# amathislab/HOISDF

Hardware: AMD Instinct MI355X
Metric: samples/sec (img + 2048 SDF queries) fwd+bwd at 1/2/4/8 MI355X (higher is better)
Workload: dtype f32 (emulated contractions, f32 accumulate, f16x2 form: operands as scaled hi + lo f16 pieces x 3 products - 22 operand bits, one power-of-two scale per ROW of a linear layer's row operand, per (sample, head) of the attention operands, per weight matrix; the attention backward's dS as three pieces x

## Files before the change

hoisdf_amd/csrc/chain.h:

```cpp
#pragma once
#include <stdlib.h>

#include <mutex>
#include <unordered_map>

#include "common.h"

namespace hoisdf {
namespace {

constexpr long EMU_MIN_ROWS = 2048;
constexpr long EMU_DW_MIN_ROWS = 8192;

inline bool al16(const void* p) { return (reinterpret_cast<uintptr_t>(p) & 15) == 0; }

struct Bump {
  char* base; long cap; long off = 0; bool overflow = false;
  Bump(void* b, long c) : base(static_cast<char*>(b)), cap(c) {}
  void* take(long bytes) {
    off = (off + 255) & ~255L;
    const long at = off;
    off += bytes;
    if (!base) return nullptr;
    if (off > cap) { overflow = true; return nullptr; }
    return base + at;
  }
  float* floats(long n) { return static_cast<float*>(take(n * 4)); }
};

struct SavedMags {
  std::mutex mu;
  std::unordered_map<const void*, int> on;
  void put(const void* key, bool v) { if (!key) return; std::lock_guard<std::mutex> l(mu); if (on.size() > 8192) on.clear(); on[key] = v ? 1 : 0; }
  int get(const void* key) { std::lock_guard<std::mutex> l(mu); auto it = on.find(key); return it == on.end() ? -1 : it->second; }
};
inline SavedMags& saved_mags() { static SavedMags s; return s; }

struct Ctx {
  hipStream_t st; void* stream;
  Bump* ws;
  bool dry;
  bool emu;
  int rc = HOISDF_OK;
  bool ok() const { return rc == HOISDF_OK; }
};

inline bool emu_small(const Ctx& c, long M, const float* a, long lda, const float* W, long ldw, int N, int K) {
  if (!c.emu || M > hoisdf_linear_emu_small_max_rows() || N % 4 || K % 4 || lda % 4 || ldw % 4) return false;
  return c.dry || hoisdf_linear_emu_small_supported(a, lda, W, ldw, M, N, K);
}
bool emu_rows(const Ctx& c, long M, const float* a, long lda, int contraction) {
  return c.emu && M >= EMU_MIN_ROWS && contraction % 4 == 0 && lda % 4 == 0 && (c.dry || al16(a));
}
const void* image_of(Ctx& c, const void* given, const float* W, int ldw, int N, int K, int transpose) {
  if (given) return given;
  void* img = c.ws->take(hoisdf_linear_emu_image_bytes(transpose ? K : N, transpose ? N : K));
  if (c.dry) return nullptr;
  if (!img) { c.rc = HOISDF_ERR_WORKSPACE; return nullptr; }
  c.rc = hoisdf_linear_emu_prepare(W, ldw, N, K, transpose, img, c.stream);
  return img;
}
void lin_fwd(Ctx& c, const float* x, int ldx, const float* W, int ldw, const void* img, const float* b, float* y, int ldy, long M, int N,
             int K, int act, float p, uint64_t seed, uint32_t* bits, int K_pad = 0, const uint32_t* x_mag = nullptr, uint32_t* y_mag = nullptr,
             uint32_t* y_heads = nullptr, int head_L = 0) {
  if (!c.ok()) return;
  if (K_pad < K || (K_pad + 15) / 16 != (K + 15) / 16) K_pad = K;
  if (emu_rows(c, M, x, ldx, K_pad)) {
    const void* im = image_of(c, img, W, ldw, N, K, 0);
    if (c.dry || !c.ok()) return;
    c.rc = linear_fwd_emu_mag(x, ldx, im, b, y, ldy, M, N, K_pad, act, p, seed, bits, x_mag, y_mag, c.stream, y_heads, head_L);
    return;
  }
  if (c.dry) return;
  if (emu_small(c, M, x, ldx, W, ldw, N, K)) { c.rc = hoisdf_linear_fwd_emu_small(x, ldx, W, ldw, b, y, ldy, M, N, K, act, p, seed, bits, c.stream); return; }
  c.rc = hoisdf_linear_fwd(x, ldx, W, ldw, b, y, ldy, M, N, K, act, p, seed, bits, c.stream);
}
void lin_bwd_input(Ctx& c, const float* dy, int lddy, const uint32_t* bits, float p, const float* W, int ldw, const void* img_t, float* dx,
                   int lddx, long M, int N, int K, int accumulate, const uint32_t* dy_mag = nullptr, uint32_t* dx_mag = nullptr,
                   uint32_t* dx_heads = nullptr, int head_L = 0) {
  if (!c.ok()) return;
  if (!bits) p = 0.f;
  if (emu_rows(c, M, dy, lddy, N)) {
    const void* im = image_of(c, img_t, W, ldw, N, K, 1);
    if (c.dry || !c.ok()) return;
    c.rc = linear_bwd_input_emu_mag(dy, lddy, bits, p, im, dx, lddx, M, N, K, accumulate, dy_mag, accumulate ? nullptr : dx_mag, c.stream,
                                    accumulate ? nullptr : dx_heads, head_L);
    return;
  }
  if (c.dry) return;
  if (emu_small(c, M, dy, lddy, W, ldw, N, K)) { c.rc = hoisdf_linear_bwd_input_emu_small(dy, lddy, bits, p, W, ldw, dx, lddx, M, N, K, accumulate, c.stream); return; }
  c.rc = hoisdf_linear_bwd_input(dy, lddy, bits, p, W, ldw, dx, lddx, M, N, K, accumulate, c.stream);
}
void lin_bwd_weight(Ctx& c, const float* dy, int lddy, const uint32_t* bits, float p, const float* x, int ldx, float* dW, float* db, long M,
                    int N, int K, int K_pad = 0, const uint32_t* dy_mag = nullptr, const uint32_t* x_mag = nullptr) {
  if (!c.ok()) return;
  if (!bits) p = 0.f;
  if (K_pad < K) K_pad = K;
  const bool emu = c.emu && M >= EMU_DW_MIN_ROWS && (N < K ? N : K) >= 64 && N % 4 == 0 && K_pad % 4 == 0 && lddy % 4 == 0 && ldx % 4 == 0 &&
                   (c.dry || (al16(dy) && al16(x) && al16(dW)));
  if (emu) {
    const long nws = hoisdf_linear_bwd_weight_emu_workspace(M, N, K_pad);
    float* w = c.ws->floats(nws > 4 ? nws : 4);
    if (!c.dry) {
      if (!w) { c.rc = HOISDF_ERR_WORKSPACE; return; }
      if (dy_mag || x_mag) c.rc = linear_bwd_weight_emu_mag(dy, lddy, bits, p, x, ldx, dW, K_pad, db, M, N, K_pad, w, nws, dy_mag, x_mag, c.stream);
      else c.rc = hoisdf_linear_bwd_weight_emu(dy, lddy, bits, p, x, ldx, dW, K_pad, db, M, N, K_pad, w, nws, c.stream);
    }
    return;
  }
  if (c.emu && M <= hoisdf_linear_emu_small_max_rows()) {
    if (!c.dry) c.rc = hoisdf_linear_bwd_weight_emu_small(dy, lddy, bits, p, x, ldx, dW, K_pad, db, M, N, K_pad, c.stream);
    return;
  }
  long nws = 0; float* w = nullptr;
  if (deterministic_mode()) {
    nws = hoisdf_linear_bwd_weight_workspace(M, N, K_pad);
    if (nws > 0) w = c.ws->floats(nws);
    if (!c.dry && nws > 0 && !w) { c.rc = HOISDF_ERR_WORKSPACE; return; }
  }
  if (c.dry) return;
  c.rc = hoisdf_linear_bwd_weight(dy, lddy, bits, p, x, ldx, dW, K_pad, db, M, N, K_pad, w, nws, c.stream);
}


}
}
```

hoisdf_amd/csrc/gemm_emu.h:

```cpp
#pragma once
#include "common.h"

namespace hoisdf {

typedef float f32x16 __attribute__((ext_vector_type(16)));
typedef float f32x4 __attribute__((ext_vector_type(4)));
typedef float f32x2 __attribute__((ext_vector_type(2)));
typedef __bf16 bf16x8 __attribute__((ext_vector_type(8)));
typedef __bf16 bf16x2 __attribute__((ext_vector_type(2)));
typedef _Float16 f16x8 __attribute__((ext_vector_type(8)));
typedef _Float16 f16x2 __attribute__((ext_vector_type(2)));
typedef unsigned int u32x4 __attribute__((ext_vector_type(4)));
typedef unsigned int u32x2 __attribute__((ext_vector_type(2)));
#define MFB(a, b, c) __builtin_amdgcn_mfma_f32_32x32x16_bf16((a), (b), (c), 0, 0, 0)
#define MFH(a, b, c) __builtin_amdgcn_mfma_f32_32x32x16_f16((a), (b), (c), 0, 0, 0)

constexpr int TM = 256, TN = 128, KS = 16, NT = 256;
constexpr int WN = TN / 2, NJ = WN / 32;
constexpr int A_U4 = 3 * 2 * TM, B_U4 = 3 * 2 * TN, STAGE_U4 = A_U4 + B_U4;
constexpr int NB = B_U4 / NT;
constexpr int HTM = 256, HTN = 256;
constexpr int HA_U4 = 2 * 2 * HTM, HB_U4 = 2 * 2 * HTN;
constexpr int H_TRAILER = 128;
constexpr int DT = 256;

#define SPLIT1(x, i)                             \
  do {                                           \
    const __bf16 a_ = (__bf16)(x);               \
    const float r1_ = (x) - (float)a_;           \
    const __bf16 b_ = (__bf16)r1_;               \
    const float r2_ = r1_ - (float)b_;           \
    p0[i] = a_; p1[i] = b_; p2[i] = (__bf16)r2_; \
  } while (0)
__device__ __forceinline__ void split3x8(const float4 u, const float4 w, bf16x8& p0, bf16x8& p1, bf16x8& p2) {
  SPLIT1(u.x, 0); SPLIT1(u.y, 1); SPLIT1(u.z, 2); SPLIT1(u.w, 3);
  SPLIT1(w.x, 4); SPLIT1(w.y, 5); SPLIT1(w.z, 6); SPLIT1(w.w, 7);
}

struct EmuArgs {
  const float* A; long lda;
  const u32x4* Bimg;
  float* C; int ldc;
  const float* bias;
  const uint32_t* abits; int ldbits; float ascale;
  uint32_t* bits_out; int ldbits_out;
  int M, N, K;
  int act; float drop_p, inv_keep; uint32_t thresh; uint64_t seed;
  int tiles_m, tiles_n, vecC, beta;
  QkvPlanes qkv;
  const uint32_t* a_amax; const float* b_scale;
  uint32_t* amax_out;
  uint32_t* head_out; int head_L, head_nb;
};

struct DwArgs {
  const float* dy; long lddy;
  const float* x; long ldx;
  const uint32_t* bits; int ldbits; float ascale;
  float* C; long c_split_stride;
  float* colsum; long colsum_split_stride;
  int M, N, K;
  int splitk, m_per_split, tiles_n, tiles_k;
  const uint32_t* dy_amax; const uint32_t* x_amax;
};

__device__ __forceinline__ uint32_t h2_exp(uint32_t amax_bits) { return mag_exp(amax_bits); }
__device__ __forceinline__ float h2_scale(uint32_t amax_bits) { return mag_scale(amax_bits); }
__device__ __forceinline__ float h2_inv_scale(uint32_t amax_bits) { return mag_inv_scale(amax_bits); }
__host__ __device__ __forceinline__ uint32_t* h2_trailer(void* image, int R, int Kc) {
  return reinterpret_cast<uint32_t*>(static_cast<char*>(image) + (size_t)((R + HTN - 1) / HTN) * ((Kc + KS - 1) / KS) * HB_U4 * 16);
}

#define EMU_PREP_FIND(items, n, lo)                                                                                    \
  int lo = 0, hi_ = (n) - 1;                                                                                           \
  while (lo < hi_) {                                                                                                   \
    const int mid_ = (lo + hi_ + 1) >> 1;                                                                              \
    if ((items)[mid_].first_block <= (long)blockIdx.x) lo = mid_; else hi_ = mid_ - 1;                                 \
  }

#define NOP_ ((void)0)
#define SYNC() do { SB(); __syncthreads(); SB(); } while (0)

#define EMU_A_DESCRIPTORS(TM_, arow0)                                                                                  \
  const int rows_in = min(TM_, g.M - m0);                                                                              \
  __amdgpu_buffer_rsrc_t rsa[4], rsm[4];                                                                               \
  _Pragma("unroll") for (int i = 0; i < 4; ++i) {                                                                      \
    const int rows_q = max(min(rows_in - i * 64, 64), 0);                              \
    rsa[i] = __builtin_amdgcn_make_buffer_rsrc(const_cast<float*>(g.A + ((size_t)(arow0) + i * 64) * g.lda), 0,        \
                                               rows_q > 0 ? (int)((((long)rows_q - 1) * g.lda + g.K) * 4) : 0, 0x00020000); \
    rsm[i] = __builtin_amdgcn_make_buffer_rsrc(const_cast<uint32_t*>(MASK ? g.abits + ((size_t)m0 + i * 64) * g.ldbits : nullptr), 0, \
                                               MASK ? (int)((long)rows_q * g.ldbits * 4) : 0, 0x00020000);             \
  }
#define EMU_A_SLOTS(TM_)                                                                                               \
  const int aoff = (int)((((long)wave * 16 + rl) * g.lda + 4 * qd) * 4);                                               \
  const int moff = (int)(((long)wave * 16 + rl) * g.ldbits * 4);                                                       \
  const int wslot = 2 * (cq * TM_ + ((wave * 16 + rl) ^ (cq << 2))) + (qd & 1);                                        \
  const int aread = (wm * 128 + l31) ^ (kh << 2);                                                                      \
  const int kq = g.K - 4 * qd;
#define EMU_LDGA(i, sl)                                                                                                \
  do {                                                                                                                 \
    const int k0_ = min((sl), last) * KS;                              \
    const f32x4 v_ = __builtin_bit_cast(f32x4, __builtin_amdgcn_raw_buffer_load_b128(rsa[i], aoff, k0_ * 4, 0));       \
    rp[2 * (i)] = f32x2{v_[0], v_[1]}; rp[2 * (i) + 1] = f32x2{v_[2], v_[3]};                                          \
    if (MASK) rm[i] = __builtin_amdgcn_raw_buffer_load_b32(rsm[i], moff, (k0_ >> 5) * 4, 0);                           \
  } while (0)
#define EMU_UI(i, sl) do { if (MASK) mb = rm[i] >> ((((sl) & 1) << 4) + 4 * qd); if (KTAIL) kin = (sl) * KS < kq; } while (0)
#define EMU_MASK_KTAIL(v_, p)                                                                                          \
  do {                                                                                                                 \
    if (MASK) {            \
      float xa_, xb_;      \
      asm("v_and_b32 %0, %1, %2" : "=v"(xa_) : "v"(__builtin_amdgcn_sbfe((int)mb, 2 * ((p) & 1), 1)), "v"(v_.x));       \
      asm("v_and_b32 %0, %1, %2" : "=v"(xb_) : "v"(__builtin_amdgcn_sbfe((int)mb, 2 * ((p) & 1) + 1, 1)), "v"(v_.y));   \
      v_ = f32x2{xa_, xb_};                                                                                            \
    }                                                                                                                  \
    if (KTAIL) { if (!kin) v_ = f32x2{0.f, 0.f}; }              \
  } while (0)

template <int TM_, int TN_, int NJ_>
__device__ __forceinline__ void emu_epilogue(const EmuArgs& g, f32x16 (&acc)[4][NJ_], u32x4* lds, int m0, int n0, int wm, int wn, int wave,
                                             int lane, int l31, int kh, float post_scale, const float* row_post = nullptr) {
  constexpr int WN_ = TN_ / 2;
  static_assert(WN_ == NJ_ * 32, "wave tile");
  if (row_post) {
#pragma unroll
    for (int i = 0; i < 4; ++i)
#pragma unroll
      for (int q = 0; q < 4; ++q) {
        const f32x4 ps = *reinterpret_cast<const f32x4*>(row_post + wm * 128 + i * 32 + 8 * q + 4 * kh);
#pragma unroll
        for (int j = 0; j < NJ_; ++j)
#pragma unroll
          for (int e = 0; e < 4; ++e) acc[i][j][4 * q + e] *= ps[e];
      }
  } else if (post_scale != 1.f) {
#pragma unroll
    for (int j = 0; j < NJ_; ++j)
#pragma unroll
      for (int i = 0; i < 4; ++i)
#pragma unroll
        for (int r = 0; r < 16; ++r) acc[i][j][r] *= post_scale;
  }
  const int rbase = m0 + wm * 128 + 4 * kh;
  const int cbase = n0 + wn * WN_ + l31;
#pragma unroll
  for (int j = 0; j < NJ_; ++j) {
    const int col = cbase + j * 32;
    const float bv = (g.bias != nullptr && col < g.N) ? g.bias[col] : 0.f;
#pragma unroll
    for (int i = 0; i < 4; ++i)
#pragma unroll
      for (int r = 0; r < 16; ++r) {
        float v = acc[i][j][r] + bv;
        if (g.act == 1) v = fmaxf(v, 0.f);
        acc[i][j][r] = v;
      }
  }
  if (g.drop_p > 0.f) {
#pragma unroll
    for (int i = 0; i < 4; ++i)
#pragma unroll
      for (int r = 0; r < 16; ++r) {
        const int row = rbase + i * 32 + (r & 3) + 8 * (r >> 2);
        const uint32_t rk = drop_rowkey(g.seed, (uint32_t)row);
#pragma unroll
        for (int j = 0; j < NJ_; ++j) acc[i][j][r] *= drop_scale(rk, (uint32_t)(cbase + j * 32), g.thresh, g.inv_keep);
      }
  }
  if (g.head_out) {
    const int row0 = m0 + wm * 128;
    if (row0 < g.M) {
      const int b0 = row0 / g.head_L, b1 = (min(row0 + 127, g.M - 1)) / g.head_L;
#pragma unroll
      for (int hh = 0; hh < NJ_ / 2; ++hh) {
        float m = 0.f;
#pragma unroll
        for (int j = 0; j < 2; ++j)
#pragma unroll
          for (int i = 0; i < 4; ++i)
#pragma unroll
            for (int r = 0; r < 16; ++r) m = fmaxf(m, __builtin_fabsf(acc[i][2 * hh + j][r]));
        uint32_t mb = group_max_u32<64>(__builtin_bit_cast(uint32_t, m));
        const int grp = (n0 + wn * WN_ + hh * 64) >> 6;
        if (lane == 0 && n0 + wn * WN_ + hh * 64 < g.N)
          for (int b = b0; b <= b1; ++b) atomicMax(g.head_out + (size_t)grp * g.head_nb + b, mb);
      }
    }
  }
  if (g.qkv.on) {
    constexpr int ES = 64 + 4;
    float* w = reinterpret_cast<float*>(lds) + wave * (32 * ES);
    const int row0 = m0 + wm * 128, cw = n0 + wn * WN_;
    if (row0 + 128 > g.M || cw + WN_ > g.N) return;
    const int b = row0 / g.qkv.L, s0 = row0 - b * g.qkv.L;
#pragma unroll
    for (int hh = 0; hh < NJ_ / 2; ++hh) {
      const int colg = g.qkv.col0 + cw + hh * 64;
      const int part = colg / g.qkv.E, head = (colg - part * g.qkv.E) >> 6;
      const size_t bh = (size_t)b * g.qkv.H + head;
      const float sc = part == 0 ? g.qkv.qscale : 1.f;
      __bf16* const r0 = static_cast<__bf16*>(g.qkv.r[part][0]);
      __bf16* const r1 = static_cast<__bf16*>(g.qkv.r[part][1]);
      __bf16* const r2 = static_cast<__bf16*>(g.qkv.r[part][2]);
      const bool trn = part == 2 && g.qkv.vt[0] != nullptr;
#pragma unroll
      for (int i = 0; i < 4; ++i) {
#pragma unroll
        for (int j = 0; j < 2; ++j)
#pragma unroll
          for (int r = 0; r < 16; ++r) w[((r & 3) + 8 * (r >> 2) + 4 * kh) * ES + j * 32 + l31] = acc[i][2 * hh + j][r] * sc;
        if (r0) {
#pragma unroll
          for (int p = 0; p < 4; ++p) {
            const int rr = p * 8 + (lane >> 3), cc = (lane & 7) * 8;
            const float4 u = *reinterpret_cast<const float4*>(w + rr * ES + cc);
            const float4 v = *reinterpret_cast<const float4*>(w + rr * ES + cc + 4);
            bf16x8 p0, p1, p2;
            split3x8(u, v, p0, p1, p2);
            const size_t o = ((size_t)bh * g.qkv.Lp + s0 + i * 32 + rr) * 64 + cc;
            *reinterpret_cast<bf16x8*>(r0 + o) = p0;
            *reinterpret_cast<bf16x8*>(r1 + o) = p1;
            *reinterpret_cast<bf16x8*>(r2 + o) = p2;
          }
        }
        if (trn) {
          __bf16* const t0 = static_cast<__bf16*>(g.qkv.vt[0]);
          __bf16* const t1 = static_cast<__bf16*>(g.qkv.vt[1]);
          __bf16* const t2 = static_cast<__bf16*>(g.qkv.vt[2]);
#pragma unroll
          for (int q = 0; q < 4; ++q) {
            const float* c0 = w + (8 * q) * ES + lane;
            const float4 u = make_float4(c0[0], c0[ES], c0[2 * ES], c0[3 * ES]);
            const float4 v = make_float4(c0[4 * ES], c0[5 * ES], c0[6 * ES], c0[7 * ES]);
            bf16x8 p0, p1, p2;
            split3x8(u, v, p0, p1, p2);
            const size_t o = ((size_t)bh * 64 + lane) * g.qkv.Lp + s0 + i * 32 + 8 * q;
            *reinterpret_cast<bf16x8*>(t0 + o) = p0;
            *reinterpret_cast<bf16x8*>(t1 + o) = p1;
            *reinterpret_cast<bf16x8*>(t2 + o) = p2;
          }
        }
      }
    }
    return;
  }
  const bool full = (m0 + TM_ <= g.M) && (n0 + TN_ <= g.N);
  const bool stream_c = !g.beta && (long)g.M * g.N >= (16L << 20);
  if (full && g.vecC) {
    constexpr int ES = WN_ + 4, LPR = WN_ / 4, RPI = 64 / LPR;
    float* w = reinterpret_cast<float*>(lds) + wave * (32 * ES);
#pragma unroll
    for (int i = 0; i < 4; ++i) {
#pragma unroll
      for (int j = 0; j < NJ_; ++j)
#pragma unroll
        for (int r = 0; r < 16; ++r) w[((r & 3) + 8 * (r >> 2) + 4 * kh) * ES + j * 32 + l31] = acc[i][j][r];
      if (g.amax_out) {
        const float* rp = w + l31 * ES + kh * (WN_ / 2);
        float m = 0.f;
#pragma unroll
        for (int q = 0; q < WN_ / 8; ++q) {
          const float4 t = *reinterpret_cast<const float4*>(rp + 4 * q);
          m = __builtin_fmaxf(__builtin_fmaxf(m, __builtin_fabsf(t.x)), __builtin_fmaxf(__builtin_fabsf(t.y), __builtin_fmaxf(__builtin_fabsf(t.z), __builtin_fabsf(t.w))));
        }
        uint32_t mb = __builtin_bit_cast(uint32_t, m);
        mb = max(mb, (uint32_t)__shfl_xor((int)mb, 32, 64));
        if (kh == 0) atomicMax(g.amax_out + (m0 + wm * 128 + i * 32 + l31), mb);
      }
#pragma unroll
      for (int p = 0; p < 32 / RPI; ++p) {
        const int rr = p * RPI + lane / LPR, cc = (lane % LPR) * 4;
        float4 v = *reinterpret_cast<const float4*>(w + rr * ES + cc);
        float4* cp = reinterpret_cast<float4*>(g.C + (size_t)(m0 + wm * 128 + i * 32 + rr) * g.ldc + n0 + wn * WN_ + cc);
        if (g.beta) {
          const float4 old = *cp;
          v.x += old.x; v.y += old.y; v.z += old.z; v.w += old.w;
        }
        typedef float v4f_ __attribute__((ext_vector_type(4)));
#ifdef H2_ABL_NOSTORE
        if (g.seed != 0x5eed5eed5eedull) continue;
#endif
        if (stream_c) __builtin_nontemporal_store(v4f_{v.x, v.y, v.z, v.w}, reinterpret_cast<v4f_*>(cp));
        else *cp = v;
      }
    }
  } else {
#pragma unroll
    for (int j = 0; j < NJ_; ++j)
#pragma unroll
      for (int i = 0; i < 4; ++i)
#pragma unroll
        for (int r = 0; r < 16; ++r) {
          const int row = rbase + i * 32 + (r & 3) + 8 * (r >> 2), col = cbase + j * 32;
          if (row < g.M && col < g.N) {
            float* cp = g.C + (size_t)row * g.ldc + col;
            *cp = g.beta ? *cp + acc[i][j][r] : acc[i][j][r];
          }
        }
    if (g.amax_out) {
#pragma unroll
      for (int i = 0; i < 4; ++i)
#pragma unroll
        for (int r = 0; r < 16; ++r) {
          const int row = rbase + i * 32 + (r & 3) + 8 * (r >> 2);
          uint32_t mb = 0u;
#pragma unroll
          for (int j = 0; j < NJ_; ++j) if (cbase + j * 32 < g.N) mb = max(mb, mag_bits(acc[i][j][r]));
          mb = group_max_u32<32>(mb);
          if (l31 == 0 && row < g.M) atomicMax(g.amax_out + row, mb);
        }
    }
  }
  if (g.bits_out) {
    uint32_t wd[2][NJ_];
#pragma unroll
    for (int hh = 0; hh < 2; ++hh)
#pragma unroll
      for (int j = 0; j < NJ_; ++j) wd[hh][j] = 0u;
#pragma unroll
    for (int i = 0; i < 4; ++i)
#pragma unroll
      for (int r = 0; r < 16; ++r) {
        const int rl = (i & 1) * 32 + (r & 3) + 8 * (r >> 2);
#pragma unroll
        for (int j = 0; j < NJ_; ++j) {
          const unsigned long long q = __ballot(acc[i][j][r] > 0.f);
          if (lane == rl) wd[i >> 1][j] = (uint32_t)q;
          if (lane == rl + 4) wd[i >> 1][j] = (uint32_t)(q >> 32);
        }
      }
    const int wcol = (n0 + wn * WN_) >> 5;
    const int nvalid = g.N - (n0 + wn * WN_);
#pragma unroll
    for (int hh = 0; hh < 2; ++hh) {
      const int row = m0 + wm * 128 + hh * 64 + lane;
      if (row < g.M) {
#pragma unroll
        for (int j = 0; j < NJ_; ++j) {
          const int nv = nvalid - 32 * j;
          if (nv > 0) g.bits_out[(size_t)row * g.ldbits_out + wcol + j] = nv >= 32 ? wd[hh][j] : (wd[hh][j] & ((1u << nv) - 1u));
        }
      }
    }
  }
}

int emu_b3_prepare(const float* W, int ldw, int R, int Kc, int transpose, void* image, hipStream_t st);
int emu_b3_prepare_batch(const hoisdf_emu_prep_item* d_items, int n, long total_blocks, hipStream_t st);
int emu_b3_launch(EmuArgs g, hipStream_t st);
int emu_h2_prepare(const float* W, int ldw, int N, int K, int transpose, void* image, hipStream_t st);
int emu_h2_prepare_batch(const hoisdf_emu_prep_item* d_items, int n, long total_blocks, hipStream_t st);
int emu_h2_launch(EmuArgs g, hipStream_t st);
int dw_tile(int K);
void plan_dw(long M, int N, int K, int& splitk, int& mper);
int emu_dw_launch(const DwArgs& g, bool h2, float* dW, float* db, float* workspace, hipStream_t st);
}
```

hoisdf_amd/csrc/gemm_emu.hip:

```cpp
#include <stdlib.h>

#include <map>
#include <mutex>
#include <unordered_map>
#include <utility>

#include "gemm_emu.h"

namespace hoisdf {

__global__ __launch_bounds__(256) void emu_rowmag_kernel(const float* __restrict__ x, long ld, long M, int K, uint32_t* __restrict__ words) {
  constexpr int RPW = 8;
  const int lane = threadIdx.x & 63;
  const long row0 = ((long)blockIdx.x * 4 + (threadIdx.x >> 6)) * RPW;
  const int k4 = K >> 2;
  uint32_t m[RPW];
#pragma unroll
  for (int r = 0; r < RPW; ++r) {
    m[r] = 0u;
    if (row0 + r < M)
      for (int c = lane; c < k4; c += 64) {
        const u32x4 v = *reinterpret_cast<const u32x4*>(x + (row0 + r) * ld + 4 * c);
        m[r] = max(m[r], max(max(v[0] & 0x7fffffffu, v[1] & 0x7fffffffu), max(v[2] & 0x7fffffffu, v[3] & 0x7fffffffu)));
      }
// ... 159 lines not shown

int hoisdf::linear_fwd_emu_mag(const float* x, int ldx, const void* w_image, const float* bias, float* y, int ldy, long M, int N, int K,
                               int act, float drop_p, uint64_t seed, uint32_t* relu_bits, const uint32_t* x_mag, uint32_t* y_mag,
                               void* stream, uint32_t* y_heads, int head_L) {
  HOISDF_REQUIRE(M == 0 || (x && w_image && y), HOISDF_ERR_INVALID, "linear_fwd_emu: null pointer");
  HOISDF_REQUIRE(M >= 0 && N > 0 && K > 0 && ldx >= K && ldy >= N && M < (1L << 31), HOISDF_ERR_INVALID,
                 "linear_fwd_emu: bad sizes M=%ld N=%d K=%d ldx=%d ldy=%d", M, N, K, ldx, ldy);
  HOISDF_REQUIRE(drop_p >= 0.f && drop_p < 1.f, HOISDF_ERR_INVALID, "linear_fwd_emu: drop_p=%f", drop_p);
  if (M == 0) return HOISDF_OK;
  HOISDF_REQUIRE(hoisdf_linear_emu_supported(x, ldx, K), HOISDF_ERR_INVALID,
                 "linear_fwd_emu: x must be 16-byte aligned with ldx and K multiples of 4 (use hoisdf_linear_fwd otherwise)");
  EmuArgs g{};
  g.A = x; g.lda = ldx; g.Bimg = static_cast<const u32x4*>(w_image);
  g.C = y; g.ldc = ldy; g.bias = bias; g.M = (int)M; g.N = N; g.K = K;
  g.act = act; g.drop_p = drop_p; g.inv_keep = 1.f / (1.f - drop_p); g.thresh = drop_threshold(drop_p); g.seed = seed;
  g.bits_out = relu_bits; g.ldbits_out = (N + 31) / 32;
  g.a_amax = x_mag; g.amax_out = y_mag;
  if (y_heads) {
    HOISDF_REQUIRE(head_L > 0 && N % 64 == 0, HOISDF_ERR_INVALID, "linear_fwd_emu: head magnitudes need N %% 64 == 0 and the rows per sample");
    g.head_out = y_heads; g.head_L = head_L; g.head_nb = cdiv(M, head_L);
  }
  return launch_emu(g, as_stream(stream));
}

int hoisdf::linear_fwd_emu_qkv(const float* x, int ldx, const void* w_image, const float* bias, long M, int N, int K,
                               const QkvPlanes& pl, void* stream, const uint32_t* x_mag) {
  HOISDF_REQUIRE(x && w_image && M > 0 && N > 0 && K > 0 && ldx >= K && M < (1L << 31), HOISDF_ERR_INVALID, "linear_fwd_emu_qkv: bad arguments");
  HOISDF_REQUIRE(hoisdf_linear_emu_supported(x, ldx, K), HOISDF_ERR_INVALID, "linear_fwd_emu_qkv: x alignment / K");
  HOISDF_REQUIRE(pl.on && pl.L > 0 && pl.L % 128 == 0 && M % pl.L == 0 && N % 64 == 0 && pl.E % 64 == 0 && pl.Lp >= pl.L &&
                     pl.col0 % 64 == 0 && pl.col0 + N <= 3 * pl.E,
                 HOISDF_ERR_INVALID, "linear_fwd_emu_qkv: plane geometry (L=%d Lp=%d N=%d E=%d col0=%d)", pl.L, pl.Lp, N, pl.E, pl.col0);
  EmuArgs g{};
  g.A = x; g.lda = ldx; g.Bimg = static_cast<const u32x4*>(w_image);
  g.C = nullptr; g.ldc = N; g.bias = bias; g.M = (int)M; g.N = N; g.K = K;
  g.inv_keep = 1.f; g.qkv = pl;
  g.a_amax = x_mag;
  return launch_emu(g, as_stream(stream));
}

extern "C" int hoisdf_linear_fwd_emu_heads(const float* x, int ldx, const void* w_image, const float* bias, float* y, int ldy, long M, int N,
                                           int K, const uint32_t* x_mag, uint32_t* y_mag, uint32_t* y_heads, int L, void* stream) {
  HOISDF_REQUIRE(y_heads, HOISDF_ERR_INVALID, "linear_fwd_emu_heads: y_heads is required");
  return linear_fwd_emu_mag(x, ldx, w_image, bias, y, ldy, M, N, K, 0, 0.f, 0, nullptr, x_mag, y_mag, stream, y_heads, L);
}
extern "C" int hoisdf_linear_bwd_input_emu_heads(const float* dy, int lddy, const void* wt_image, float* dx, int lddx, long M, int N, int K,
                                                 const uint32_t* dy_mag, uint32_t* dx_mag, uint32_t* dx_heads, int L, void* stream) {
  HOISDF_REQUIRE(dx_heads, HOISDF_ERR_INVALID, "linear_bwd_input_emu_heads: dx_heads is required");
  return linear_bwd_input_emu_mag(dy, lddy, nullptr, 0.f, wt_image, dx, lddx, M, N, K, 0, dy_mag, dx_mag, stream, dx_heads, L);
}
extern "C" int hoisdf_linear_bwd_input_emu(const float* dy, int lddy, const uint32_t* relu_bits, float drop_p,
                                           const void* wt_image, float* dx, int lddx, long M, int N, int K, int accumulate,
                                           void* stream) {
  return linear_bwd_input_emu_mag(dy, lddy, relu_bits, drop_p, wt_image, dx, lddx, M, N, K, accumulate, nullptr, nullptr, stream);
}
extern "C" int hoisdf_linear_bwd_input_emu_mag(const float* dy, int lddy, const uint32_t* relu_bits, float drop_p,
                                               const void* wt_image, float* dx, int lddx, long M, int N, int K, int accumulate,
                                               const uint32_t* dy_mag, uint32_t* dx_mag, void* stream) {
  return linear_bwd_input_emu_mag(dy, lddy, relu_bits, drop_p, wt_image, dx, lddx, M, N, K, accumulate, dy_mag, dx_mag, stream);
}

int hoisdf::linear_bwd_input_emu_mag(const float* dy, int lddy, const uint32_t* relu_bits, float drop_p, const void* wt_image, float* dx,
                                     int lddx, long M, int N, int K, int accumulate, const uint32_t* dy_mag, uint32_t* dx_mag,
                                     void* stream, uint32_t* dx_heads, int head_L) {
  HOISDF_REQUIRE(M == 0 || (dy && wt_image && dx), HOISDF_ERR_INVALID, "linear_bwd_input_emu: null pointer");
  HOISDF_REQUIRE(M >= 0 && N > 0 && K > 0 && lddy >= N && lddx >= K && M < (1L << 31) && drop_p >= 0.f && drop_p < 1.f,
                 HOISDF_ERR_INVALID, "linear_bwd_input_emu: bad sizes");
  if (M == 0) return HOISDF_OK;
  HOISDF_REQUIRE(hoisdf_linear_emu_supported(dy, lddy, N), HOISDF_ERR_INVALID,
                 "linear_bwd_input_emu: dy must be 16-byte aligned with lddy and N multiples of 4");
  EmuArgs g{};
  g.A = dy; g.lda = lddy; g.Bimg = static_cast<const u32x4*>(wt_image);
  g.abits = relu_bits; g.ldbits = (N + 31) / 32; g.ascale = 1.f / (1.f - drop_p);
  g.C = dx; g.ldc = lddx; g.M = (int)M; g.N = K; g.K = N;
  g.inv_keep = 1.f;
  g.beta = accumulate ? 1 : 0;
  g.a_amax = dy_mag; g.amax_out = dx_mag;
  if (dx_heads) {
    HOISDF_REQUIRE(head_L > 0 && K % 64 == 0 && !accumulate, HOISDF_ERR_INVALID, "linear_bwd_input_emu: head magnitudes need K %% 64 == 0, the rows per sample, no accumulation");
    g.head_out = dx_heads; g.head_L = head_L; g.head_nb = cdiv(M, head_L);
  }
  return launch_emu(g, as_stream(stream));
}

extern "C" long hoisdf_linear_bwd_weight_emu_workspace(long M, int N, int K) {
  if (M <= 0 || N <= 0 || K <= 0) return 0;
  int splitk, mper;
  plan_dw(M, N, K, splitk, mper);
  if (splitk <= 1) return 0;
  return (long)splitk * ((long)N * K + N);
}

namespace {
int bwd_weight_emu(const float* dy, int lddy, const uint32_t* relu_bits, float drop_p, const float* x, int ldx, float* dW, int lddw,
                   float* db, long M, int N, int K, float* workspace, long workspace_floats, bool h2, const uint32_t* dy_mag,
                   const uint32_t* x_mag, void* stream) {
  HOISDF_REQUIRE(dW && (M == 0 || (dy && x)), HOISDF_ERR_INVALID, "linear_bwd_weight_emu: null pointer");
  HOISDF_REQUIRE(M > 0 && N > 0 && K > 0 && lddy >= N && ldx >= K && lddw == K && M < (1L << 31) && drop_p >= 0.f && drop_p < 1.f,
                 HOISDF_ERR_INVALID, "linear_bwd_weight_emu: bad sizes (a dense dW, lddw == K, is required)");
  HOISDF_REQUIRE(al16(dy) && al16(x) && al16(dW) && (lddy % 4 == 0) && (ldx % 4 == 0) && (N % 4 == 0) && (K % 4 == 0),
                 HOISDF_ERR_INVALID, "linear_bwd_weight_emu: operands must be 16-byte aligned with N, K and leading dims multiples of 4");
  hipStream_t st = as_stream(stream);
  DwArgs g{};
  g.dy = dy; g.lddy = lddy; g.x = x; g.ldx = ldx;
  g.bits = relu_bits; g.ldbits = (N + 31) / 32; g.ascale = 1.f / (1.f - drop_p);
  g.M = (int)M; g.N = N; g.K = K;
  const int dtk = dw_tile(K);
  g.tiles_n = cdiv(N, DT); g.tiles_k = cdiv(K, dtk);
  plan_dw(M, N, K, g.splitk, g.m_per_split);
  const long need = g.splitk > 1 ? (long)g.splitk * ((long)N * K + N) : 0;
  HOISDF_REQUIRE(need == 0 || (workspace && workspace_floats >= need && al16(workspace)), HOISDF_ERR_WORKSPACE,
                 "linear_bwd_weight_emu: workspace of %ld floats needed", need);
  if (g.splitk > 1) {
    g.C = workspace; g.c_split_stride = (long)N * K;
    g.colsum = db ? workspace + (size_t)g.splitk * N * K : nullptr; g.colsum_split_stride = N;
  } else {
    g.C = dW; g.c_split_stride = 0; g.colsum = db; g.colsum_split_stride = 0;
  }
  if (dtk == 256 && h2) {
    g.dy_amax = dy_mag; g.x_amax = x_mag;
    if (!dy_mag) {
      uint32_t* part = mag_scratch(st, M);
      if (!part) { set_error("linear_bwd_weight_emu: cannot allocate the row magnitudes"); return HOISDF_ERR_LAUNCH; }
      mag_trace("grad-weight dy", M, N);
      if (int rc = emu_rowmag_launch(dy, lddy, M, N, part, st)) return rc;
      g.dy_amax = part;
    }
    if (!x_mag) {
      uint32_t* part = mag_scratch(st, M);
      if (!part) { set_error("linear_bwd_weight_emu: cannot allocate the row magnitudes"); return HOISDF_ERR_LAUNCH; }
      mag_trace("grad-weight x", M, K);
      if (int rc = emu_rowmag_launch(x, ldx, M, K, part, st)) return rc;
      g.x_amax = part;
    }
  }
  return emu_dw_launch(g, h2, dW, db, workspace, st);
}
}

extern "C" int hoisdf_linear_bwd_weight_emu(const float* dy, int lddy, const uint32_t* relu_bits, float drop_p, const float* x,
                                            int ldx, float* dW, int lddw, float* db, long M, int N, int K, float* workspace,
                                            long workspace_floats, void* stream) {
  return bwd_weight_emu(dy, lddy, relu_bits, drop_p, x, ldx, dW, lddw, db, M, N, K, workspace, workspace_floats, false, nullptr, nullptr, stream);
}
int hoisdf::linear_bwd_weight_emu_mag(const float* dy, int lddy, const uint32_t* relu_bits, float drop_p, const float* x, int ldx,
                                      float* dW, int lddw, float* db, long M, int N, int K, float* workspace, long workspace_floats,
                                      const uint32_t* dy_mag, const uint32_t* x_mag, void* stream) {
  return bwd_weight_emu(dy, lddy, relu_bits, drop_p, x, ldx, dW, lddw, db, M, N, K, workspace, workspace_floats, form_h2(), dy_mag, x_mag, stream);
}
extern "C" int hoisdf_linear_bwd_weight_emu_mag(const float* dy, int lddy, const uint32_t* relu_bits, float drop_p, const float* x,
                                                int ldx, float* dW, int lddw, float* db, long M, int N, int K, float* workspace,
                                                long workspace_floats, const uint32_t* dy_mag, const uint32_t* x_mag, void* stream) {
  return linear_bwd_weight_emu_mag(dy, lddy, relu_bits, drop_p, x, ldx, dW, lddw, db, M, N, K, workspace, workspace_floats, dy_mag, x_mag, stream);
}
```

hoisdf_amd/csrc/gemm_emu_dw.hip:

```cpp
#include "gemm_emu.h"

namespace hoisdf {

namespace {
__device__ __forceinline__ uint64_t uni64(uint64_t v) {
  const uint32_t lo = __builtin_amdgcn_readfirstlane((uint32_t)v), hi = __builtin_amdgcn_readfirstlane((uint32_t)(v >> 32));
  return ((uint64_t)hi << 32) | lo;
}
}

#define DW_TILE_SETUP(DTK_)                                                                                            \
  const int tid = threadIdx.x, lane = tid & 63, wave = tid >> 6;                                                       \
  const int wm = wave >> 1, wn = wave & 1;                                                                             \
  const int l31 = lane & 31, kh = lane >> 5;                                                                           \
  const int ntile = g.tiles_n * g.tiles_k;                                                                             \
  const int bid = blockIdx.x;                                                                                          \
  const int split = (bid & 7) + 8 * (bid / (8 * ntile));       \
  const int t = (bid >> 3) % ntile;                                                                                    \
  if (split >= g.splitk) return;                                                                                       \
  const int tn = t / g.tiles_k, tk = t - tn * g.tiles_k;                                                               \
  const int n0 = tn * DT, k0 = tk * DTK_;                                                                              \
  const int mbeg = split * g.m_per_split;                                                                              \
  const int mend = min(g.M, mbeg + g.m_per_split);                                                                     \
  const int nslab = (mend - mbeg + KS - 1) / KS;

#define DW2_STORE_COLSUM()                                                                                             \
  do {                                                                                                                 \
    if (HASDB && tk == 0) {                                                                                            \
      float* red = reinterpret_cast<float*>(lds);                                                                      \
      if (isA) *reinterpret_cast<f32x4*>(&red[c * DT + 4 * cg]) = csum * post;                                         \
      __syncthreads();                                                                                                 \
      if (tid < DT) {                                                                                                  \
        const int n = n0 + tid;                                                                                        \
        if (n < g.N) g.colsum[(size_t)split * g.colsum_split_stride + n] = red[tid] + red[DT + tid];                   \
      }                                                                                                                \
      __syncthreads();                                                                                                 \
    }                                                                                                                  \
  } while (0)
#define DW_EPILOGUE(DTK_, VAL)                                                                                         \
  do {                                                                                                                 \
    float* Cb = g.C + (size_t)split * g.c_split_stride;                                                                \
    const bool full = (n0 + DT <= g.N) && (k0 + (DTK_) <= g.K) && (g.K % 4 == 0);                                      \
    constexpr int WK_ = (DTK_) / 2, ES = WK_ + 4;                                                                      \
    constexpr int LPR = WK_ / 4, RPI = 64 / LPR;           \
    float* w = reinterpret_cast<float*>(lds) + wave * (32 * ES);                                                       \
    _Pragma("unroll") for (int i = 0; i < 4; ++i) {                                                                    \
      _Pragma("unroll") for (int j = 0; j < (DTK_) / 64; ++j)                                                          \
        _Pragma("unroll") for (int r = 0; r < 16; ++r) w[((r & 3) + 8 * (r >> 2) + 4 * kh) * ES + j * 32 + l31] = (VAL); \
      _Pragma("unroll") for (int p = 0; p < 32 / RPI; ++p) {                                                           \
        const int rr = p * RPI + lane / LPR, cc = (lane % LPR) * 4;                                                    \
        const int row = n0 + wm * 128 + i * 32 + rr, col = k0 + wn * WK_ + cc;                                         \
        const float4 v = *reinterpret_cast<const float4*>(w + rr * ES + cc);                                           \
        if (full) {                                                                                                    \
          *reinterpret_cast<float4*>(Cb + (size_t)row * g.K + col) = v;                                                \
        } else if (row < g.N) {                                                                                        \
          float* cp = Cb + (size_t)row * g.K + col;                                                                    \
          if (col + 0 < g.K) cp[0] = v.x;                                                                              \
          if (col + 1 < g.K) cp[1] = v.y;                                                                              \
          if (col + 2 < g.K) cp[2] = v.z;                                                                              \
          if (col + 3 < g.K) cp[3] = v.w;                                                                              \
        }                                                                                                              \
      }                                                                                                                \
    }                                                                                                                  \
  } while (0)

template <bool MASK, int DTK>
__global__ __launch_bounds__(NT, DTK == 256 ? 1 : 2) void emu_dw_kernel(DwArgs g) {
  constexpr int NJ = DTK / 64;
  constexpr int WK = DTK / 2;
  constexpr int A_U4 = 3 * 2 * DT, STAGE = A_U4 + 3 * 2 * DTK;
  extern __shared__ __attribute__((aligned(16))) u32x4 lds[];
  DW_TILE_SETUP(DTK)
  const int last = nslab - 1;

  f32x16 acc[4][NJ];
#pragma unroll
  for (int i = 0; i < 4; ++i)
#pragma unroll
    for (int j = 0; j < NJ; ++j)
#pragma unroll
      for (int r = 0; r < 16; ++r) acc[i][j][r] = 0.f;

  const bool isA = tid < 128;
  const bool stager = DTK == 256 || tid < 192;
  const int cg = (isA || DTK == 256) ? (tid & 63) : (tid & 31), c = (isA || DTK == 256) ? ((tid >> 6) & 1) : ((tid >> 5) & 1);
  const int col0 = (isA ? n0 : k0) + 4 * cg;
  const int ncol = isA ? g.N : g.K;
  const bool col_ok = stager && col0 < ncol;
  const long ld = uni64(isA ? g.lddy : g.ldx);
  const char* opbase = reinterpret_cast<const char*>(g.dy) +
                       (long)uni64(isA ? 0ul : (uint64_t)(reinterpret_cast<const char*>(g.x) - reinterpret_cast<const char*>(g.dy)));
  const uint32_t voff = (uint32_t)(((long)c * 8 * ld + (col_ok ? col0 : 0)) * 4);
  const char* bitbase = reinterpret_cast<const char*>(g.bits);
  const uint32_t boff = (uint32_t)(((long)c * 8 * g.ldbits + ((col_ok ? col0 : 0) >> 5)) * 4);
  const float* src = (isA ? g.dy : g.x) + (col_ok ? col0 : 0);
  const uint32_t* bsrc = (MASK && isA) ? g.bits + ((col_ok ? col0 : 0) >> 5) : nullptr;
  const int bsh = col0 & 31;
  const bool do_colsum = isA && g.colsum != nullptr && tk == 0;
  float4 rv[8];
  uint32_t rm[8];
  float4 csum = make_float4(0.f, 0.f, 0.f, 0.f);
#define DW_LOAD(sl)                                                                                                   \
  do {                                                                                                                \
    const int ms_ = mbeg + (sl) * KS;                                            \
    if (ms_ + KS <= g.M) {                                                                                            \
      const char* sb_ = opbase + (size_t)ms_ * ld * 4;                                                                \
      const char* mb2_ = bitbase + (size_t)ms_ * g.ldbits * 4;                                                        \
      _Pragma("unroll") for (int e = 0; e < 8; ++e) {                                                                 \
        rv[e] = *reinterpret_cast<const float4*>(sb_ + (size_t)e * ld * 4 + voff);                                    \
        if (MASK) rm[e] = isA ? *reinterpret_cast<const uint32_t*>(mb2_ + (size_t)e * g.ldbits * 4 + boff) : 0xffffffffu; \
      }                                                                                                               \
    } else {                                                       \
      const int mb_ = ms_ + c * 8;                                                                                    \
      _Pragma("unroll") for (int e = 0; e < 8; ++e) {                                                                 \
        const int m_ = min(mb_ + e, g.M - 1);                                                                         \
        rv[e] = *reinterpret_cast<const float4*>(src + (size_t)m_ * ld);                                              \
        if (MASK) rm[e] = isA ? bsrc[(size_t)m_ * g.ldbits] : 0xffffffffu;                                            \
      }                                                                                                               \
    }                                                                                                                 \
  } while (0)
#define DW_STORE(st, sl)                                                                                              \
  do {                                                                                                                \
    const int mb_ = mbeg + (sl) * KS + c * 8;                                                                         \
    _Pragma("unroll") for (int e = 0; e < 8; ++e) {                                                                   \
      float4 v_ = rv[e];                                                                                              \
      if (MASK && isA) {                                                                                              \
        const uint32_t nib_ = rm[e] >> bsh;                                                                           \
        v_.x = (nib_ & 1u) ? v_.x * g.ascale : 0.f;                                                                   \
        v_.y = (nib_ & 2u) ? v_.y * g.ascale : 0.f;                                                                   \
        v_.z = (nib_ & 4u) ? v_.z * g.ascale : 0.f;                                                                   \
        v_.w = (nib_ & 8u) ? v_.w * g.ascale : 0.f;                                                                   \
      }                                                                                                               \
      rv[e] = v_;                                                                                                     \
    }                                                                                                                 \
    if (!col_ok || mbeg + (sl) * KS + KS > mend) {            \
      _Pragma("unroll") for (int e = 0; e < 8; ++e)                                                                   \
        if (mb_ + e >= mend || !col_ok) rv[e] = make_float4(0.f, 0.f, 0.f, 0.f);                                      \
    }                                                                                                                 \
    if (do_colsum) {                                                                                                  \
      _Pragma("unroll") for (int e = 0; e < 8; ++e) {                                                                 \
        csum.x += rv[e].x; csum.y += rv[e].y; csum.z += rv[e].z; csum.w += rv[e].w;                                   \
      }                                                                                                               \
    }                                                                                                                 \
    const int rs_ = isA ? DT : DTK;                                \
    u32x4* dst_ = (st) + (isA ? 0 : A_U4) + c * rs_ + 4 * cg;                                                         \
    bf16x8 p0, p1, p2;                                                                                                \
    split3x8(make_float4(rv[0].x, rv[1].x, rv[2].x, rv[3].x), make_float4(rv[4].x, rv[5].x, rv[6].x, rv[7].x), p0, p1, p2); \
    dst_[0] = __builtin_bit_cast(u32x4, p0); dst_[2 * rs_] = __builtin_bit_cast(u32x4, p1); dst_[4 * rs_] = __builtin_bit_cast(u32x4, p2); \
    split3x8(make_float4(rv[0].y, rv[1].y, rv[2].y, rv[3].y), make_float4(rv[4].y, rv[5].y, rv[6].y, rv[7].y), p0, p1, p2); \
    dst_[1] = __builtin_bit_cast(u32x4, p0); dst_[2 * rs_ + 1] = __builtin_bit_cast(u32x4, p1); dst_[4 * rs_ + 1] = __builtin_bit_cast(u32x4, p2); \
    split3x8(make_float4(rv[0].z, rv[1].z, rv[2].z, rv[3].z), make_float4(rv[4].z, rv[5].z, rv[6].z, rv[7].z), p0, p1, p2); \
    dst_[2] = __builtin_bit_cast(u32x4, p0); dst_[2 * rs_ + 2] = __builtin_bit_cast(u32x4, p1); dst_[4 * rs_ + 2] = __builtin_bit_cast(u32x4, p2); \
    split3x8(make_float4(rv[0].w, rv[1].w, rv[2].w, rv[3].w), make_float4(rv[4].w, rv[5].w, rv[6].w, rv[7].w), p0, p1, p2); \
    dst_[3] = __builtin_bit_cast(u32x4, p0); dst_[2 * rs_ + 3] = __builtin_bit_cast(u32x4, p1); dst_[4 * rs_ + 3] = __builtin_bit_cast(u32x4, p2); \
  } while (0)

  if (nslab > 0 && stager) {
    DW_LOAD(0);
    DW_STORE(lds, 0);
    DW_LOAD(min(1, last));
  }
  __syncthreads();

  for (int s = 0; s < nslab; ++s) {
    const u32x4* st = lds + (s & 1) * STAGE;
    u32x4* nx = lds + ((s + 1) & 1) * STAGE;
    const u32x4* sa = st + wm * 128 + l31;
    const u32x4* sb = st + A_U4 + wn * WK + l31;
    bf16x8 b0[NJ], b1[NJ], b2[NJ], a[4];
#define RD_B(dst, p) _Pragma("unroll") for (int j = 0; j < NJ; ++j) dst[j] = __builtin_bit_cast(bf16x8, sb[((p) * 2 + kh) * DTK + j * 32])
#define RD_A(p) _Pragma("unroll") for (int i = 0; i < 4; ++i) a[i] = __builtin_bit_cast(bf16x8, sa[((p) * 2 + kh) * DT + i * 32])
#define MM1(bx) _Pragma("unroll") for (int i = 0; i < 4; ++i) _Pragma("unroll") for (int j = 0; j < NJ; ++j) acc[i][j] = MFB(a[i], bx[j], acc[i][j])
    RD_B(b0, 0); RD_A(0); RD_B(b1, 1); RD_B(b2, 2);
    MM1(b2); MM1(b1); MM1(b0);
    __builtin_amdgcn_sched_barrier(0);
    RD_A(1);
    if (stager) {
      if (s + 1 < nslab) DW_STORE(nx, s + 1);
      DW_LOAD(min(s + 2, last));
    }
    __builtin_amdgcn_sched_barrier(0);
    MM1(b1); MM1(b0);
    RD_A(2);
    MM1(b0);
    __syncthreads();
  }
#undef DW_LOAD
#undef DW_STORE
#undef RD_A
#undef RD_B
#undef MM1

  if (g.colsum != nullptr && tk == 0) {
    float* red = reinterpret_cast<float*>(lds);
    if (isA) *reinterpret_cast<float4*>(&red[c * DT + 4 * cg]) = csum;
    __syncthreads();
    if (tid < DT) {
      const int n = n0 + tid;
      if (n < g.N) g.colsum[(size_t)split * g.colsum_split_stride + n] = red[tid] + red[DT + tid];
    }
    __syncthreads();
  }

  DW_EPILOGUE(DTK, acc[i][j][r]);
}

#define DW2_STAGING_SETUP(A_U4_)                                                                                       \
   \
  const bool isA = wave < 2;                                                                                           \
  const int c = wave & 1, cg = lane;                                                                                   \
  const int col0 = (isA ? n0 : k0) + 4 * cg;                                                                           \
  const bool col_ok = col0 < (isA ? g.N : g.K);              \
  const long ld = uni64(isA ? g.lddy : g.ldx);                                                                         \
  const char* opbase = reinterpret_cast<const char*>(g.dy) +                                                           \
                       (long)uni64(isA ? 0ul : (uint64_t)(reinterpret_cast<const char*>(g.x) - reinterpret_cast<const char*>(g.dy))); \
   \
                                            \
  const int voff0 = col_ok ? (int)(((long)c * 8 * ld + col0) * 4) : 0x40000000;                                        \
  const int boff0 = (MASK && isA && col_ok) ? (int)(((long)c * 8 * g.ldbits + (col0 >> 5)) * 4) : 0x40000000;          \
  const int ldb4 = (int)(ld * 4), ldm4 = g.ldbits * 4;                                                                 \
  const uint32_t notA = isA ? 0u : 0xffffffffu;                                         \
  const int bsh = col0 & 31;                                    \
  constexpr bool SWZ = true;                                                                                           \
  const int sw = SWZ ? (cg >> 1) & 3 : 0;                                                                              \
  const int wbase = (isA ? 0 : A_U4_) + c * DT + 4 * cg;        \
  const int rsw = SWZ ? (l31 >> 3) & 3 : 0;                                                                            \
  const int aread = (wm * 128 + l31) ^ rsw, bread = A_U4_ + ((wn * 128 + l31) ^ rsw);                                  \
  f32x2 rvL[8], rvH[8];                                            \
  uint32_t rm[8], mpk = 0xffffffffu;
#define DSLAB(sl)                                                                                                      \
    const int ms_ = mbeg + (sl) * KS;                                                                                  \
    const int left_ = max(mend - ms_, 0);
#define DLDG(hf, e, sl)                                                                                                \
  do {                                                                                                                 \
    DSLAB(sl)                                                                                                          \
    const __amdgpu_buffer_rsrc_t r_ = __builtin_amdgcn_make_buffer_rsrc(                                               \
        const_cast<char*>(opbase + (size_t)ms_ * ld * 4), 0, (int)min((long)left_ * ld * 4, 0x3fffffffL), 0x00020000); \
    const f32x2 v_ = __builtin_bit_cast(f32x2, __builtin_amdgcn_raw_buffer_load_b64(r_, voff0 + (e) * ldb4 + (hf) * 8, 0, 0)); \
    if ((hf) == 0) rvL[e] = v_; else rvH[e] = v_;                                                                      \
  } while (0)
#define DLDM(e, sl)                                                                                                    \
  do {                                                                                                                 \
    if (MASK) {                                                                                                        \
      DSLAB(sl)                                                                                                        \
      const __amdgpu_buffer_rsrc_t b_ = __builtin_amdgcn_make_buffer_rsrc(                                             \
          const_cast<uint32_t*>(g.bits + (size_t)ms_ * g.ldbits), 0, (int)min((long)left_ * g.ldbits * 4, 0x3fffffffL), 0x00020000); \
      rm[e] = __builtin_amdgcn_raw_buffer_load_b32(b_, boff0 + (e) * ldm4, 0, 0);                                      \
    }                                                                                                                  \
  } while (0)
#define DLOAD_ALL(sl) _Pragma("unroll") for (int e = 0; e < 8; ++e) { DLDG(0, e, sl); DLDG(1, e, sl); }
#define DLOADM_ALL(sl) _Pragma("unroll") for (int e = 0; e < 8; ++e) DLDM(e, sl)

namespace {
constexpr int DSTAGE = 3 * 2 * DT * 2;
}
template <bool MASK, bool HASDB>
__global__ __launch_bounds__(NT, 1) void emu_dw2_kernel(DwArgs g) {
  constexpr int A_U4 = 3 * 2 * DT;
  __shared__ __attribute__((aligned(16))) u32x4 s0[DSTAGE];
  __shared__ __attribute__((aligned(16))) u32x4 s1[DSTAGE];
  DW_TILE_SETUP(DT)

  f32x16 acc[4][4];
#pragma unroll
  for (int i = 0; i < 4; ++i)
#pragma unroll
    for (int j = 0; j < 4; ++j)
#pragma unroll
      for (int r = 0; r < 16; ++r) acc[i][j][r] = 0.f;

  DW2_STAGING_SETUP(A_U4)
  uint32_t t0[4], t1[4], t2[4];
  f32x2 rp_, fu_;
  f32x4 csum = {0.f, 0.f, 0.f, 0.f};
#define DU1(j, pr)                                                                                                     \
  do {                                                                                                                 \
    f32x2 v_ = (j) < 2 ? f32x2{rvL[2 * (pr)][(j) & 1], rvL[2 * (pr) + 1][(j) & 1]} : f32x2{rvH[2 * (pr)][(j) & 1], rvH[2 * (pr) + 1][(j) & 1]}; \
    if (MASK) {                                                                                                        \
      if ((j) == 0) {                                                                                                  \
        const uint32_t n0_ = ((rm[2 * (pr)] | notA) >> bsh) & 0xfu, n1_ = ((rm[2 * (pr) + 1] | notA) >> bsh) & 0xfu;   \
        mpk = ((pr) == 0 ? 0u : mpk) | (n0_ << (8 * (pr))) | (n1_ << (8 * (pr) + 4));                                  \
      }                                                                                                                \
      float xa_, xb_;                                                              \
      asm("v_and_b32 %0, %1, %2" : "=v"(xa_) : "v"(__builtin_amdgcn_sbfe((int)mpk, 8 * (pr) + (j), 1)), "v"(v_.x));    \
      asm("v_and_b32 %0, %1, %2" : "=v"(xb_) : "v"(__builtin_amdgcn_sbfe((int)mpk, 8 * (pr) + 4 + (j), 1)), "v"(v_.y)); \
      v_ = f32x2{xa_, xb_};                                                                                            \
    }                                                                                                                  \
    if (HASDB) csum[j] += v_.x + v_.y;                                                                                 \
    const uint32_t h_ = __builtin_bit_cast(uint32_t, __builtin_convertvector(v_, bf16x2));                             \
    t0[pr] = h_; rp_ = v_;                                                                                             \
    fu_ = f32x2{__builtin_bit_cast(float, h_ << 16), __builtin_bit_cast(float, h_ & 0xffff0000u)};                     \
  } while (0)
#define DU2(j, pr) PK_SUB(rp_, rp_, fu_)
#define DU3(j, pr)                                                                                                     \
  do {                                                                                                                 \
    const uint32_t h_ = __builtin_bit_cast(uint32_t, __builtin_convertvector(rp_, bf16x2));                            \
    t1[pr] = h_;                                                                                                       \
    fu_ = f32x2{__builtin_bit_cast(float, h_ << 16), __builtin_bit_cast(float, h_ & 0xffff0000u)};                     \
  } while (0)
#define DU4(j, pr) do { f32x2 w_; PK_SUB(w_, rp_, fu_); t2[pr] = __builtin_bit_cast(uint32_t, __builtin_convertvector(w_, bf16x2)); } while (0)
#define DSTA(st, j, pl) (st)[wbase + ((j) ^ sw) + (pl) * 2 * DT] = ((pl) == 0 ? u32x4{t0[0], t0[1], t0[2], t0[3]} : (pl) == 1 ? u32x4{t1[0], t1[1], t1[2], t1[3]} : u32x4{t2[0], t2[1], t2[2], t2[3]})
#define DLA(st, p, i) __builtin_bit_cast(bf16x8, (st)[aread + ((p) * 2 + kh) * DT + (i) * 32])
#define DLB(st, p, j) __builtin_bit_cast(bf16x8, (st)[bread + ((p) * 2 + kh) * DT + (j) * 32])
#define M1(ax, bx, i, j, work) do { acc[i][j] = MFB(ax[i], bx[j], acc[i][j]); work; SB(); } while (0)
#define MM(ax, bx) _Pragma("unroll") for (int i = 0; i < 4; ++i) _Pragma("unroll") for (int j = 0; j < 4; ++j) acc[i][j] = MFB(ax[i], bx[j], acc[i][j])
#include "dw2_phase.inc"
#define DSTAGE_ALL(st)                                                                                                 \
  do {                                                                                                                 \
    _Pragma("unroll") for (int j = 0; j < 4; ++j) {                                                                    \
      _Pragma("unroll") for (int pr = 0; pr < 4; ++pr) { DU1(j, pr); DU2(j, pr); DU3(j, pr); DU4(j, pr); }             \
      DSTA(st, j, 0); DSTA(st, j, 1); DSTA(st, j, 2);                                                                  \
    }                                                                                                                  \
  } while (0)

  const int nslab2 = (max(nslab, 1) + 1) & ~1;
  bf16x8 aX[4], aY[4], aZ[4], bP[4], bQ[4], bR[4];
  DLOAD_ALL(0);
  DLOADM_ALL(0);
  DSTAGE_ALL(s0);
  DLOAD_ALL(1);
  DLOADM_ALL(1);
  __syncthreads();
#pragma unroll
  for (int i = 0; i < 4; ++i) { aZ[i] = DLA(s0, 0, i); aX[i] = DLA(s0, 1, i); aY[i] = DLA(s0, 2, i); }
#pragma unroll
  for (int j = 0; j < 4; ++j) { bQ[j] = DLB(s0, 0, j); bP[j] = DLB(s0, 1, j); bR[j] = DLB(s0, 2, j); }
  MM(aZ, bR); MM(aZ, bP); MM(aZ, bQ);
  DSTAGE_ALL(s1);
  DLOAD_ALL(2);
  DLOADM_ALL(2);
  SYNC();
  for (int s = 1; s + 1 < nslab2; s += 2) {
    DPHASE(s1, s0, s, aX, aY, aZ, bP, bQ, bR);
    SYNC();
    DPHASE(s0, s1, s + 1, aX, aY, aZ, bR, bQ, bP);
    SYNC();
  }
  DPHASE(s1, s0, nslab2 - 1, aX, aY, aZ, bP, bQ, bR);
  SB();
  MM(aX, bR); MM(aX, bQ); MM(aY, bQ);
  __syncthreads();
#undef DU1
#undef DU2
#undef DU3
#undef DU4
#undef DSTA
#undef DLA
#undef DLB
#undef M1
#undef MM
#undef DPHASE
#undef DSTAGE_ALL
  const float post = MASK ? g.ascale : 1.f;
  u32x4* lds = s0;
  DW2_STORE_COLSUM();
  DW_EPILOGUE(DT, MASK ? acc[i][j][r] * post : acc[i][j][r]);
}

template <bool MASK, bool HASDB>
__global__ __launch_bounds__(NT, 1) void emu_dw2h_kernel(DwArgs g) {
  constexpr int A_U4 = 2 * 2 * DT;
  constexpr int STG = 2 * A_U4;
  constexpr int EPI = (4 * 32 * (DT / 2 + 4) * 4 + 15) / 16;
  __shared__ __attribute__((aligned(16))) u32x4 lds_all[2 * STG > EPI ? 2 * STG : EPI];
  __shared__ uint32_t red4[4];
  u32x4* const s0 = lds_all;
  u32x4* const s1 = lds_all + STG;
  DW_TILE_SETUP(DT)
  f16_saturate_on();
  uint32_t am_dy = 0u, am_x = 0u;
  for (int i = mbeg + (int)threadIdx.x; i < mend; i += NT) { am_dy = max(am_dy, g.dy_amax[i]); am_x = max(am_x, g.x_amax[i]); }
  am_dy = block_max_u32(am_dy, red4);
  __syncthreads();
  am_x = block_max_u32(am_x, red4);

  f32x16 acc[4][4];
#pragma unroll
  for (int i = 0; i < 4; ++i)
#pragma unroll
    for (int j = 0; j < 4; ++j)
#pragma unroll
      for (int r = 0; r < 16; ++r) acc[i][j][r] = 0.f;

  DW2_STAGING_SETUP(A_U4)
  uint32_t t0[4], t1[4];
  const float sc = isA ? h2_scale(am_dy) : h2_scale(am_x);
  f32x2 rp_, fu_;
  f32x4 csum = {0.f, 0.f, 0.f, 0.f};
#define DU1(j, pr)                                                                                                     \
  do {                                                                                                                 \
    f32x2 v_ = (j) < 2 ? f32x2{rvL[2 * (pr)][(j) & 1], rvL[2 * (pr) + 1][(j) & 1]} : f32x2{rvH[2 * (pr)][(j) & 1], rvH[2 * (pr) + 1][(j) & 1]}; \
    if (MASK) {                                                                                                        \
      if ((j) == 0) {                                                                                                  \
        const uint32_t n0_ = ((rm[2 * (pr)] | notA) >> bsh) & 0xfu, n1_ = ((rm[2 * (pr) + 1] | notA) >> bsh) & 0xfu;   \
        mpk = ((pr) == 0 ? 0u : mpk) | (n0_ << (8 * (pr))) | (n1_ << (8 * (pr) + 4));                                  \
      }                                                                                                                \
      float xa_, xb_;                                                              \
      asm("v_and_b32 %0, %1, %2" : "=v"(xa_) : "v"(__builtin_amdgcn_sbfe((int)mpk, 8 * (pr) + (j), 1)), "v"(v_.x));    \
      asm("v_and_b32 %0, %1, %2" : "=v"(xb_) : "v"(__builtin_amdgcn_sbfe((int)mpk, 8 * (pr) + 4 + (j), 1)), "v"(v_.y)); \
      v_ = f32x2{xa_, xb_};                                                                                            \
    }                                                                                                                  \
    if (HASDB) csum[j] += v_.x + v_.y;                                                                                 \
    v_ *= sc;                                                                                                          \
    const f16x2 h_ = __builtin_convertvector(v_, f16x2);                       \
    t0[pr] = __builtin_bit_cast(uint32_t, h_); rp_ = v_;                                                               \
    fu_ = __builtin_convertvector(h_, f32x2);                                                                          \
  } while (0)
#define DU2(j, pr) do { f32x2 w_; PK_SUB(w_, rp_, fu_); t1[pr] = __builtin_bit_cast(uint32_t, __builtin_convertvector(w_, f16x2)); } while (0)
#define DSTA(st, j, pl) (st)[wbase + ((j) ^ sw) + (pl) * 2 * DT] = ((pl) == 0 ? u32x4{t0[0], t0[1], t0[2], t0[3]} : u32x4{t1[0], t1[1], t1[2], t1[3]})
#define DLA(st, p, i) __builtin_bit_cast(f16x8, (st)[aread + ((p) * 2 + kh) * DT + (i) * 32])
#define DLB(st, p, j) __builtin_bit_cast(f16x8, (st)[bread + ((p) * 2 + kh) * DT + (j) * 32])
#define M1(ax, bx, i, j, work) do { acc[i][j] = MFH(ax[i], bx[j], acc[i][j]); work; SB(); } while (0)
#define MM(ax, bx) _Pragma("unroll") for (int i = 0; i < 4; ++i) _Pragma("unroll") for (int j = 0; j < 4; ++j) acc[i][j] = MFH(ax[i], bx[j], acc[i][j])
#include "dw2h_phase.inc"
#define DSTAGE_ALL(st)                                                                                                 \
  do {                                                                                                                 \
    _Pragma("unroll") for (int j = 0; j < 4; ++j) {                                                                    \
      _Pragma("unroll") for (int pr = 0; pr < 4; ++pr) { DU1(j, pr); DU2(j, pr); }                                     \
      DSTA(st, j, 0); DSTA(st, j, 1);                                                                                  \
    }                                                                                                                  \
  } while (0)

  const int nslab2 = (max(nslab, 1) + 1) & ~1;
  f16x8 aH[4], aL[4], bP[4], bQ[4], bL[4];
  DLOAD_ALL(0);
  DLOADM_ALL(0);
  DSTAGE_ALL(s0);
  DLOAD_ALL(1);
  DLOADM_ALL(1);
  __syncthreads();
#pragma unroll
  for (int i = 0; i < 4; ++i) { aL[i] = DLA(s0, 1, i); aH[i] = DLA(s0, 0, i); }
#pragma unroll
  for (int j = 0; j < 4; ++j) { bP[j] = DLB(s0, 0, j); bL[j] = DLB(s0, 1, j); }
  MM(aL, bP); MM(aH, bL);
  DSTAGE_ALL(s1);
  DLOAD_ALL(2);
  DLOADM_ALL(2);
  SYNC();
  for (int s = 1; s + 1 < nslab2; s += 2) {
    DHPHASE(s1, s0, s, bP, bQ);
    SYNC();
    DHPHASE(s0, s1, s + 1, bQ, bP);
    SYNC();
  }
  DHPHASE(s1, s0, nslab2 - 1, bP, bQ);
  SB();
  MM(aH, bQ);
  __syncthreads();
#undef DU1
#undef DU2
#undef DSTA
#undef DLA
#undef DLB
#undef M1
#undef MM
#undef DHPHASE
#undef DSTAGE_ALL
  const float unscale = h2_inv_scale(am_dy) * h2_inv_scale(am_x);
  const float post = MASK ? g.ascale : 1.f;
  u32x4* lds = lds_all;
  DW2_STORE_COLSUM();
  DW_EPILOGUE(DT, acc[i][j][r] * (MASK ? post * unscale : unscale));
}

__global__ __launch_bounds__(1024) void emu_reduce_partials_kernel(const float* __restrict__ part, long stride, int splits,
                                                                   float* __restrict__ out, long n, int blocks0,
                                                                   const float* __restrict__ part1, long stride1,
                                                                   float* __restrict__ out1, long n1) {
  __shared__ float4 red[16][64];
  const int lane = threadIdx.x & 63, w = threadIdx.x >> 6;
  int blk = blockIdx.x;
  if (blk >= blocks0) { blk -= blocks0; part = part1; stride = stride1; out = out1; n = n1; }
  const long i = ((long)blk * 64 + lane) * 4;
  float4 s = make_float4(0.f, 0.f, 0.f, 0.f);
  if (i < n) {
    const float* p = part + i;
    int k = w;
    for (; k + 16 < splits; k += 32) {
      const float4 u = *reinterpret_cast<const float4*>(p + (size_t)k * stride);
      const float4 v = *reinterpret_cast<const float4*>(p + (size_t)(k + 16) * stride);
      s.x += u.x; s.y += u.y; s.z += u.z; s.w += u.w;
      s.x += v.x; s.y += v.y; s.z += v.z; s.w += v.w;
    }
    if (k < splits) {
      const float4 u = *reinterpret_cast<const float4*>(p + (size_t)k * stride);
      s.x += u.x; s.y += u.y; s.z += u.z; s.w += u.w;
    }
  }
  red[w][lane] = s;
  __syncthreads();
  if (w == 0 && i < n) {
    float4 t = red[0][lane];
#pragma unroll
    for (int j = 1; j < 16; ++j) {
      const float4 v = red[j][lane];
      t.x += v.x; t.y += v.y; t.z += v.z; t.w += v.w;
    }
    *reinterpret_cast<float4*>(out + i) = t;
  }
}

int dw_tile(int K) { return K <= 128 ? 128 : 256; }
void plan_dw(long M, int N, int K, int& splitk, int& mper) {
  const int dtk = dw_tile(K);
  const int ntile = cdiv(N, DT) * cdiv(K, dtk);
  const int slabs = cdiv(M, KS);
  const int slots = dtk == 256 ? 256 : 512;
  const int per_xcd = slots / 8 / ntile;
  int want = per_xcd >= 1 ? per_xcd * 8 : (ntile >= slots ? 1 : slots / ntile);
  if (want > slabs / 8) want = slabs / 8 > 0 ? slabs / 8 : 1;
  mper = cdiv(slabs, want) * KS;
  splitk = cdiv(M, mper);
}

int emu_dw_launch(const DwArgs& g, bool h2, float* dW, float* db, float* workspace, hipStream_t st) {
  const int dtk = dw_tile(g.K);
  const unsigned lb = 2u * (3 * 2 * DT + 3 * 2 * 128) * 16u;
  static bool attr_set = false;
  if (!attr_set) {
    auto raise = [&](const void* k) { return hipFuncSetAttribute(k, hipFuncAttributeMaxDynamicSharedMemorySize, (int)lb) == hipSuccess; };
    const bool ok = raise(reinterpret_cast<const void*>(emu_dw_kernel<false, 128>)) && raise(reinterpret_cast<const void*>(emu_dw_kernel<true, 128>));
    if (!ok) {
      set_error("linear_bwd_weight_emu: cannot raise the dynamic LDS limit");
      return HOISDF_ERR_LAUNCH;
    }
    attr_set = true;
  }
  const dim3 grid((unsigned)(g.tiles_n * g.tiles_k * 8 * cdiv(g.splitk, 8))), block(NT);
  const bool mask = g.bits != nullptr, hasdb = g.colsum != nullptr;
  static void (*const dw2h[2][2])(DwArgs) = {{emu_dw2h_kernel<false, false>, emu_dw2h_kernel<false, true>},
                                             {emu_dw2h_kernel<true, false>, emu_dw2h_kernel<true, true>}};
  static void (*const dw2[2][2])(DwArgs) = {{emu_dw2_kernel<false, false>, emu_dw2_kernel<false, true>},
                                            {emu_dw2_kernel<true, false>, emu_dw2_kernel<true, true>}};
  if (dtk == 256) hipLaunchKernelGGL((h2 ? dw2h : dw2)[mask][hasdb], grid, block, 0, st, g);
  else hipLaunchKernelGGL((mask ? emu_dw_kernel<true, 128> : emu_dw_kernel<false, 128>), grid, block, lb, st, g);
  if (int rc = check_launch("linear_bwd_weight_emu")) return rc;
  if (g.splitk > 1) {
    const long n = (long)g.N * g.K;
    const int b0 = (int)((n + 255) / 256), b1 = db ? (g.N + 255) / 256 : 0;
    hipLaunchKernelGGL(emu_reduce_partials_kernel, dim3((unsigned)(b0 + b1)), dim3(1024), 0, st, workspace, n, g.splitk, dW, n, b0,
                       workspace + (size_t)g.splitk * g.N * g.K, (long)g.N, db, (long)g.N);
    return check_launch("linear_bwd_weight_emu reduce");
  }
  return HOISDF_OK;
}

}
```

hoisdf_amd/csrc/heads.hip:

```cpp
#include "chain.h"

using namespace hoisdf;

namespace {
constexpr int MLP_MAX = HOISDF_MLP_MAX_LAYERS;
inline long bits_words(int N) { return (N + 31) / 32; }

struct MlpSaved { float* h[MLP_MAX]; uint32_t* bits[MLP_MAX]; uint32_t* mag; };

bool mlp_ok(const hoisdf_mlp* m) {
  if (!m || m->n_layers < 1 || m->n_layers > MLP_MAX) return false;
  for (int i = 0; i <= m->n_layers; ++i) if (m->dims[i] <= 0) return false;
  return true;
}
void mlp_carve(const hoisdf_mlp* m, long M, Bump& b, MlpSaved& s) {
  const int last = m->n_layers - 1;
  for (int i = 0; i < m->n_layers; ++i) {
    s.h[i] = i < last ? b.floats(M * m->dims[i + 1]) : nullptr;
    const bool act = i < last || m->act_last;
    s.bits[i] = act ? static_cast<uint32_t*>(b.take(M * bits_words(m->dims[i + 1]) * 4)) : nullptr;
  }
  s.mag = static_cast<uint32_t*>(b.take((long)m->n_layers * M * 4));
}
inline bool chain_mags_on(const Ctx& c, long M) { return c.emu && emu_form_h2() && M >= EMU_MIN_ROWS; }
uint32_t* chain_mags(Ctx& c, long M, int n) {
  if (!chain_mags_on(c, M)) return nullptr;
  uint32_t* p = static_cast<uint32_t*>(c.ws->take((long)n * M * 4));
  if (c.dry || !p || !c.ok()) return nullptr;
  if (hipMemsetAsync(p, 0, (size_t)n * M * 4, c.st) != hipSuccess) { c.rc = HOISDF_ERR_LAUNCH; return nullptr; }
  return p;
}
void mlp_forward(Ctx& c, const hoisdf_mlp* m, const float* x, int ldx, long M, const MlpSaved& s, float* y, int ldy, const uint32_t* x_mag = nullptr) {
  const int last = m->n_layers - 1;
  const float* in = x; int ldin = ldx;
  uint32_t* mg = chain_mags_on(c, M) && !c.dry && s.mag && c.ok() ? s.mag : nullptr;
  if (!c.dry) saved_mags().put(s.mag, mg != nullptr);
  if (mg && hipMemsetAsync(mg, 0, (size_t)m->n_layers * M * 4, c.st) != hipSuccess) { c.rc = HOISDF_ERR_LAUNCH; return; }
  const uint32_t* in_mag = mg ? x_mag : nullptr;
  if (mg && !in_mag && emu_rows(c, M, x, ldx, m->dims[0])) {
    if ((c.rc = emu_mag_measure(x, ldx, M, m->dims[0], mg, c.st)) != HOISDF_OK) return;
    in_mag = mg;
  }
  for (int i = 0; i < m->n_layers; ++i) {
    float* out = i < last ? s.h[i] : y;
    const int ldo = i < last ? m->dims[i + 1] : ldy;
    uint32_t* out_mag = mg && i < last && emu_rows(c, M, in, ldin, m->dims[i]) ? mg + (long)(i + 1) * M : nullptr;
    lin_fwd(c, in, ldin, m->w[i], m->dims[i], m->img[i], m->b[i], out, ldo, M, m->dims[i + 1], m->dims[i], s.bits[i] ? 1 : 0, 0.f, 0, s.bits[i], 0,
            in_mag, out_mag);
    in = out; ldin = ldo; in_mag = out_mag;
  }
}
void mlp_backward(Ctx& c, const hoisdf_mlp* m, const hoisdf_mlp_grads* G, const float* x, int ldx, long M, const MlpSaved& s, const float* dy,
                  int lddy, float* dx, int lddx, int accumulate_dx, const uint32_t* x_mag = nullptr) {
  const float* g = dy; int ldg = lddy;
  const int last = m->n_layers - 1;
  uint32_t* mg = chain_mags(c, M, m->n_layers + 1);
  const bool fwd_mags = mg && s.mag && saved_mags().get(s.mag) != 0;
  const uint32_t* g_mag = nullptr;
  if (mg && emu_rows(c, M, dy, lddy, m->dims[last + 1])) {
    if ((c.rc = emu_mag_measure(dy, lddy, M, m->dims[last + 1], mg + (long)(last + 1) * M, c.st)) != HOISDF_OK) return;
    g_mag = mg + (long)(last + 1) * M;
  }
  for (int i = last; i >= 0; --i) {
    const float* in = i > 0 ? s.h[i - 1] : x;
    const int ldin = i > 0 ? m->dims[i] : ldx;
    const uint32_t* in_mag = !fwd_mags ? nullptr : i > 0 ? (emu_rows(c, M, i > 1 ? s.h[i - 2] : x, i > 1 ? m->dims[i - 1] : ldx, m->dims[i - 1]) ? s.mag + (long)i * M : nullptr)
                                                         : (x_mag ? x_mag : (emu_rows(c, M, x, ldx, m->dims[0]) ? s.mag : nullptr));
    lin_bwd_weight(c, g, ldg, s.bits[i], 0.f, in, ldin, G->dw[i], G->db[i], M, m->dims[i + 1], m->dims[i], 0, g_mag, g_mag ? in_mag : nullptr);
    if (i == 0 && !dx) break;
    float* gin = i > 0 ? c.ws->floats(M * m->dims[i]) : dx;
    const int ldgin = i > 0 ? m->dims[i] : lddx;
    if (!c.dry && c.ok() && !gin) { c.rc = HOISDF_ERR_WORKSPACE; return; }
    uint32_t* gin_mag = mg && i > 0 && emu_rows(c, M, g, ldg, m->dims[i + 1]) ? mg + (long)i * M : nullptr;
    lin_bwd_input(c, g, ldg, s.bits[i], 0.f, m->w[i], m->dims[i], m->img_t[i], gin, ldgin, M, m->dims[i + 1], m->dims[i], i == 0 ? accumulate_dx : 0,
                  g_mag, gin_mag);
    g = gin; ldg = ldgin; g_mag = gin_mag;
  }
}
const uint32_t* enc_mag(const Ctx& c, const hoisdf_mlp* m, const float* x, int ldx, long M, const MlpSaved& s) {
  return chain_mags_on(c, M) && !c.dry && s.mag && saved_mags().get(s.mag) != 0 && emu_rows(c, M, x, ldx, m->dims[0]) ? s.mag : nullptr;
}
bool grads_ok(const hoisdf_mlp* m, const hoisdf_mlp_grads* G) {
  if (!G) return false;
  for (int i = 0; i < m->n_layers; ++i) if (!G->dw[i] || !G->db[i]) return false;
  return true;
}

struct TokSaved { float* feat; float* fea; MlpSaved mlp; };
void tok_carve(const hoisdf_mlp* m, long M, bool own_feat, Bump& b, TokSaved& s) {
  s.feat = own_feat ? b.floats(M * m->dims[0]) : nullptr;
  s.fea = b.floats(M * m->dims[m->n_layers]);
  mlp_carve(m, M, b, s.mlp);
}

struct VoteSaved { float *off, *cls, *stats; MlpSaved vote, cl; };
void vote_carve(const hoisdf_mlp* mv, const hoisdf_mlp* mc, long M, int LB, int J, Bump& b, VoteSaved& s) {
  s.off = b.floats(M * 3 * J); s.cls = b.floats(M * J); s.stats = b.floats((long)LB * J * 2);
  mlp_carve(mv, M, b, s.vote); mlp_carve(mc, M, b, s.cl);
}
}

extern "C" long hoisdf_tokens_saved_bytes(const hoisdf_mlp* mlp, long n_rows, int gather_inside) {
  if (!mlp_ok(mlp) || n_rows <= 0) return 0;
  Bump b(nullptr, 0); TokSaved s;
  tok_carve(mlp, n_rows, gather_inside != 0, b, s);
  return b.off + 256;
}

static int tokens_backward(const hoisdf_mlp* mlp, const hoisdf_mlp_grads* G, const float* feat, long M, TokSaved& s, const float* dtok,
                           const float* sdf, const float* beta, float* dfeat, int accumulate_dfeat, float* dbeta, int B, int P, int S, int row0,
                           int D, Bump& ws, bool dry, void* stream) {
  Ctx c{as_stream(stream), stream, &ws, dry, gemm_emu_mode()};
  const int F = mlp->dims[mlp->n_layers];
  float* dfea = ws.floats(M * F);
  float* part = ws.floats(hoisdf_token_build_bwd_partials());
  if (!dry) {
    if (!dfea || !part) { set_error("tokens_bwd: workspace too small"); return HOISDF_ERR_WORKSPACE; }
    c.rc = hoisdf_token_build_bwd_ordered(dtok, s.fea, F, sdf, beta, dfea, F, dbeta, part, B, P, S, row0, D, stream);
  }
  mlp_backward(c, mlp, G, feat, mlp->dims[0], M, s.mlp, dfea, F, dfeat, mlp->dims[0], accumulate_dfeat);
  if (c.ok() && !dry && ws.overflow) { set_error("tokens_bwd: workspace too small"); return HOISDF_ERR_WORKSPACE; }
  return c.rc;
}

extern "C" long hoisdf_tokens_workspace_bytes(const hoisdf_mlp* mlp, long n_rows, int backward_pass) {
  if (!mlp_ok(mlp) || n_rows <= 0) return 0;
  Bump ws(nullptr, 0), sv(nullptr, 0);
  TokSaved s; tok_carve(mlp, n_rows, false, sv, s);
  Ctx c{nullptr, nullptr, &ws, true, gemm_emu_mode()};
  if (backward_pass) {
    hoisdf_mlp_grads G{};
    (void)tokens_backward(mlp, &G, nullptr, n_rows, s, nullptr, nullptr, nullptr, reinterpret_cast<float*>(1), 0, nullptr, 1, 1, 1, 0, 1, ws, true, nullptr);
  } else {
    mlp_forward(c, mlp, nullptr, mlp->dims[0], n_rows, s.mlp, nullptr, mlp->dims[mlp->n_layers]);
  }
  return ws.off + 256;
}

extern "C" int hoisdf_tokens_fwd(const hoisdf_pyramid* pyr, const float* points, const float* center, const float* cam_intr, float scale,
                                 int img_h, int img_w, const float* feat_in, const float* cam_in, const hoisdf_mlp* mlp, const float* pe,
                                 const float* sdf, const float* beta_ptr, float* tok, float* fea_out, float* cam_out, int B, int P, int S,
                                 int row0, int D, void* saved, long saved_bytes, void* workspace, long workspace_bytes, void* stream) {
  HOISDF_REQUIRE(mlp_ok(mlp) && center && pe && sdf && beta_ptr && tok && saved && workspace, HOISDF_ERR_INVALID, "tokens_fwd: null pointer / bad MLP");
  HOISDF_REQUIRE(B > 0 && P > 0 && S >= row0 + P && row0 >= 0 && mlp->act_last && mlp->dims[mlp->n_layers] == D - 33, HOISDF_ERR_INVALID,
                 "tokens_fwd: bad sizes (the MLP must end in D - 33 = %d activated columns)", D - 33);
  const bool gather = feat_in == nullptr;
  HOISDF_REQUIRE(gather ? (pyr && points && cam_intr && cam_out) : (cam_in != nullptr), HOISDF_ERR_INVALID,
                 "tokens_fwd: either gathered rows + their camera points, or a pyramid + points + cam_out");
  const long M = (long)B * P;
  HOISDF_REQUIRE(saved_bytes >= hoisdf_tokens_saved_bytes(mlp, M, gather), HOISDF_ERR_WORKSPACE, "tokens_fwd: saved buffer of %ld bytes, need %ld", saved_bytes,
                 hoisdf_tokens_saved_bytes(mlp, M, gather));
  Bump sv(saved, saved_bytes), ws(workspace, workspace_bytes);
  TokSaved s; tok_carve(mlp, M, gather, sv, s);
  Ctx c{as_stream(stream), stream, &ws, false, gemm_emu_mode()};
  const int C = mlp->dims[0], F = D - 33;
  const float* feat = feat_in;
  const float* cam = cam_in;
  if (gather) {
    c.rc = hoisdf_project_gather_fwd(pyr, points, nullptr, M, P, center, cam_intr, scale, img_h, img_w, s.feat, C, cam_out, nullptr, stream);
    feat = s.feat; cam = cam_out;
  }
  mlp_forward(c, mlp, feat, C, M, s.mlp, s.fea, F);
  if (c.ok()) c.rc = hoisdf_token_build_fwd(cam, center, pe, s.fea, F, sdf, beta_ptr, tok, B, P, S, row0, D, stream);
  if (c.ok() && fea_out && hipMemcpyAsync(fea_out, s.fea, sizeof(float) * M * F, hipMemcpyDeviceToDevice, c.st) != hipSuccess) c.rc = HOISDF_ERR_LAUNCH;
  if (c.ok() && (sv.overflow || ws.overflow)) c.rc = HOISDF_ERR_WORKSPACE;
  if (c.rc == HOISDF_ERR_WORKSPACE) set_error("tokens_fwd: workspace (%ld bytes) too small", workspace_bytes);
  return c.rc;
}

extern "C" int hoisdf_tokens_bwd(const hoisdf_pyramid_grad* dpyr, const float* points, const float* center, const float* cam_intr, float scale,
                                 int img_h, int img_w, const float* feat_in, const hoisdf_mlp* mlp, const float* sdf, const float* beta_ptr,
                                 const float* dtok, const void* saved, long saved_bytes, const hoisdf_mlp_grads* grads, float* dfeat,
                                 int accumulate_dfeat, float* dbeta, int B, int P, int S, int row0, int D, void* workspace, long workspace_bytes,
                                 void* stream) {
  HOISDF_REQUIRE(mlp_ok(mlp) && grads_ok(mlp, grads) && sdf && beta_ptr && dtok && saved && dbeta && workspace, HOISDF_ERR_INVALID,
                 "tokens_bwd: null pointer (every weight-gradient buffer is required, zero-filled)");
  const bool gather = feat_in == nullptr;
  const long M = (long)B * P;
  HOISDF_REQUIRE(B > 0 && P > 0 && saved_bytes >= hoisdf_tokens_saved_bytes(mlp, M, gather), HOISDF_ERR_INVALID, "tokens_bwd: bad sizes / saved buffer");
  HOISDF_REQUIRE(gather ? (points && center && cam_intr) : true, HOISDF_ERR_INVALID, "tokens_bwd: the gather's arguments are needed again");
  Bump sv(const_cast<void*>(saved), saved_bytes), ws(workspace, workspace_bytes);
  TokSaved s; tok_carve(mlp, M, gather, sv, s);
  const int C = mlp->dims[0];
  float* df = dfeat;
  int acc = accumulate_dfeat;
  if (gather && dpyr && !df) {
    df = ws.floats(M * C); acc = 0;
    if (!df) { set_error("tokens_bwd: workspace too small"); return HOISDF_ERR_WORKSPACE; }
  }
  int rc = tokens_backward(mlp, grads, gather ? s.feat : feat_in, M, s, dtok, sdf, beta_ptr, df, acc, dbeta, B, P, S, row0, D, ws, false, stream);
  if (rc == HOISDF_OK && gather && dpyr && df)
    rc = hoisdf_project_gather_bwd(dpyr, points, nullptr, M, P, center, cam_intr, scale, img_h, img_w, df, C, stream);
  return rc;
}

extern "C" long hoisdf_heads_vote_saved_bytes(const hoisdf_mlp* vote, const hoisdf_mlp* cls, int L, int B, int P, int J) {
  if (!mlp_ok(vote) || !mlp_ok(cls) || L <= 0 || B <= 0 || P <= 0 || J <= 0) return 0;
  Bump b(nullptr, 0); VoteSaved s;
  vote_carve(vote, cls, (long)L * B * P, L * B, J, b, s);
  return b.off + 256;
}

static int heads_vote_backward(const hoisdf_mlp* mv, const hoisdf_mlp* mc, const hoisdf_mlp_grads* Gv, const hoisdf_mlp_grads* Gc, const float* enc,
                               const float* pts, const float* gt, float radius, const float* joints, VoteSaved& s, const float* djoints,
                               const float* dl3d, const float* dbce, float* denc, int L, int B, int P, int J, Bump& ws, bool dry, void* stream) {
  Ctx c{as_stream(stream), stream, &ws, dry, gemm_emu_mode()};
  const long M = (long)L * B * P;
  float* doff = ws.floats(M * 3 * J); float* dcls = ws.floats(M * J);
  if (!dry) {
    if (!doff || !dcls) { set_error("heads_vote_bwd: workspace too small"); return HOISDF_ERR_WORKSPACE; }
    c.rc = hoisdf_vote_loss_bwd(s.off, s.cls, pts, gt, radius, joints, s.stats, djoints, dl3d, dbce, doff, dcls, L, B, P, J, stream);
  }
  const int E = mv->dims[0];
  mlp_backward(c, mv, Gv, enc, E, M, s.vote, doff, 3 * J, denc, E, 0);
  mlp_backward(c, mc, Gc, enc, E, M, s.cl, dcls, J, denc, E, 1, enc_mag(c, mv, enc, E, M, s.vote));
  if (c.ok() && !dry && ws.overflow) { set_error("heads_vote_bwd: workspace too small"); return HOISDF_ERR_WORKSPACE; }
  return c.rc;
}

extern "C" long hoisdf_heads_vote_workspace_bytes(const hoisdf_mlp* vote, const hoisdf_mlp* cls, int L, int B, int P, int J, int backward_pass) {
  if (!mlp_ok(vote) || !mlp_ok(cls) || L <= 0 || B <= 0 || P <= 0 || J <= 0) return 0;
  const long M = (long)L * B * P;
  Bump ws(nullptr, 0), sv(nullptr, 0);
  VoteSaved s; vote_carve(vote, cls, M, L * B, J, sv, s);
  if (backward_pass) {
    hoisdf_mlp_grads G{};
    (void)heads_vote_backward(vote, cls, &G, &G, nullptr, nullptr, nullptr, 0.f, nullptr, s, nullptr, nullptr, nullptr, reinterpret_cast<float*>(1), L, B, P, J, ws,
                              true, nullptr);
  } else {
    Ctx c{nullptr, nullptr, &ws, true, gemm_emu_mode()};
    mlp_forward(c, vote, nullptr, vote->dims[0], M, s.vote, nullptr, 3 * J);
    mlp_forward(c, cls, nullptr, cls->dims[0], M, s.cl, nullptr, J);
  }
  return ws.off + 256;
}

extern "C" int hoisdf_heads_vote_fwd(const float* enc, const hoisdf_mlp* vote, const hoisdf_mlp* cls, const float* pts, const float* joint_gt_mm,
                                     float radius, float* joints, float* l3d_sum, float* bce_sum, float* near_sum, int L, int B, int P, int J,
                                     void* saved, long saved_bytes, void* workspace, long workspace_bytes, void* stream) {
  HOISDF_REQUIRE(enc && mlp_ok(vote) && mlp_ok(cls) && pts && joint_gt_mm && joints && l3d_sum && bce_sum && near_sum && saved && workspace,
                 HOISDF_ERR_INVALID, "heads_vote_fwd: null pointer / bad MLP");
  HOISDF_REQUIRE(L > 0 && B > 0 && P > 0 && J > 0 && vote->dims[vote->n_layers] == 3 * J && cls->dims[cls->n_layers] == J &&
                     vote->dims[0] == cls->dims[0] && !vote->act_last && !cls->act_last,
                 HOISDF_ERR_INVALID, "heads_vote_fwd: the vote MLP must end in 3 J = %d, the class MLP in J = %d plain columns", 3 * J, J);
  HOISDF_REQUIRE(saved_bytes >= hoisdf_heads_vote_saved_bytes(vote, cls, L, B, P, J), HOISDF_ERR_WORKSPACE, "heads_vote_fwd: saved buffer too small");
  const long M = (long)L * B * P;
  Bump sv(saved, saved_bytes), ws(workspace, workspace_bytes);
  VoteSaved s; vote_carve(vote, cls, M, L * B, J, sv, s);
  Ctx c{as_stream(stream), stream, &ws, false, gemm_emu_mode()};
  const int E = vote->dims[0];
  mlp_forward(c, vote, enc, E, M, s.vote, s.off, 3 * J);
  mlp_forward(c, cls, enc, E, M, s.cl, s.cls, J, enc_mag(c, vote, enc, E, M, s.vote));
  if (c.ok()) c.rc = hoisdf_vote_loss_fwd(s.off, s.cls, pts, joint_gt_mm, radius, joints, s.stats, l3d_sum, bce_sum, near_sum, L, B, P, J, stream);
  if (c.ok() && (sv.overflow || ws.overflow)) c.rc = HOISDF_ERR_WORKSPACE;
  if (c.rc == HOISDF_ERR_WORKSPACE) set_error("heads_vote_fwd: workspace (%ld bytes) too small", workspace_bytes);
  return c.rc;
}

extern "C" int hoisdf_heads_vote_bwd(const float* enc, const hoisdf_mlp* vote, const hoisdf_mlp* cls, const float* pts, const float* joint_gt_mm,
                                     float radius, const float* joints, const void* saved, long saved_bytes, const float* djoints,
                                     const float* dl3d_sum, const float* dbce_sum, const hoisdf_mlp_grads* vote_grads,
                                     const hoisdf_mlp_grads* cls_grads, float* denc, int L, int B, int P, int J, void* workspace,
                                     long workspace_bytes, void* stream) {
  HOISDF_REQUIRE(enc && mlp_ok(vote) && mlp_ok(cls) && grads_ok(vote, vote_grads) && grads_ok(cls, cls_grads) && pts && joint_gt_mm && joints && saved &&
                     denc && workspace,
                 HOISDF_ERR_INVALID, "heads_vote_bwd: null pointer (every weight-gradient buffer is required, zero-filled)");
  HOISDF_REQUIRE(L > 0 && B > 0 && P > 0 && J > 0 && saved_bytes >= hoisdf_heads_vote_saved_bytes(vote, cls, L, B, P, J), HOISDF_ERR_INVALID,
                 "heads_vote_bwd: bad sizes / saved buffer");
  Bump sv(const_cast<void*>(saved), saved_bytes), ws(workspace, workspace_bytes);
  VoteSaved s; vote_carve(vote, cls, (long)L * B * P, L * B, J, sv, s);
  return heads_vote_backward(vote, cls, vote_grads, cls_grads, enc, pts, joint_gt_mm, radius, joints, s, djoints, dl3d_sum, dbce_sum, denc, L, B, P, J, ws, false,
                             stream);
}
```

hoisdf_amd/csrc/layers.hip:

```cpp
#include <stdlib.h>

#include <mutex>
#include <unordered_map>

#include "chain.h"

namespace hoisdf {
namespace {

__global__ void rows_copy_add_kernel(float* __restrict__ dst, long dst_gs, const float* __restrict__ src, long src_gs, int rows, int E4,
                                     long total, int add) {
  const long i = (long)blockIdx.x * blockDim.x + threadIdx.x;
  if (i >= total) return;
  const long per = (long)rows * E4;
  const long g = i / per, r = i - g * per;
  float4* d = reinterpret_cast<float4*>(dst + g * dst_gs) + r;
  const float4 s = reinterpret_cast<const float4*>(src + g * src_gs)[r];
  if (add) { float4 t = *d; t.x += s.x; t.y += s.y; t.z += s.z; t.w += s.w; *d = t; }
  else *d = s;
}
int rows_copy_add(float* dst, long dst_gs, const float* src, long src_gs, int groups, int rows, int E, int add, hipStream_t st) {
  const long total = (long)groups * rows * (E / 4);
  if (total == 0) return HOISDF_OK;
  hipLaunchKernelGGL(rows_copy_add_kernel, dim3((unsigned)cdiv(total, 256)), dim3(256), 0, st, dst, dst_gs, src, src_gs, rows, E / 4, total, add);
// ... 31 lines not shown
  HOISDF_REQUIRE(d->drop_p >= 0.f && d->drop_p < 1.f, HOISDF_ERR_INVALID, "encoder_layer: drop_p=%f", d->drop_p);
  HOISDF_REQUIRE(d->attention == 0 || d->attention == 2, HOISDF_ERR_INVALID, "encoder_layer: attention must be 0 (exact f32) or 2 (emulated fp32)");
  g.B = d->B; g.S = d->S; g.E = d->E; g.F = d->F; g.H = d->H;
  g.nq = (d->n_query <= 0 || d->n_query >= d->S) ? d->S : d->n_query;
  g.ni = (d->n_inter <= 0 || d->n_inter >= g.nq) ? g.nq : d->n_inter;
  g.full = g.nq == g.S;
  g.M = (long)g.B * g.nq; g.Ms = (long)g.B * g.S;
  g.eps = d->eps; g.p = d->drop_p;
  g.att = g.nq < 32 ? 0 : d->attention;
  g.att_bwd_emu = g.att == 2 && d->attention_bwd_emulated && d->training;
  g.att_h2 = attn_h2_enabled() && g.att == 2 && g.E == g.H * 64 && gemm_emu_mode() && emu_form_h2() && g.M >= EMU_MIN_ROWS;
  g.fused_qkv = !g.att_h2 && g.att == 2 && (g.att_bwd_emu || !d->training) && g.E == g.H * 64 && g.S % 128 == 0 &&
                g.nq % 128 == 0 && gemm_emu_mode() && g.M >= EMU_MIN_ROWS;
  return HOISDF_OK;
}

struct Saved {
  float* qkv; float* qbuf; float* kvbuf; float* xq; float* o; float* lse; float* a; float* x1; float* h; uint32_t* bits; float* f; float* st;
  void* planes; long planes_bytes;
  uint32_t* mag; long mag_bytes;
};
enum { MAG_O = 0, MAG_X1 = 1, MAG_H = 2, MAG_XOUT = 3, MAG_ROWS = 4 };
void carve_saved(const Geo& g, Bump& b, Saved& s) {
  const int E = g.E;
  s.qkv = s.qbuf = s.kvbuf = s.xq = nullptr;
  if (g.full) { if (!g.fused_qkv) s.qkv = b.floats(g.Ms * 3 * E); }
  else {
    if (!g.fused_qkv) { s.qbuf = b.floats(g.M * E); s.kvbuf = b.floats(g.Ms * 2 * E); }
    s.xq = b.floats(g.M * E);
  }
  s.o = b.floats(g.M * E); s.lse = b.floats((long)g.B * g.H * g.nq); s.a = b.floats(g.M * E); s.x1 = b.floats(g.M * E);
  s.h = b.floats(g.M * g.F); s.bits = static_cast<uint32_t*>(b.take(g.M * ((g.F + 31) / 32) * 4)); s.f = b.floats(g.M * E);
  s.st = b.floats(6 * g.M);
  s.planes_bytes = g.att_bwd_emu ? hoisdf_attention_emu_workspace(g.B, g.H, g.nq, g.S, 2) : 0;
  s.planes = s.planes_bytes ? b.take(s.planes_bytes) : nullptr;
  s.mag_bytes = ((long)MAG_ROWS * g.M + 3L * g.H * g.B) * 4;
  s.mag = static_cast<uint32_t*>(b.take(s.mag_bytes));
}
uint32_t* head_q(const Geo& g, uint32_t* mag) { return mag ? mag + (long)MAG_ROWS * g.M : nullptr; }
uint32_t* head_k(const Geo& g, uint32_t* mag) { return mag ? head_q(g, mag) + (long)g.H * g.B : nullptr; }
uint32_t* head_v(const Geo& g, uint32_t* mag) { return mag ? head_q(g, mag) + 2L * g.H * g.B : nullptr; }
bool layer_mags(const Ctx& c, const Geo& g) { return c.emu && emu_form_h2() && g.M >= EMU_MIN_ROWS; }

int forward(const float* x, const hoisdf_encoder_layer_weights* w, const hoisdf_encoder_layer_desc* d, const Geo& g, float* x_out, float* y_out,
            Bump& saved, Bump& ws, bool dry, void* stream) {
  Ctx c{as_stream(stream), stream, &ws, dry, gemm_emu_mode()};
  Saved s;
  carve_saved(g, d->training ? saved : ws, s);
  const int E = g.E, F = g.F;
  const float *q = nullptr, *k = nullptr, *v = nullptr; int ldq = 0, ldkv = 0;
  const float* xq2 = x;
  void* aw = s.planes; long ab = s.planes_bytes;
  if (g.att == 2 && !aw) { ab = hoisdf_attention_emu_workspace(g.B, g.H, g.nq, g.S, 0); aw = ws.take(ab); }
  const bool mags = layer_mags(c, g) && (dry || s.mag);
  auto mg = [&](int i) -> uint32_t* { return mags && s.mag ? s.mag + (long)i * g.M : nullptr; };
  uint32_t* const smag = mags ? s.mag : nullptr;
  const uint32_t* xm = mags ? d->x_mag : nullptr;
  if (mags && !dry && c.ok() && hipMemsetAsync(s.mag, 0, (size_t)s.mag_bytes, c.st) != hipSuccess) c.rc = HOISDF_ERR_LAUNCH;
  if (g.fused_qkv) {
    QkvPlanes pq{}, pkv{};
    const void* im = nullptr; const void* im_q = nullptr; const void* im_kv = nullptr;
    if (g.full) im = image_of(c, w->img_in, w->w_in, E, 3 * E, E, 0);
    else {
      if (!dry && c.ok()) c.rc = rows_copy_add(s.xq, (long)g.nq * E, x, (long)g.S * E, g.B, g.nq, E, 0, c.st);
      xq2 = s.xq;
      im_q = image_of(c, w->img_in_q, w->w_in, E, E, E, 0);
      im_kv = image_of(c, w->img_in_kv, w->w_in + (size_t)E * E, E, 2 * E, E, 0);
    }
    if (!dry && c.ok()) {
      if (!aw) c.rc = HOISDF_ERR_WORKSPACE;
      else {
        attention_emu_plane_targets(aw, g.B, g.H, g.nq, g.S, s.planes ? 1 : 0, pq, pkv);
        if (g.full) c.rc = linear_fwd_emu_qkv(x, E, im, w->b_in, g.Ms, 3 * E, E, pq, stream, xm);
        else {
          c.rc = linear_fwd_emu_qkv(s.xq, E, im_q, w->b_in, g.M, E, E, pq, stream, nullptr);
          pkv.col0 = E;
          if (c.ok()) c.rc = linear_fwd_emu_qkv(x, E, im_kv, w->b_in ? w->b_in + E : nullptr, g.Ms, 2 * E, E, pkv, stream, xm);
        }
      }
    }
  } else if (g.full) {
    lin_fwd(c, x, E, w->w_in, E, w->img_in, w->b_in, s.qkv, 3 * E, g.Ms, 3 * E, E, 0, 0.f, 0, nullptr, 0, xm, nullptr,
            g.att_h2 ? head_q(g, smag) : nullptr, g.S);
    q = s.qkv; k = s.qkv + E; v = s.qkv + 2 * E; ldq = ldkv = 3 * E;
  } else {
    if (!dry && c.ok()) c.rc = rows_copy_add(s.xq, (long)g.nq * E, x, (long)g.S * E, g.B, g.nq, E, 0, c.st);
    xq2 = s.xq;
    lin_fwd(c, s.xq, E, w->w_in, E, w->img_in_q, w->b_in, s.qbuf, E, g.M, E, E, 0, 0.f, 0, nullptr, 0, nullptr, nullptr,
            g.att_h2 ? head_q(g, smag) : nullptr, g.nq);
    lin_fwd(c, x, E, w->w_in + (size_t)E * E, E, w->img_in_kv, w->b_in ? w->b_in + E : nullptr, s.kvbuf, 2 * E, g.Ms, 2 * E, E, 0, 0.f, 0, nullptr, 0, xm, nullptr,
            g.att_h2 ? head_k(g, smag) : nullptr, g.S);
    q = s.qbuf; k = s.kvbuf; v = s.kvbuf + E; ldq = E; ldkv = 2 * E;
  }
  const uint32_t* o_mag = g.att == 2 ? mg(MAG_O) : nullptr;
  if (g.fused_qkv) {
    if (!dry && c.ok())
      c.rc = attention_fwd_emu_planes(s.o, E, s.lse, g.B, g.H, g.nq, g.S, g.S, g.p, d->seed[0], aw, s.planes ? 1 : 0, stream, mg(MAG_O));
  } else if (g.att == 2) {
    if (!dry && c.ok()) {
      if (!aw) c.rc = HOISDF_ERR_WORKSPACE;
      else {
        const bool hm = g.att_h2 && smag;
        c.rc = attention_fwd_emu_mag(q, ldq, k, ldkv, v, ldkv, s.o, E, s.lse, g.B, g.H, g.nq, g.S, g.S, g.p, d->seed[0], aw, ab,
                                     s.planes ? 1 : 0, mg(MAG_O), stream, hm ? head_q(g, smag) : nullptr, hm ? head_k(g, smag) : nullptr,
                                     hm ? head_v(g, smag) : nullptr);
      }
    }
  } else if (!dry && c.ok()) {
    c.rc = hoisdf_attention_fwd(q, ldq, k, ldkv, v, ldkv, s.o, E, s.lse, g.B, g.H, g.nq, g.S, g.S, g.p, d->seed[0], stream);
  }
  lin_fwd(c, s.o, E, w->w_out, E, w->img_out, w->b_out, s.a, E, g.M, E, E, 0, 0.f, 0, nullptr, 0, o_mag, nullptr);
  float* st = s.st;
  if (!dry && c.ok()) c.rc = add_layernorm_fwd_mag(xq2, s.a, w->g1, w->be1, s.x1, st, st + g.M, g.M, E, g.eps, g.p, d->seed[1], mg(MAG_X1), stream);
  lin_fwd(c, s.x1, E, w->w1, E, w->img_1, w->b1, s.h, F, g.M, F, E, 1, g.p, d->seed[2], s.bits, 0, mg(MAG_X1), mg(MAG_H));
  lin_fwd(c, s.h, F, w->w2, F, w->img_2, w->b2, s.f, E, g.M, E, F, 0, 0.f, 0, nullptr, 0, mg(MAG_H), nullptr);
  if (!dry && c.ok()) c.rc = add_layernorm_fwd_mag(s.x1, s.f, w->g2, w->be2, x_out, st + 2 * g.M, st + 3 * g.M, g.M, E, g.eps, g.p, d->seed[3], mg(MAG_XOUT), stream);
  if (w->g3 && !dry && c.ok()) {
    if (g.ni == g.nq) c.rc = hoisdf_add_layernorm_fwd(x_out, nullptr, w->g3, w->be3, y_out, st + 4 * g.M, st + 5 * g.M, g.M, E, g.eps, 0.f, 0, stream);
    else c.rc = hoisdf_layernorm_rows_fwd(x_out, w->g3, w->be3, y_out, st + 4 * g.M, st + 5 * g.M, g.B, g.nq, g.ni, E, g.eps, stream);
  }
  if (c.ok() && !dry && (ws.overflow || saved.overflow)) { set_error("encoder_layer_fwd: workspace / saved buffer too small"); return HOISDF_ERR_WORKSPACE; }
  return c.rc;
}

int backward(const float* x, const float* x_out, const hoisdf_encoder_layer_weights* w, const hoisdf_encoder_layer_desc* d, const Geo& g,
             Bump& saved, const float* g_x_out, const float* g_y, float* dx, const hoisdf_encoder_layer_grads* G, Bump& ws, bool dry,
             void* stream, bool fwd_mags = true) {
  Ctx c{as_stream(stream), stream, &ws, dry, gemm_emu_mode()};
  Saved s;
  carve_saved(g, saved, s);
  const int E = g.E, F = g.F;
  const long M = g.M, Ms = g.Ms;
  const float* st = s.st;
  const float* dx2 = g_x_out;
  if (g_y && w->g3) {
    float* t = ws.floats(M * E);
    if (!dry && c.ok()) {
      if (!t) c.rc = HOISDF_ERR_WORKSPACE;
      else if (g.ni == g.nq) c.rc = hoisdf_add_layernorm_bwd(g_y, x_out, nullptr, w->g3, st + 4 * M, st + 5 * M, g_x_out, t, nullptr, G->dg3, G->dbe3, M, E, 0.f, 0, stream);
      else c.rc = hoisdf_layernorm_rows_bwd(g_y, x_out, w->g3, st + 4 * M, st + 5 * M, g_x_out, t, G->dg3, G->dbe3, g.B, g.nq, g.ni, E, stream);
    }
    dx2 = t;
  }
  float* dx1 = ws.floats(M * E); float* df = ws.floats(M * E); float* dh = ws.floats(M * F);
  float* dxq = g.full ? dx : ws.floats(M * E);
  float* da = ws.floats(M * E); float* dO = ws.floats(M * E);
  float* delta = ws.floats((long)g.B * g.H * g.nq);
  if (!dry && (!dx1 || !df || !dh || !dxq || !da || !dO || !delta)) { set_error("encoder_layer_bwd: workspace too small"); return HOISDF_ERR_WORKSPACE; }
  if (!dry && !dx2) { set_error("encoder_layer_bwd: no upstream gradient (g_x_out and g_y both null)"); return HOISDF_ERR_INVALID; }
  enum { MAG_DF = 0, MAG_DH = 1, MAG_DA = 2, MAG_BROWS = 3 };
  const long bmag_bytes = ((long)MAG_BROWS * M + Ms + (long)g.H * g.B) * 4;
  uint32_t* bmag = static_cast<uint32_t*>(ws.take(bmag_bytes));
  const bool mags = layer_mags(c, g) && (dry || bmag);
  auto mg = [&](int i) -> uint32_t* { return mags && bmag ? bmag + (long)i * M : nullptr; };
  uint32_t* const mag_dqkv = mags && bmag ? bmag + (long)MAG_BROWS * M : nullptr;
  uint32_t* const head_do = mags && bmag ? bmag + (long)MAG_BROWS * M + Ms : nullptr;
  auto fm = [&](int i) -> const uint32_t* { return mags && fwd_mags && s.mag ? s.mag + (long)i * M : nullptr; };
  uint32_t* const smag = mags && fwd_mags ? s.mag : nullptr;
  if (mags && !dry && c.ok() && hipMemsetAsync(bmag, 0, (size_t)bmag_bytes, c.st) != hipSuccess) c.rc = HOISDF_ERR_LAUNCH;
  if (!dry && c.ok()) c.rc = add_layernorm_bwd_mag(dx2, s.x1, s.f, w->g2, st + 2 * M, st + 3 * M, nullptr, dx1, df, G->dg2, G->dbe2, M, E, g.p, d->seed[3], nullptr, mg(MAG_DF), stream);
  lin_bwd_input(c, df, E, nullptr, 0.f, w->w2, F, w->img_t_2, dh, F, M, E, F, 0, mg(MAG_DF), mg(MAG_DH));
  lin_bwd_weight(c, df, E, nullptr, 0.f, s.h, F, G->dw2, G->db2, M, E, F, 0, mg(MAG_DF), fm(MAG_H));
  lin_bwd_input(c, dh, F, s.bits, g.p, w->w1, E, w->img_t_1, dx1, E, M, F, E, 1, mg(MAG_DH), nullptr);
  lin_bwd_weight(c, dh, F, s.bits, g.p, s.x1, E, G->dw1, G->db1, M, F, E, 0, mg(MAG_DH), fm(MAG_X1));
  const float* xq2 = g.full ? x : s.xq;
  if (!dry && c.ok()) c.rc = add_layernorm_bwd_mag(dx1, xq2, s.a, w->g1, st, st + M, nullptr, dxq, da, G->dg1, G->dbe1, M, E, g.p, d->seed[1], nullptr, mg(MAG_DA), stream);
  lin_bwd_input(c, da, E, nullptr, 0.f, w->w_out, E, w->img_t_out, dO, E, M, E, E, 0, mg(MAG_DA), nullptr, g.att_h2 ? head_do : nullptr, g.nq);
  lin_bwd_weight(c, da, E, nullptr, 0.f, s.o, E, G->dw_out, G->db_out, M, E, E, 0, mg(MAG_DA), g.att == 2 ? fm(MAG_O) : nullptr);
  const bool amag = mags && g.att_bwd_emu && g.full;
  auto attn_bwd = [&](const float* q, int ldq, const float* k, const float* v, int ldkv, float* dq, float* dk, float* dv) {
    if (g.att_bwd_emu) {
      const long ab = hoisdf_attention_bwd_emu_workspace(g.B, g.H, g.nq, g.S, s.planes ? 1 : 0);
      void* aw = ws.take(ab);
      if (dry || !c.ok()) return;
      if (!aw) { c.rc = HOISDF_ERR_WORKSPACE; return; }
      const bool hm = g.att_h2 && smag && head_do;
      if (g.att_h2 && !hm) { set_error("encoder_layer_bwd: the forward ran the f16x2 attention but the head magnitudes are not available"); c.rc = HOISDF_ERR_INVALID; return; }
      c.rc = attention_bwd_emu_mag(q, ldq, k, ldkv, v, ldkv, s.o, E, dO, E, s.lse, delta, dq, dk, dv, g.B, g.H, g.nq, g.S, g.S, g.p, d->seed[0],
                                   s.planes, aw, ab, amag ? mag_dqkv : nullptr, stream, hm ? head_q(g, smag) : nullptr,
                                   hm ? head_k(g, smag) : nullptr, hm ? head_v(g, smag) : nullptr, hm ? head_do : nullptr);
    } else if (!dry && c.ok()) {
      c.rc = hoisdf_attention_bwd(q, ldq, k, ldkv, v, ldkv, s.o, E, dO, E, s.lse, delta, dq, dk, dv, g.B, g.H, g.nq, g.S, g.S, g.p, d->seed[0], stream);
    }
  };
  if (g.full) {
    float* dqkv = ws.floats(Ms * 3 * E);
    if (!dry && !dqkv) { set_error("encoder_layer_bwd: workspace too small"); return HOISDF_ERR_WORKSPACE; }
    if (g.fused_qkv) attn_bwd(nullptr, 3 * E, nullptr, nullptr, 3 * E, dqkv, dqkv + E, dqkv + 2 * E);
    else attn_bwd(s.qkv, 3 * E, s.qkv + E, s.qkv + 2 * E, 3 * E, dqkv, dqkv + E, dqkv + 2 * E);
    lin_bwd_input(c, dqkv, 3 * E, nullptr, 0.f, w->w_in, E, w->img_t_in, dxq, E, Ms, 3 * E, E, 1, amag ? mag_dqkv : nullptr, nullptr);
    lin_bwd_weight(c, dqkv, 3 * E, nullptr, 0.f, x, E, G->dw_in, G->db_in, Ms, 3 * E, E, 0, amag ? mag_dqkv : nullptr, amag ? d->x_mag : nullptr);
  } else {
    float* dq = ws.floats(M * E); float* dkv = ws.floats(Ms * 2 * E);
    if (!dry && (!dq || !dkv)) { set_error("encoder_layer_bwd: workspace too small"); return HOISDF_ERR_WORKSPACE; }
    if (g.fused_qkv) attn_bwd(nullptr, E, nullptr, nullptr, 2 * E, dq, dkv, dkv + E);
    else attn_bwd(s.qbuf, E, s.kvbuf, s.kvbuf + E, 2 * E, dq, dkv, dkv + E);
    lin_bwd_input(c, dq, E, nullptr, 0.f, w->w_in, E, w->img_t_in_q, dxq, E, M, E, E, 1);
    lin_bwd_weight(c, dq, E, nullptr, 0.f, s.xq, E, G->dw_in, G->db_in, M, E, E);
    lin_bwd_input(c, dkv, 2 * E, nullptr, 0.f, w->w_in + (size_t)E * E, E, w->img_t_in_kv, dx, E, Ms, 2 * E, E, 0);
    lin_bwd_weight(c, dkv, 2 * E, nullptr, 0.f, x, E, G->dw_in + (size_t)E * E, G->db_in ? G->db_in + E : nullptr, Ms, 2 * E, E);
    if (!dry && c.ok()) c.rc = rows_copy_add(dx, (long)g.S * E, dxq, (long)g.nq * E, g.B, g.nq, E, 1, c.st);
  }
  if (c.ok() && !dry && ws.overflow) { set_error("encoder_layer_bwd: workspace too small"); return HOISDF_ERR_WORKSPACE; }
  return c.rc;
}

}
}

using namespace hoisdf;

extern "C" long hoisdf_encoder_layer_saved_bytes(const hoisdf_encoder_layer_desc* d) {
  Geo g;
  if (geometry(d, g) != HOISDF_OK) return -1;
  Bump b(nullptr, 0); Saved s;
  carve_saved(g, b, s);
  return b.off + 256;
}

extern "C" const uint32_t* hoisdf_encoder_layer_out_mag(const hoisdf_encoder_layer_desc* d, const void* saved) {
  Geo g;
  if (!saved || geometry(d, g) != HOISDF_OK || !d->training) return nullptr;
  Ctx c{nullptr, nullptr, nullptr, false, gemm_emu_mode()};
  if (!layer_mags(c, g)) return nullptr;
  Bump b(const_cast<void*>(saved), 1L << 62); Saved s;
  carve_saved(g, b, s);
  return s.mag ? s.mag + (long)MAG_XOUT * g.M : nullptr;
}

extern "C" long hoisdf_encoder_layer_workspace_bytes(const hoisdf_encoder_layer_desc* d, int backward_pass) {
  Geo g;
  if (geometry(d, g) != HOISDF_OK) return -1;
  hoisdf_encoder_layer_weights w{};
  hoisdf_encoder_layer_grads G{};
  float dummy = 0.f;
  w.g3 = &dummy;
  Bump saved(nullptr, 0), ws(nullptr, 0);
  if (backward_pass) (void)backward(nullptr, nullptr, &w, d, g, saved, &dummy, &dummy, nullptr, &G, ws, true, nullptr);
  else (void)forward(nullptr, &w, d, g, nullptr, nullptr, saved, ws, true, nullptr);
  return ws.off + 256;
}

extern "C" int hoisdf_encoder_layer_fwd(const float* x, const hoisdf_encoder_layer_weights* w, const hoisdf_encoder_layer_desc* d, float* x_out,
                                        float* y_out, void* saved, long saved_bytes, void* workspace, long workspace_bytes, void* stream) {
  Geo g;
  if (int rc = geometry(d, g)) return rc;
  HOISDF_REQUIRE(x && w && x_out && w->w_in && w->w_out && w->w1 && w->w2 && w->g1 && w->be1 && w->g2 && w->be2, HOISDF_ERR_INVALID,
                 "encoder_layer_fwd: null pointer");
  HOISDF_REQUIRE(!w->g3 || (w->be3 && y_out), HOISDF_ERR_INVALID, "encoder_layer_fwd: inter_norm needs be3 and y_out");
  HOISDF_REQUIRE(!d->training || saved, HOISDF_ERR_WORKSPACE, "encoder_layer_fwd: training needs the saved buffer (hoisdf_encoder_layer_saved_bytes)");
  HOISDF_REQUIRE(workspace || workspace_bytes == 0, HOISDF_ERR_WORKSPACE, "encoder_layer_fwd: null workspace");
  HOISDF_REQUIRE(al16(x) && al16(x_out) && al16(saved) && al16(workspace), HOISDF_ERR_INVALID, "encoder_layer_fwd: buffers must be 16-byte aligned");
  Bump sv(saved, saved_bytes), ws(workspace, workspace_bytes);
  static char none;
  if (!sv.base) { sv.base = &none; sv.cap = 0; }
  if (!ws.base) { ws.base = &none; ws.cap = 0; }
  if (d->training) {
    Ctx c0{nullptr, nullptr, nullptr, false, gemm_emu_mode()};
    saved_forms().put(saved, (g.fused_qkv ? 1 : 0) | (g.att_h2 ? 2 : 0) | (layer_mags(c0, g) ? 4 : 0));
  }
  const int rc = forward(x, w, d, g, x_out, y_out, sv, ws, false, stream);
  if (rc == HOISDF_ERR_WORKSPACE) set_error("encoder_layer_fwd: workspace (%ld bytes) or saved buffer (%ld bytes) too small", workspace_bytes, saved_bytes);
  return rc;
}

extern "C" int hoisdf_encoder_layer_bwd(const float* x, const float* x_out, const hoisdf_encoder_layer_weights* w, const hoisdf_encoder_layer_desc* d,
                                        const void* saved, long saved_bytes, const float* g_x_out, const float* g_y, float* dx,
                                        const hoisdf_encoder_layer_grads* grads, void* workspace, long workspace_bytes, void* stream) {
  Geo g;
  if (int rc = geometry(d, g)) return rc;
  HOISDF_REQUIRE(x && x_out && w && saved && dx && grads && workspace, HOISDF_ERR_INVALID, "encoder_layer_bwd: null pointer");
  HOISDF_REQUIRE(grads->dw_in && grads->db_in && grads->dw_out && grads->db_out && grads->dg1 && grads->dbe1 && grads->dw1 && grads->db1 &&
                     grads->dw2 && grads->db2 && grads->dg2 && grads->dbe2 && (!w->g3 || !g_y || (grads->dg3 && grads->dbe3)),
                 HOISDF_ERR_INVALID, "encoder_layer_bwd: every parameter gradient buffer is required (zero-filled)");
  HOISDF_REQUIRE(d->training, HOISDF_ERR_INVALID, "encoder_layer_bwd: the forward call must have run with training = 1");
  HOISDF_REQUIRE(al16(x) && al16(dx) && al16(saved) && al16(workspace), HOISDF_ERR_INVALID, "encoder_layer_bwd: buffers must be 16-byte aligned");
  const int recorded = saved_forms().take(saved);
  if (recorded >= 0) { g.fused_qkv = (recorded & 1) != 0; g.att_h2 = (recorded & 2) != 0; }
  const bool fwd_mags = recorded < 0 || (recorded & 4) != 0;
  Bump sv(const_cast<void*>(saved), saved_bytes), ws(workspace, workspace_bytes);
  const int rc = backward(x, x_out, w, d, g, sv, g_x_out, g_y, dx, grads, ws, false, stream, fwd_mags);
  if (rc == HOISDF_OK && sv.overflow) { set_error("encoder_layer_bwd: saved buffer too small"); return HOISDF_ERR_WORKSPACE; }
  if (rc == HOISDF_ERR_WORKSPACE) set_error("encoder_layer_bwd: workspace (%ld bytes) too small", workspace_bytes);
  return rc;
}

namespace hoisdf {
namespace {

__global__ void add_bcast_kernel(float* __restrict__ out, const float* __restrict__ a, const float* __restrict__ p, int rows_p, int E4, long total) {
  const long i = (long)blockIdx.x * blockDim.x + threadIdx.x;
  if (i >= total) return;
  const long per = (long)rows_p * E4;
  const float4 x = reinterpret_cast<const float4*>(a)[i], y = reinterpret_cast<const float4*>(p)[i % per];
  reinterpret_cast<float4*>(out)[i] = make_float4(x.x + y.x, x.y + y.y, x.z + y.z, x.w + y.w);
}
__global__ void sum_bcast_grad_kernel(float* __restrict__ dp, const float* __restrict__ g1, const float* __restrict__ g2, int B, int rows_p, int E4) {
  const int i = blockIdx.x * blockDim.x + threadIdx.x;
  if (i >= rows_p * E4) return;
  float4 acc = reinterpret_cast<float4*>(dp)[i];
  for (int b = 0; b < B; ++b) {
    const float4 x = reinterpret_cast<const float4*>(g1)[(long)b * rows_p * E4 + i], y = reinterpret_cast<const float4*>(g2)[(long)b * rows_p * E4 + i];
    acc.x += x.x + y.x; acc.y += x.y + y.y; acc.z += x.z + y.z; acc.w += x.w + y.w;
  }
  reinterpret_cast<float4*>(dp)[i] = acc;
}

struct DGeo { int B, Q, S, E, F, H, kv; long M, Ms; float eps, p; };
int dgeometry(const hoisdf_decoder_layer_desc* d, DGeo& g) {
  HOISDF_REQUIRE(d, HOISDF_ERR_INVALID, "decoder_layer: null descriptor");
  HOISDF_REQUIRE(d->B > 0 && d->Q > 0 && d->Q <= 64 && d->S > 0 && d->E > 0 && d->F > 0 && d->H > 0 && d->E % d->H == 0 && d->E % 4 == 0 &&
                     d->F % 4 == 0 && d->kv_len > 0 && d->kv_len <= d->S,
                 HOISDF_ERR_INVALID, "decoder_layer: bad sizes B=%d Q=%d S=%d E=%d F=%d H=%d kv_len=%d", d->B, d->Q, d->S, d->E, d->F, d->H, d->kv_len);
  HOISDF_REQUIRE(d->drop_p >= 0.f && d->drop_p < 1.f, HOISDF_ERR_INVALID, "decoder_layer: drop_p=%f", d->drop_p);
  g.B = d->B; g.Q = d->Q; g.S = d->S; g.E = d->E; g.F = d->F; g.H = d->H; g.kv = d->kv_len;
  g.M = (long)d->B * d->Q; g.Ms = (long)d->B * d->S; g.eps = d->eps; g.p = d->drop_p;
  return HOISDF_OK;
}
struct DSaved {
  float *tq1, *qk, *v, *probs, *o1, *a1, *x1, *tq2, *q2, *kv, *o2, *lse2, *a2, *x2, *h, *f, *st; uint32_t* bits;
};
void dcarve(const DGeo& g, Bump& b, DSaved& s) {
  const long M = g.M; const int E = g.E;
  s.tq1 = b.floats(M * E); s.qk = b.floats(M * 2 * E); s.v = b.floats(M * E); s.probs = b.floats((long)g.B * g.H * g.Q * g.Q);
  s.o1 = b.floats(M * E); s.a1 = b.floats(M * E); s.x1 = b.floats(M * E); s.tq2 = b.floats(M * E); s.q2 = b.floats(M * E);
  s.kv = b.floats(g.Ms * 2 * E); s.o2 = b.floats(M * E); s.lse2 = b.floats((long)g.B * g.H * g.Q); s.a2 = b.floats(M * E);
  s.x2 = b.floats(M * E); s.h = b.floats(M * g.F); s.bits = static_cast<uint32_t*>(b.take(M * ((g.F + 31) / 32) * 4)); s.f = b.floats(M * E);
  s.st = b.floats(8 * M);
}
int add_bcast(float* out, const float* a, const float* p, const DGeo& g, hipStream_t st) {
  const long total = g.M * (g.E / 4);
  hipLaunchKernelGGL(add_bcast_kernel, dim3((unsigned)cdiv(total, 256)), dim3(256), 0, st, out, a, p, g.Q, g.E / 4, total);
  return check_launch("decoder_layer add");
}

int dforward(const float* tgt, const float* memory, const float* qpos, const uint8_t* mask, const hoisdf_decoder_layer_weights* w,
             const hoisdf_decoder_layer_desc* d, const DGeo& g, float* out, float* y_out, Bump& saved, Bump& ws, bool dry, void* stream) {
  Ctx c{as_stream(stream), stream, &ws, dry, gemm_emu_mode()};
  DSaved s;
  dcarve(g, d->training ? saved : ws, s);
  const int E = g.E, F = g.F;
  const long M = g.M;
  float* st = s.st;
  if (!dry && c.ok()) c.rc = add_bcast(s.tq1, tgt, qpos, g, c.st);
  lin_fwd(c, s.tq1, E, w->sa_w_in, E, nullptr, w->sa_b_in, s.qk, 2 * E, M, 2 * E, E, 0, 0.f, 0, nullptr);
  lin_fwd(c, tgt, E, w->sa_w_in + (size_t)2 * E * E, E, nullptr, w->sa_b_in ? w->sa_b_in + 2 * E : nullptr, s.v, E, M, E, E, 0, 0.f, 0, nullptr);
  if (!dry && c.ok())
    c.rc = hoisdf_attention_small_fwd(s.qk, 2 * E, s.qk + E, 2 * E, s.v, E, mask, s.o1, E, s.probs, g.B, g.H, g.Q, g.Q, g.p, d->seed[0], stream);
  lin_fwd(c, s.o1, E, w->sa_w_out, E, nullptr, w->sa_b_out, s.a1, E, M, E, E, 0, 0.f, 0, nullptr);
  if (!dry && c.ok()) c.rc = hoisdf_add_layernorm_fwd(tgt, s.a1, w->g1, w->be1, s.x1, st, st + M, M, E, g.eps, g.p, d->seed[1], stream);
  if (!dry && c.ok()) c.rc = add_bcast(s.tq2, s.x1, qpos, g, c.st);
  lin_fwd(c, s.tq2, E, w->ca_w_in, E, nullptr, w->ca_b_in, s.q2, E, M, E, E, 0, 0.f, 0, nullptr);
  lin_fwd(c, memory, E, w->ca_w_in + (size_t)E * E, E, w->img_ca_kv, w->ca_b_in ? w->ca_b_in + E : nullptr, s.kv, 2 * E, g.Ms, 2 * E, E, 0, 0.f, 0, nullptr);
  if (!dry && c.ok())
    c.rc = hoisdf_attention_fwd(s.q2, E, s.kv, 2 * E, s.kv + E, 2 * E, s.o2, E, s.lse2, g.B, g.H, g.Q, g.S, g.kv, g.p, d->seed[2], stream);
// ... 145 lines not shown
```

hoisdf_amd/csrc/sdf_query.hip:

```cpp
#include "common.h"

using namespace hoisdf;

namespace {
constexpr int HID0 = 512, LAT = 256, PF = 33, H1 = 223, X0 = LAT + PF, CAT_K = 516, X0_COL = 224;
constexpr int CAT_LD = 544;
inline long align64(long v) { return (v + 63) / 64 * 64; }
constexpr long EMU_MIN_ROWS_Q = 2048;

inline long emu_scratch_bytes(int C) {
  const long a = hoisdf_linear_emu_image_bytes(HID0, C), b = hoisdf_linear_emu_image_bytes(HID0, CAT_K);
  return ((a > b ? a : b) + 255) / 256 * 256;
}

int layer(const float* x, int ldx, const float* W, int ldw, const float* b, float* y, int ldy, long M, int N, int K,
          int K_pad, float drop_p, uint64_t seed, void* emu_img, const void* given, void* stream, const uint32_t* x_mag = nullptr,
          uint32_t* y_mag = nullptr, bool* y_has = nullptr) {
  if (y_has) *y_has = false;
  if (emu_img && M >= EMU_MIN_ROWS_Q && hoisdf_linear_emu_supported(x, ldx, K_pad) && (K_pad + 15) / 16 == (K + 15) / 16) {
    if (!given) { if (int rc = hoisdf_linear_emu_prepare(W, ldw, N, K, 0, emu_img, stream)) return rc; }
    if (y_has) *y_has = y_mag != nullptr;
    return linear_fwd_emu_mag(x, ldx, given ? given : emu_img, b, y, ldy, M, N, K_pad, 1, drop_p, seed, nullptr, x_mag, y_mag, stream);
  }
  return hoisdf_linear_fwd(x, ldx, W, ldw, b, y, ldy, M, N, K, 1, drop_p, seed, nullptr, stream);
// ... 85 lines not shown
  return HOISDF_OK;
}

extern "C" int hoisdf_sdf_infer_count(const float* center, const float* cam_intr, const float* bbox, float scale, int bins_n, int B,
                                      int32_t* counts_device, int32_t* counts_host, long* n_rows, void* stream) {
  HOISDF_REQUIRE(n_rows, HOISDF_ERR_INVALID, "sdf_infer_count: bad arguments");
  if (int rc = hoisdf_sdf_infer_count_begin(center, cam_intr, bbox, scale, bins_n, B, counts_device, counts_host, stream)) return rc;
  if (hipStreamSynchronize(as_stream(stream)) != hipSuccess) {
    set_error("sdf_infer_count: reading the counts back failed: %s", hipGetErrorString(hipGetLastError()));
    return HOISDF_ERR_LAUNCH;
  }
  long n = 0;
  for (int b = 0; b < B; ++b) n += counts_host[b];
  *n_rows = n;
  return HOISDF_OK;
}

namespace hoisdf {
__global__ __launch_bounds__(64) void exclusive_scan_counts_kernel(const int32_t* __restrict__ counts, int B, int32_t* __restrict__ offsets) {
  const int lane = threadIdx.x;
  int carry = 0;
  for (int base = 0; base < B; base += 64) {
    const int b = base + lane;
    const int c = b < B ? counts[b] : 0;
    int incl = c;
#pragma unroll
    for (int o = 1; o < 64; o <<= 1) {
      const int up = __shfl_up(incl, o, 64);
      if (lane >= o) incl += up;
    }
    if (b < B) offsets[b] = carry + incl - c;
    carry += __shfl(incl, 63, 64);
  }
}
}

extern "C" long hoisdf_sdf_infer_workspace(long n_rows, int B, int C) {
  if (n_rows < 0 || B <= 0 || C <= 0) return -1;
  return up256(4L * B) + up256(12 * n_rows) + 2 * up256(4 * n_rows) + 2 * up256(4 * n_rows) + up256(120 * n_rows) + up256(4 * n_rows) +
         up256(hoisdf_sdf_query_workspace(n_rows, C, 1)) + 256;
}

extern "C" int hoisdf_sdf_infer(const hoisdf_pyramid* pyr, const float* center, const float* cam_intr, const float* bbox, float scale,
                                int bins_n, int B, const int32_t* counts_device, const int32_t* counts_host, int num_points, int img_h,
                                int img_w, const hoisdf_sdf_weights* w, float clamp, float drop_p, uint64_t seed, float* points_out,
                                float* sdf_out, float* pe_out, void* workspace, long workspace_bytes, void* stream) {
  HOISDF_REQUIRE(pyr && center && cam_intr && bbox && counts_device && counts_host && w && points_out && sdf_out && workspace && B > 0 &&
                     num_points > 0,
                 HOISDF_ERR_INVALID, "sdf_infer: bad arguments");
  long n = 0;
  for (int b = 0; b < B; ++b) {
    HOISDF_REQUIRE(counts_host[b] >= num_points, HOISDF_ERR_INVALID,
                   "sdf_infer: sample %d has only %d lattice points inside its bbox, fewer than num_points=%d", b, counts_host[b], num_points);
    n += counts_host[b];
  }
  const long need = hoisdf_sdf_infer_workspace(n, B, w->C);
  HOISDF_REQUIRE(workspace_bytes >= need, HOISDF_ERR_WORKSPACE, "sdf_infer: workspace of %ld bytes, need %ld", workspace_bytes, need);
  char* p = static_cast<char*>(workspace);
  auto take = [&](long bytes) { char* r = p; p += up256(bytes); return r; };
  int32_t* offsets = reinterpret_cast<int32_t*>(take(4L * B));
  float* pts = reinterpret_cast<float*>(take(12 * n));
  int32_t* sidx = reinterpret_cast<int32_t*>(take(4 * n));
  int32_t* lidx = reinterpret_cast<int32_t*>(take(4 * n));
  float* sdf = reinterpret_cast<float*>(take(4 * n));
  float* raw = reinterpret_cast<float*>(take(4 * n));
  float* pe = reinterpret_cast<float*>(take(120 * n));
  int32_t* sel = reinterpret_cast<int32_t*>(take(4L * B * num_points));
  const long qbytes = hoisdf_sdf_query_workspace(n, w->C, 1);
  void* qws = take(0);
  hipStream_t st = as_stream(stream);
  hipLaunchKernelGGL(exclusive_scan_counts_kernel, dim3(1), dim3(64), 0, st, counts_device, B, offsets);
  if (int rc0 = check_launch("sdf_infer offsets")) return rc0;
  int rc = hoisdf_lattice_fill(center, cam_intr, bbox, scale, bins_n, B, offsets, pts, sidx, lidx, stream);
  if (rc) return rc;
  rc = hoisdf_sdf_query_fwd(pyr, pts, sidx, n, 1, center, cam_intr, scale, img_h, img_w, nullptr, nullptr, w, clamp, drop_p, seed, sdf, raw, pe,
                            nullptr, qws, qbytes, stream);
  if (rc) return rc;
  rc = hoisdf_select_smallest_abs(raw, offsets, counts_device, B, num_points, sel, stream);
  if (rc) return rc;
  const long ns = (long)B * num_points;
  rc = hoisdf_gather_rows(pts, 3, sel, ns, 3, points_out, 3, stream);
  if (rc) return rc;
  rc = hoisdf_gather_rows(sdf, 1, sel, ns, 1, sdf_out, 1, stream);
  if (rc) return rc;
  if (pe_out) rc = hoisdf_gather_rows(pe, 30, sel, ns, 30, pe_out, 30, stream);
  return rc;
}

#include "chain.h"

namespace {
struct TrainSaved { float *feat, *ha, *cat, *h0, *h2, *h3, *raw; uint32_t *ba, *bf, *b0, *b1, *b2, *b3; uint32_t* mag; };
enum { TM_FEAT = 0, TM_HA = 1, TM_CAT = 2, TM_H0 = 3, TM_H2 = 4, TM_N = 5 };
inline bool train_mags(const Ctx& c, long n) { return c.emu && emu_form_h2() && n >= EMU_MIN_ROWS; }
inline long bits_words(int N) { return (N + 31) / 32; }
void train_carve(long n, int C, Bump& b, TrainSaved& s) {
  s.feat = b.floats(n * C); s.ha = b.floats(n * HID0); s.cat = b.floats(n * CAT_LD); s.h0 = b.floats(n * HID0); s.h2 = b.floats(n * HID0);
  s.h3 = b.floats(n * HID0); s.raw = b.floats(n);
  s.ba = static_cast<uint32_t*>(b.take(n * bits_words(HID0) * 4)); s.bf = static_cast<uint32_t*>(b.take(n * bits_words(LAT) * 4));
  s.b0 = static_cast<uint32_t*>(b.take(n * bits_words(HID0) * 4)); s.b1 = static_cast<uint32_t*>(b.take(n * bits_words(H1 + 1) * 4));
  s.b2 = static_cast<uint32_t*>(b.take(n * bits_words(HID0) * 4)); s.b3 = static_cast<uint32_t*>(b.take(n * bits_words(HID0) * 4));
  s.mag = static_cast<uint32_t*>(b.take((long)TM_N * n * 4));
}
}

extern "C" long hoisdf_sdf_query_train_saved_bytes(long n_rows, int C) {
  if (n_rows <= 0 || C <= 0) return 0;
  Bump b(nullptr, 0); TrainSaved s;
  train_carve(n_rows, C, b, s);
  return b.off + 256;
}

static int sdf_train_forward(const hoisdf_pyramid* pyr, const float* points, const int32_t* sample_idx, long n, int rps, const float* center,
                             const float* cam_intr, float scale, int img_h, int img_w, const hoisdf_sdf_weights* w, float clamp, float drop_p,
                             uint64_t seed, float* sdf, float* pe, float* cam_out, Bump& saved, Bump& ws, bool dry, void* stream) {
  Ctx c{as_stream(stream), stream, &ws, dry, gemm_emu_mode()};
  TrainSaved s;
  const int C = w ? w->C : 1;
  train_carve(n, C, saved, s);
  const bool mags = train_mags(c, n) && !dry && s.mag;
  if (!dry) saved_mags().put(s.mag, mags);
  auto mg = [&](int i) -> uint32_t* { return mags ? s.mag + (long)i * n : nullptr; };
  if (!dry) {
    if (mags) c.rc = hipMemsetAsync(s.mag, 0, (size_t)TM_N * n * 4, c.st) == hipSuccess ? HOISDF_OK : HOISDF_ERR_LAUNCH;
    if (c.ok()) c.rc = project_gather_fwd_mag(pyr, points, sample_idx, n, rps, center, cam_intr, scale, img_h, img_w, s.feat, C, cam_out, nullptr, mg(TM_FEAT), stream);
    if (c.ok()) c.rc = hipMemsetAsync(s.cat, 0, sizeof(float) * n * CAT_LD, c.st) == hipSuccess ? HOISDF_OK : HOISDF_ERR_LAUNCH;
  }
  float* x0 = dry ? nullptr : s.cat + X0_COL;
  lin_fwd(c, s.feat, C, w->sdfin_w0, C, w->emu_img[0], w->sdfin_b0, s.ha, HID0, n, HID0, C, 1, 0.f, 0, s.ba, 0, mg(TM_FEAT), mg(TM_HA));
  lin_fwd(c, s.ha, HID0, w->sdfin_w1, HID0, w->emu_img[1], w->sdfin_b1, x0, CAT_LD, n, LAT, HID0, 1, 0.f, 0, s.bf, 0, mg(TM_HA), mg(TM_CAT));
  if (!dry && c.ok()) c.rc = posenc_fwd_mag(points, n, s.cat, CAT_LD, X0_COL + LAT, pe, mg(TM_CAT), stream);
  lin_fwd(c, x0, CAT_LD, w->dec_w0, w->dec_ld0, w->emu_img[2], w->dec_b0, s.h0, HID0, n, HID0, X0, 1, drop_p, seed, s.b0, X0 + 3, mg(TM_CAT), mg(TM_H0));
  lin_fwd(c, s.h0, HID0, w->dec_w1, HID0, w->emu_img[3], w->dec_b1, s.cat, CAT_LD, n, H1 + 1, HID0, 1, drop_p, seed + 1, s.b1, 0, mg(TM_H0), mg(TM_CAT));
  lin_fwd(c, s.cat, CAT_LD, w->dec_w2, CAT_K, w->emu_img[4], w->dec_b2, s.h2, HID0, n, HID0, CAT_K, 1, drop_p, seed + 2, s.b2, 0, mg(TM_CAT), mg(TM_H2));
  lin_fwd(c, s.h2, HID0, w->dec_w3, HID0, w->emu_img[5], w->dec_b3, s.h3, HID0, n, HID0, HID0, 1, drop_p, seed + 3, s.b3, 0, mg(TM_H2), nullptr);
  if (!dry && c.ok()) c.rc = hoisdf_sdf_head_fwd(s.h3, HID0, w->dec_w4, w->dec_b4, s.raw, sdf, n, HID0, clamp, stream);
  return c.rc;
}

static int sdf_train_backward(const hoisdf_pyramid_grad* dpyr, const float* points, const int32_t* sample_idx, long n, int rps, const float* center,
                              const float* cam_intr, float scale, int img_h, int img_w, const hoisdf_sdf_weights* w, float clamp, float drop_p,
                              const float* d_sdf, const hoisdf_sdf_weight_grads* G, Bump& saved, Bump& ws, bool dry, void* stream) {
  Ctx c{as_stream(stream), stream, &ws, dry, gemm_emu_mode()};
  TrainSaved s;
  const int C = w ? w->C : 1;
  train_carve(n, C, saved, s);
  float* dh3 = ws.floats(n * HID0); float* dh2 = ws.floats(n * HID0); float* dcat = ws.floats(n * CAT_LD); float* dh0 = ws.floats(n * HID0);
  float* dha = ws.floats(n * HID0); float* dfeat = ws.floats(n * (long)C);
  if (!dry && (!dh3 || !dh2 || !dcat || !dh0 || !dha || !dfeat)) { set_error("sdf_query_bwd: workspace too small"); return HOISDF_ERR_WORKSPACE; }
  enum { BM_DH3 = 0, BM_DH2 = 1, BM_DCAT = 2, BM_DH0 = 3, BM_DHA = 4, BM_N = 5 };
  uint32_t* bmag = static_cast<uint32_t*>(ws.take((long)BM_N * n * 4));
  const bool mags = train_mags(c, n) && !dry && bmag && s.mag;
  const bool fmags = mags && saved_mags().get(s.mag) != 0;
  auto mg = [&](int i) -> uint32_t* { return mags ? bmag + (long)i * n : nullptr; };
  auto fm = [&](int i) -> const uint32_t* { return fmags ? s.mag + (long)i * n : nullptr; };
  if (mags) c.rc = hipMemsetAsync(bmag, 0, (size_t)BM_N * n * 4, c.st) == hipSuccess ? HOISDF_OK : HOISDF_ERR_LAUNCH;
  if (!dry && c.ok()) c.rc = sdf_head_bwd_mag(d_sdf, s.raw, s.h3, HID0, w->dec_w4, dh3, HID0, G->d_dec_w4, G->d_dec_b4, n, HID0, clamp, mg(BM_DH3), stream);
  lin_bwd_input(c, dh3, HID0, s.b3, drop_p, w->dec_w3, HID0, w->emu_img_t[5], dh2, HID0, n, HID0, HID0, 0, mg(BM_DH3), mg(BM_DH2));
  lin_bwd_weight(c, dh3, HID0, s.b3, drop_p, s.h2, HID0, G->d_dec_w3, G->d_dec_b3, n, HID0, HID0, 0, mg(BM_DH3), fm(TM_H2));
  lin_bwd_input(c, dh2, HID0, s.b2, drop_p, w->dec_w2, CAT_K, w->emu_img_t[4], dcat, CAT_LD, n, HID0, CAT_K, 0, mg(BM_DH2), mg(BM_DCAT));
  lin_bwd_weight(c, dh2, HID0, s.b2, drop_p, s.cat, CAT_LD, G->d_dec_w2, G->d_dec_b2, n, HID0, CAT_K, 0, mg(BM_DH2), fm(TM_CAT));
  lin_bwd_input(c, dcat, CAT_LD, s.b1, drop_p, w->dec_w1, HID0, w->emu_img_t[3], dh0, HID0, n, H1 + 1, HID0, 0, mg(BM_DCAT), mg(BM_DH0));
  lin_bwd_weight(c, dcat, CAT_LD, s.b1, drop_p, s.h0, HID0, G->d_dec_w1, G->d_dec_b1, n, H1 + 1, HID0, 0, mg(BM_DCAT), fm(TM_H0));
  float* dx0 = dry ? nullptr : dcat + X0_COL;
  const float* x0 = dry ? nullptr : s.cat + X0_COL;
  lin_bwd_input(c, dh0, HID0, s.b0, drop_p, w->dec_w0, w->dec_ld0, w->emu_img_t[2], dx0, CAT_LD, n, HID0, X0, 1, mg(BM_DH0), nullptr);
  lin_bwd_weight(c, dh0, HID0, s.b0, drop_p, x0, CAT_LD, G->d_dec_w0, G->d_dec_b0, n, HID0, X0, X0 + 3, mg(BM_DH0), fm(TM_CAT));
  lin_bwd_input(c, dx0, CAT_LD, s.bf, 0.f, w->sdfin_w1, HID0, w->emu_img_t[1], dha, HID0, n, LAT, HID0, 0, nullptr, mg(BM_DHA));
  lin_bwd_weight(c, dx0, CAT_LD, s.bf, 0.f, s.ha, HID0, G->d_sdfin_w1, G->d_sdfin_b1, n, LAT, HID0, 0, nullptr, fm(TM_HA));
  lin_bwd_input(c, dha, HID0, s.ba, 0.f, w->sdfin_w0, C, w->emu_img_t[0], dfeat, C, n, HID0, C, 0, mg(BM_DHA), nullptr);
  lin_bwd_weight(c, dha, HID0, s.ba, 0.f, s.feat, C, G->d_sdfin_w0, G->d_sdfin_b0, n, HID0, C, 0, mg(BM_DHA), fm(TM_FEAT));
  if (!dry && c.ok() && dpyr)
    c.rc = hoisdf_project_gather_bwd(dpyr, points, sample_idx, n, rps, center, cam_intr, scale, img_h, img_w, dfeat, C, stream);
  if (c.ok() && !dry && ws.overflow) { set_error("sdf_query_bwd: workspace too small"); return HOISDF_ERR_WORKSPACE; }
  return c.rc;
}

extern "C" long hoisdf_sdf_query_train_workspace_bytes(long n_rows, int C, int backward_pass) {
  if (n_rows <= 0 || C <= 0) return 0;
  hoisdf_sdf_weights w{}; w.C = C; w.dec_ld0 = X0;
  hoisdf_sdf_weight_grads G{};
  Bump saved(nullptr, 0), ws(nullptr, 0);
  if (backward_pass) (void)sdf_train_backward(nullptr, nullptr, nullptr, n_rows, 1, nullptr, nullptr, 1.f, 1, 1, &w, 0.f, 0.f, nullptr, &G, saved, ws, true, nullptr);
  else (void)sdf_train_forward(nullptr, nullptr, nullptr, n_rows, 1, nullptr, nullptr, 1.f, 1, 1, &w, 0.f, 0.f, 0, nullptr, nullptr, nullptr, saved, ws, true, nullptr);
  return ws.off + 256;
}

extern "C" int hoisdf_sdf_query_train_fwd(const hoisdf_pyramid* pyr, const float* points, const int32_t* sample_idx, long n_rows, int rows_per_sample,
                                          const float* center, const float* cam_intr, float scale, int img_h, int img_w,
                                          const hoisdf_sdf_weights* w, float clamp, float drop_p, uint64_t seed, float* sdf, float* pe,
                                          float* cam_out, void* saved, long saved_bytes, void* workspace, long workspace_bytes, void* stream) {
  HOISDF_REQUIRE(pyr && points && w && sdf && saved && workspace && center && cam_intr, HOISDF_ERR_INVALID, "sdf_query_train_fwd: null pointer");
  HOISDF_REQUIRE(n_rows > 0 && n_rows < (1L << 31) && w->C > 0 && w->C % 4 == 0 && w->dec_ld0 >= X0, HOISDF_ERR_INVALID, "sdf_query_train_fwd: bad sizes");
  HOISDF_REQUIRE(drop_p >= 0.f && drop_p < 1.f, HOISDF_ERR_INVALID, "sdf_query_train_fwd: drop_p=%f", drop_p);
  HOISDF_REQUIRE(saved_bytes >= hoisdf_sdf_query_train_saved_bytes(n_rows, w->C), HOISDF_ERR_WORKSPACE, "sdf_query_train_fwd: saved buffer of %ld bytes, need %ld",
                 saved_bytes, hoisdf_sdf_query_train_saved_bytes(n_rows, w->C));
  Bump sv(saved, saved_bytes), ws(workspace, workspace_bytes);
  int rc = sdf_train_forward(pyr, points, sample_idx, n_rows, rows_per_sample, center, cam_intr, scale, img_h, img_w, w, clamp, drop_p, seed, sdf, pe, cam_out,
                             sv, ws, false, stream);
  if (rc == HOISDF_OK && (sv.overflow || ws.overflow)) rc = HOISDF_ERR_WORKSPACE;
  if (rc == HOISDF_ERR_WORKSPACE) set_error("sdf_query_train_fwd: workspace (%ld bytes) too small", workspace_bytes);
  return rc;
}

extern "C" int hoisdf_sdf_query_bwd(const hoisdf_pyramid_grad* dpyr, const float* points, const int32_t* sample_idx, long n_rows, int rows_per_sample,
                                    const float* center, const float* cam_intr, float scale, int img_h, int img_w, const hoisdf_sdf_weights* w,
                                    float clamp, float drop_p, const void* saved, long saved_bytes, const float* d_sdf,
                                    const hoisdf_sdf_weight_grads* grads, void* workspace, long workspace_bytes, void* stream) {
  HOISDF_REQUIRE(points && w && saved && d_sdf && grads && workspace && center && cam_intr, HOISDF_ERR_INVALID, "sdf_query_bwd: null pointer");
  HOISDF_REQUIRE(grads->d_sdfin_w0 && grads->d_sdfin_b0 && grads->d_sdfin_w1 && grads->d_sdfin_b1 && grads->d_dec_w0 && grads->d_dec_b0 && grads->d_dec_w1 &&
                     grads->d_dec_b1 && grads->d_dec_w2 && grads->d_dec_b2 && grads->d_dec_w3 && grads->d_dec_b3 && grads->d_dec_w4 && grads->d_dec_b4,
                 HOISDF_ERR_INVALID, "sdf_query_bwd: every weight gradient buffer is required (zero-filled)");
  HOISDF_REQUIRE(n_rows > 0 && n_rows < (1L << 31) && saved_bytes >= hoisdf_sdf_query_train_saved_bytes(n_rows, w->C), HOISDF_ERR_INVALID,
                 "sdf_query_bwd: bad sizes / saved buffer");
  Bump sv(const_cast<void*>(saved), saved_bytes), ws(workspace, workspace_bytes);
  int rc = sdf_train_backward(dpyr, points, sample_idx, n_rows, rows_per_sample, center, cam_intr, scale, img_h, img_w, w, clamp, drop_p, d_sdf, grads, sv, ws,
                              false, stream);
  if (rc == HOISDF_ERR_WORKSPACE) set_error("sdf_query_bwd: workspace (%ld bytes) too small", workspace_bytes);
  return rc;
}
```

include/hoisdf.h:

```cpp
#ifndef HOISDF_H_
#define HOISDF_H_

#include <stdint.h>

#ifdef __cplusplus
extern "C" {
#endif

#define HOISDF_VERSION_MAJOR 0
#define HOISDF_VERSION_MINOR 1

typedef enum hoisdf_status {
  HOISDF_OK = 0,
  HOISDF_ERR_INVALID = -1,
  HOISDF_ERR_LAUNCH = -2,
  HOISDF_ERR_TOO_FEW = -3,
  HOISDF_ERR_WORKSPACE = -4
} hoisdf_status;

#define HOISDF_MAX_LEVELS 8

typedef struct hoisdf_pyramid {
  int n_levels;
  int B;
  const float* data[HOISDF_MAX_LEVELS];
  int C[HOISDF_MAX_LEVELS];
  int H[HOISDF_MAX_LEVELS];
  int W[HOISDF_MAX_LEVELS];
} hoisdf_pyramid;

typedef struct hoisdf_pyramid_grad {
  int n_levels;
  int B;
  float* data[HOISDF_MAX_LEVELS];
  int C[HOISDF_MAX_LEVELS];
  int H[HOISDF_MAX_LEVELS];
  int W[HOISDF_MAX_LEVELS];
} hoisdf_pyramid_grad;

const char* hoisdf_version(void);
const char* hoisdf_last_error(void);
void hoisdf_set_deterministic(int on);
void hoisdf_set_gemm_emu(int on);
int hoisdf_get_gemm_emu(void);
int hoisdf_get_deterministic(void);

int hoisdf_project_gather_fwd(const hoisdf_pyramid* pyr, const float* points,
                              const int32_t* sample_idx, long n_rows, int rows_per_sample,
                              const float* center, const float* cam_intr, float scale,
                              int img_h, int img_w, float* feat, int ldf, float* cam_out,
                              float* uv_out, void* stream);
int hoisdf_project_gather_bwd(const hoisdf_pyramid_grad* dpyr, const float* points,
                              const int32_t* sample_idx, long n_rows, int rows_per_sample,
                              const float* center, const float* cam_intr, float scale,
                              int img_h, int img_w, const float* dfeat, int ldf, void* stream);

int hoisdf_linear_fwd(const float* x, int ldx, const float* W, int ldw, const float* bias,
                      float* y, int ldy, long M, int N, int K, int act, float drop_p,
                      uint64_t seed, uint32_t* relu_bits, void* stream);
int hoisdf_linear_bwd_input(const float* dy, int lddy, const uint32_t* relu_bits, float drop_p,
                            const float* W, int ldw, float* dx, int lddx, long M, int N, int K,
                            int accumulate ,
                            void* stream);
long hoisdf_linear_bwd_weight_workspace(long M, int N, int K);
int hoisdf_linear_bwd_weight(const float* dy, int lddy, const uint32_t* relu_bits, float drop_p,
                             const float* x, int ldx, float* dW, int lddw, float* db, long M, int N,
                             int K, float* workspace, long workspace_floats, void* stream);
long hoisdf_linear_emu_image_bytes(int rows, int K);
int hoisdf_linear_emu_prepare(const float* W, int ldw, int N, int K, int transpose, void* image, void* stream);
typedef struct hoisdf_emu_prep_item {
  const float* W;
  void* image;
  long first_block;
  int ldw, N, K, transpose;
} hoisdf_emu_prep_item;
long hoisdf_linear_emu_prepare_blocks(int N, int K, int transpose);
int hoisdf_linear_emu_prepare_batch(const hoisdf_emu_prep_item* d_items, int n, long total_blocks, void* stream);
int hoisdf_linear_emu_supported(const float* a, long lda, int contraction);
int hoisdf_linear_emu_pieces(void);
long hoisdf_mag_words(long rows);
int hoisdf_mag_measure(const float* x, long ldx, long M, int K, uint32_t* words, void* stream);
long hoisdf_head_mag_words(long M, int groups, int L);
int hoisdf_head_mag_measure(const float* x, long ldx, long M, int groups, int L, uint32_t* words, void* stream);
int hoisdf_linear_fwd_emu_heads(const float* x, int ldx, const void* w_image, const float* bias, float* y, int ldy, long M, int N,
                                int K, const uint32_t* x_mag, uint32_t* y_mag, uint32_t* y_heads, int L, void* stream);
int hoisdf_linear_bwd_input_emu_heads(const float* dy, int lddy, const void* wt_image, float* dx, int lddx, long M, int N, int K,
                                      const uint32_t* dy_mag, uint32_t* dx_mag, uint32_t* dx_heads, int L, void* stream);
int hoisdf_linear_fwd_emu_mag(const float* x, int ldx, const void* w_image, const float* bias, float* y, int ldy, long M, int N,
                              int K, int act, float drop_p, uint64_t seed, uint32_t* relu_bits, const uint32_t* x_mag,
                              uint32_t* y_mag, void* stream);
int hoisdf_linear_bwd_input_emu_mag(const float* dy, int lddy, const uint32_t* relu_bits, float drop_p, const void* wt_image,
                                    float* dx, int lddx, long M, int N, int K, int accumulate, const uint32_t* dy_mag,
                                    uint32_t* dx_mag, void* stream);
int hoisdf_linear_bwd_weight_emu_mag(const float* dy, int lddy, const uint32_t* relu_bits, float drop_p, const float* x, int ldx,
                                     float* dW, int lddw, float* db, long M, int N, int K, float* workspace, long workspace_floats,
                                     const uint32_t* dy_mag, const uint32_t* x_mag, void* stream);
int hoisdf_linear_fwd_emu(const float* x, int ldx, const void* w_image, const float* bias, float* y, int ldy, long M, int N,
                          int K, int act, float drop_p, uint64_t seed, uint32_t* relu_bits, void* stream);
int hoisdf_linear_bwd_input_emu(const float* dy, int lddy, const uint32_t* relu_bits, float drop_p, const void* wt_image,
                                float* dx, int lddx, long M, int N, int K, int accumulate, void* stream);
int hoisdf_linear_emu_small_max_rows(void);
int hoisdf_linear_emu_small_supported(const float* a, long lda, const float* W, long ldw, long M, int N, int K);
int hoisdf_linear_fwd_emu_small(const float* x, int ldx, const float* W, int ldw, const float* bias, float* y, int ldy, long M,
                                int N, int K, int act, float drop_p, uint64_t seed, uint32_t* relu_bits, void* stream);
int hoisdf_linear_bwd_input_emu_small(const float* dy, int lddy, const uint32_t* relu_bits, float drop_p, const float* W, int ldw,
                                      float* dx, int lddx, long M, int N, int K, int accumulate, void* stream);
int hoisdf_linear_bwd_weight_emu_small(const float* dy, int lddy, const uint32_t* relu_bits, float drop_p, const float* x, int ldx,
                                       float* dW, int lddw, float* db, long M, int N, int K, void* stream);
long hoisdf_linear_bwd_weight_emu_workspace(long M, int N, int K);
int hoisdf_linear_bwd_weight_emu(const float* dy, int lddy, const uint32_t* relu_bits, float drop_p, const float* x, int ldx,
                                 float* dW, int lddw, float* db, long M, int N, int K, float* workspace, long workspace_floats,
                                 void* stream);
int hoisdf_relu_dropout_bwd(const float* y, int ldy, const float* dy, int lddy, float* dpre,
                            int ldd, long M, int N, float drop_p, void* stream);

int hoisdf_posenc_fwd(const float* points, long n_rows, float* x0, int ldx0, int col0,
                      float* pe, void* stream);
int hoisdf_weightnorm_fwd(const float* v, const float* g, float* W, int ldw, float* norms,
                          int out, int in, void* stream);
int hoisdf_weightnorm_bwd(const float* v, const float* g, const float* dW, int ldw, float* dv,
                          float* dg, int out, int in, void* stream);
int hoisdf_sdf_head_fwd(const float* h, int ldh, const float* w, const float* b, float* sdf_raw,
                        float* sdf, long n_rows, int K, float clamp, void* stream);
int hoisdf_sdf_head_bwd(const float* dsdf, const float* sdf_raw, const float* h, int ldh,
                        const float* w, float* dh, int lddh, float* dw, float* db, long n_rows,
                        int K, float clamp, void* stream);

typedef struct hoisdf_sdf_weights {
  int C;
  const float *sdfin_w0, *sdfin_b0;
  const float *sdfin_w1, *sdfin_b1;
  const float *dec_w0, *dec_b0;
  int dec_ld0;
  const float *dec_w1, *dec_b1;
  const float *dec_w2, *dec_b2;
  const float *dec_w3, *dec_b3;
  const float *dec_w4, *dec_b4;
  const void* emu_img[6];
  const void* emu_img_t[6];
} hoisdf_sdf_weights;
long hoisdf_sdf_query_workspace(long n_rows, int C, int need_feat);
int hoisdf_sdf_query_fwd(const hoisdf_pyramid* pyr, const float* points, const int32_t* sample_idx, long n_rows,
                         int rows_per_sample, const float* center, const float* cam_intr, float scale, int img_h,
                         int img_w, const float* feat_in, float* feat_out, const hoisdf_sdf_weights* w, float clamp,
                         float drop_p, uint64_t seed, float* sdf, float* sdf_raw, float* pe, float* cam_out,
                         void* workspace, long workspace_bytes, void* stream);

int hoisdf_lattice_count(const float* center, const float* cam_intr, const float* bbox, float scale,
                         int bins_n, int B, int32_t* counts, void* stream);
int hoisdf_lattice_fill(const float* center, const float* cam_intr, const float* bbox, float scale,
                        int bins_n, int B, const int32_t* offsets, float* points,
                        int32_t* sample_idx, int32_t* lattice_idx, void* stream);
int hoisdf_select_smallest_abs(const float* sdf_raw, const int32_t* offsets, const int32_t* counts,
                               int B, int k, int32_t* sel, void* stream);
int hoisdf_gather_rows(const float* src, int lds, const int32_t* sel, long n_sel, int width,
                       float* out, int ldo, void* stream);
typedef struct hoisdf_sdf_weight_grads {
  float *d_sdfin_w0, *d_sdfin_b0, *d_sdfin_w1, *d_sdfin_b1;
  float *d_dec_w0, *d_dec_b0, *d_dec_w1, *d_dec_b1, *d_dec_w2, *d_dec_b2, *d_dec_w3, *d_dec_b3, *d_dec_w4, *d_dec_b4;
} hoisdf_sdf_weight_grads;
long hoisdf_sdf_query_train_saved_bytes(long n_rows, int C);
long hoisdf_sdf_query_train_workspace_bytes(long n_rows, int C, int backward_pass);
int hoisdf_sdf_query_train_fwd(const hoisdf_pyramid* pyr, const float* points, const int32_t* sample_idx, long n_rows,
                               int rows_per_sample, const float* center, const float* cam_intr, float scale, int img_h, int img_w,
                               const hoisdf_sdf_weights* w, float clamp, float drop_p, uint64_t seed, float* sdf, float* pe,
                               float* cam_out, void* saved, long saved_bytes, void* workspace, long workspace_bytes, void* stream);
int hoisdf_sdf_query_bwd(const hoisdf_pyramid_grad* dpyr, const float* points, const int32_t* sample_idx, long n_rows,
                         int rows_per_sample, const float* center, const float* cam_intr, float scale, int img_h, int img_w,
                         const hoisdf_sdf_weights* w, float clamp, float drop_p, const void* saved, long saved_bytes,
                         const float* d_sdf, const hoisdf_sdf_weight_grads* grads, void* workspace, long workspace_bytes,
                         void* stream);

int hoisdf_sdf_infer_count_begin(const float* center, const float* cam_intr, const float* bbox, float scale, int bins_n,
                                 int B, int32_t* counts_device, int32_t* counts_host, void* stream);
int hoisdf_sdf_infer_count(const float* center, const float* cam_intr, const float* bbox, float scale, int bins_n, int B,
                           int32_t* counts_device, int32_t* counts_host, long* n_rows, void* stream);
long hoisdf_sdf_infer_workspace(long n_rows, int B, int C);
int hoisdf_sdf_infer(const hoisdf_pyramid* pyr, const float* center, const float* cam_intr, const float* bbox, float scale,
                     int bins_n, int B, const int32_t* counts_device, const int32_t* counts_host, int num_points, int img_h,
                     int img_w, const hoisdf_sdf_weights* w, float clamp, float drop_p, uint64_t seed, float* points_out,
                     float* sdf_out, float* pe_out, void* workspace, long workspace_bytes, void* stream);

int hoisdf_sdf_sample_keys(const float* rows, int ld, const int64_t* seg_row0, const int32_t* seg_len,
                           const int32_t* seg_off, const int32_t* seg_col, int n_seg, int max_len, float dist,
                           uint64_t seed, float* keys, int32_t* eligible, void* stream);

int hoisdf_token_build_fwd(const float* cam, const float* center, const float* pe,
                           const float* feat, int ldfeat, const float* sdf, const float* beta_ptr,
                           float* tok, int B, int P, int S, int row0, int D, void* stream);
int hoisdf_token_build_bwd(const float* dtok, const float* feat, int ldfeat, const float* sdf,
                           const float* beta_ptr, float* dfeat, int lddfeat, float* dbeta, int B,
                           int P, int S, int row0, int D, void* stream);

int hoisdf_token_build_bwd_partials(void);
int hoisdf_token_build_bwd_ordered(const float* dtok, const float* feat, int ldfeat, const float* sdf, const float* beta_ptr,
                                   float* dfeat, int lddfeat, float* dbeta, float* partials, int B, int P, int S, int row0,
                                   int D, void* stream);

int hoisdf_attention_fwd(const float* q, int ldq, const float* k, int ldk, const float* v, int ldv,
                         float* o, int ldo, float* lse, int B, int H, int Lq, int Lk, int kv_len,
                         float drop_p, uint64_t seed, void* stream);
int hoisdf_attention_bwd(const float* q, int ldq, const float* k, int ldk, const float* v, int ldv,
                         const float* o, int ldo, const float* dout, int lddo, const float* lse,
                         float* delta, float* dq, float* dk, float* dv, int B, int H, int Lq, int Lk,
                         int kv_len, float drop_p, uint64_t seed, void* stream);
long hoisdf_attention_bf16x2_workspace(int B, int H, int Lq, int Lk);
int hoisdf_attention_fwd_bf16x2(const float* q, int ldq, const float* k, int ldk, const float* v, int ldv, float* o, int ldo,
                                int B, int H, int Lq, int Lk, int kv_len, void* workspace, long workspace_bytes, void* stream);

long hoisdf_attention_emu_workspace(int B, int H, int Lq, int Lk, int mode);
int hoisdf_attention_fwd_emu(const float* q, int ldq, const float* k, int ldk, const float* v, int ldv, float* o, int ldo,
                             float* lse, int B, int H, int Lq, int Lk, int kv_len, float drop_p, uint64_t seed, void* workspace,
                             long workspace_bytes, int keep, void* stream);
int hoisdf_attention_fwd_emu_mag(const float* q, int ldq, const float* k, int ldk, const float* v, int ldv, float* o, int ldo,
                                 float* lse, int B, int H, int Lq, int Lk, int kv_len, float drop_p, uint64_t seed, void* workspace,
                                 long workspace_bytes, int keep, const uint32_t* q_mag, const uint32_t* k_mag, const uint32_t* v_mag,
                                 uint32_t* o_mag, void* stream);
long hoisdf_attention_bwd_emu_workspace(int B, int H, int Lq, int Lk, int kept);
int hoisdf_attention_bwd_emu(const float* q, int ldq, const float* k, int ldk, const float* v, int ldv, const float* o, int ldo,
                             const float* dout, int lddo, const float* lse, float* delta, float* dq, float* dk, float* dv, int B,
                             int H, int Lq, int Lk, int kv_len, float drop_p, uint64_t seed, const void* fwd_workspace,
                             void* workspace, long workspace_bytes, void* stream);
int hoisdf_attention_bwd_emu_mag(const float* q, int ldq, const float* k, int ldk, const float* v, int ldv, const float* o, int ldo,
                                 const float* dout, int lddo, const float* lse, float* delta, float* dq, float* dk, float* dv, int B,
                                 int H, int Lq, int Lk, int kv_len, float drop_p, uint64_t seed, const void* fwd_workspace,
                                 void* workspace, long workspace_bytes, const uint32_t* q_mag, const uint32_t* k_mag,
                                 const uint32_t* v_mag, const uint32_t* do_mag, uint32_t* g_mag, void* stream);
int hoisdf_attention_small_fwd(const float* q, int ldq, const float* k, int ldk, const float* v,
                               int ldv, const uint8_t* mask, float* o, int ldo, float* probs, int B,
                               int H, int Lq, int Lk, float drop_p, uint64_t seed, void* stream);
int hoisdf_attention_small_bwd(const float* q, int ldq, const float* k, int ldk, const float* v,
                               int ldv, const float* probs, const float* dout, int lddo, float* dq,
                               float* dk, float* dv, int B, int H, int Lq, int Lk, float drop_p,
                               uint64_t seed, void* stream);

int hoisdf_add_layernorm_fwd(const float* x, const float* r, const float* gamma, const float* beta,
                             float* y, float* mean, float* rstd, long M, int D, float eps,
                             float drop_p, uint64_t seed, void* stream);
int hoisdf_add_layernorm_bwd(const float* dy, const float* x, const float* r, const float* gamma,
                             const float* mean, const float* rstd,
                             const float* dx_add ,
                             float* dx, float* dr, float* dgamma, float* dbeta, long M, int D, float drop_p,
                             uint64_t seed, void* stream);

int hoisdf_residual_dropout(const float* x, const float* r, float* y, long M, int D, float drop_p, uint64_t seed, void* stream);

int hoisdf_layernorm_rows_fwd(const float* x, const float* gamma, const float* beta, float* y, float* mean, float* rstd,
                              long groups, int rows_per_group, int take, int D, float eps, void* stream);
int hoisdf_layernorm_rows_bwd(const float* dy, const float* x, const float* gamma, const float* mean, const float* rstd,
// ... 354 lines not shown
```

Before: 445.3.

## Batch weight-gradient GEMMs into grouped persistent launches with a shared split-K reduce

Weight-gradient GEMMs in the f16x2 emulated path are no longer launched one by one. They are queued in a per-context list of up to eight and flushed at the end of each backward stage. The flush issues a grouped kernel whose unit table covers the tiles of all queued GEMMs, with a joint split-K plan and one combined reduction launch. This aims to cut launch count and fill the GPU better when single dW GEMMs are small. The cost is more workspace, deferred execution, and extra plumbing, including dry-run placeholder magnitude words so that workspace sizing sees the grouped path.

```diff
diff --git a/hoisdf_amd/csrc/chain.h b/hoisdf_amd/csrc/chain.h
--- a/hoisdf_amd/csrc/chain.h
+++ b/hoisdf_amd/csrc/chain.h
@@ -43,7 +43,11 @@
   bool emu;
   int rc = HOISDF_OK;
   bool ok() const { return rc == HOISDF_OK; }
+  hoisdf_dw_group_item dw[8];
+  int ndw = 0;
 };
+
+inline uint32_t* dry_words() { static uint32_t w; return &w; }
 
 inline bool emu_small(const Ctx& c, long M, const float* a, long lda, const float* W, long ldw, int N, int K) {
   if (!c.emu || M > hoisdf_linear_emu_small_max_rows() || N % 4 || K % 4 || lda % 4 || ldw % 4) return false;
@@ -91,6 +95,16 @@
   if (emu_small(c, M, dy, lddy, W, ldw, N, K)) { c.rc = hoisdf_linear_bwd_input_emu_small(dy, lddy, bits, p, W, ldw, dx, lddx, M, N, K, accumulate, c.stream); return; }
   c.rc = hoisdf_linear_bwd_input(dy, lddy, bits, p, W, ldw, dx, lddx, M, N, K, accumulate, c.stream);
 }
+void dw_flush(Ctx& c) {
+  const int n = c.ndw;
+  c.ndw = 0;
+  if (n == 0 || !c.ok()) return;
+  const long nws = hoisdf_linear_bwd_weight_emu_group_workspace(c.dw, n);
+  float* w = c.ws->floats(nws > 4 ? nws : 4);
+  if (c.dry) return;
+  if (!w) { c.rc = HOISDF_ERR_WORKSPACE; return; }
+  c.rc = hoisdf_linear_bwd_weight_emu_group(c.dw, n, w, nws, c.stream);
+}
 void lin_bwd_weight(Ctx& c, const float* dy, int lddy, const uint32_t* bits, float p, const float* x, int ldx, float* dW, float* db, long M,
                     int N, int K, int K_pad = 0, const uint32_t* dy_mag = nullptr, const uint32_t* x_mag = nullptr) {
   if (!c.ok()) return;
@@ -98,6 +112,12 @@
   if (K_pad < K) K_pad = K;
   const bool emu = c.emu && M >= EMU_DW_MIN_ROWS && (N < K ? N : K) >= 64 && N % 4 == 0 && K_pad % 4 == 0 && lddy % 4 == 0 && ldx % 4 == 0 &&
                    (c.dry || (al16(dy) && al16(x) && al16(dW)));
+  if (emu && (dy_mag || x_mag) && emu_form_h2() && K_pad > 128) {
+    if (c.ndw == 8) dw_flush(c);
+    if (!c.ok()) return;
+    c.dw[c.ndw++] = hoisdf_dw_group_item{dy, lddy, bits, p, x, ldx, dW, db, M, N, K_pad, c.dry ? nullptr : dy_mag, c.dry ? nullptr : x_mag};
+    return;
+  }
   if (emu) {
     const long nws = hoisdf_linear_bwd_weight_emu_workspace(M, N, K_pad);
     float* w = c.ws->floats(nws > 4 ? nws : 4);
diff --git a/hoisdf_amd/csrc/dw2h_body.inc b/hoisdf_amd/csrc/dw2h_body.inc
--- /dev/null
+++ b/hoisdf_amd/csrc/dw2h_body.inc
@@ -0,0 +1,95 @@
+  f16_saturate_on();
+  uint32_t am_dy = 0u, am_x = 0u;
+  for (int i = mbeg + (int)threadIdx.x; i < mend; i += NT) { am_dy = max(am_dy, g.dy_amax[i]); am_x = max(am_x, g.x_amax[i]); }
+  am_dy = block_max_u32(am_dy, red4);
+  __syncthreads();
+  am_x = block_max_u32(am_x, red4);
+
+  f32x16 acc[4][4];
+#pragma unroll
+  for (int i = 0; i < 4; ++i)
+#pragma unroll
+    for (int j = 0; j < 4; ++j)
+#pragma unroll
+      for (int r = 0; r < 16; ++r) acc[i][j][r] = 0.f;
+
+  DW2_STAGING_SETUP(A_U4)
+  uint32_t t0[4], t1[4];
+  const float sc = isA ? h2_scale(am_dy) : h2_scale(am_x);
+  f32x2 rp_, fu_;
+  f32x4 csum = {0.f, 0.f, 0.f, 0.f};
+#define DU1(j, pr)                                                                                                     \
+  do {                                                                                                                 \
+    f32x2 v_ = (j) < 2 ? f32x2{rvL[2 * (pr)][(j) & 1], rvL[2 * (pr) + 1][(j) & 1]} : f32x2{rvH[2 * (pr)][(j) & 1], rvH[2 * (pr) + 1][(j) & 1]}; \
+    if (MASK) {                                                                                                        \
+      if ((j) == 0) {                                                                                                  \
+        const uint32_t n0_ = ((rm[2 * (pr)] | notA) >> bsh) & 0xfu, n1_ = ((rm[2 * (pr) + 1] | notA) >> bsh) & 0xfu;   \
+        mpk = ((pr) == 0 ? 0u : mpk) | (n0_ << (8 * (pr))) | (n1_ << (8 * (pr) + 4));                                  \
+      }                                                                                                                \
+      float xa_, xb_;                                                              \
+      asm("v_and_b32 %0, %1, %2" : "=v"(xa_) : "v"(__builtin_amdgcn_sbfe((int)mpk, 8 * (pr) + (j), 1)), "v"(v_.x));    \
+      asm("v_and_b32 %0, %1, %2" : "=v"(xb_) : "v"(__builtin_amdgcn_sbfe((int)mpk, 8 * (pr) + 4 + (j), 1)), "v"(v_.y)); \
+      v_ = f32x2{xa_, xb_};                                                                                            \
+    }                                                                                                                  \
+    if (HASDB) csum[j] += v_.x + v_.y;                                                                                 \
+    v_ *= sc;                                                                                                          \
+    const f16x2 h_ = __builtin_convertvector(v_, f16x2);                       \
+    t0[pr] = __builtin_bit_cast(uint32_t, h_); rp_ = v_;                                                               \
+    fu_ = __builtin_convertvector(h_, f32x2);                                                                          \
+  } while (0)
+#define DU2(j, pr) do { f32x2 w_; PK_SUB(w_, rp_, fu_); t1[pr] = __builtin_bit_cast(uint32_t, __builtin_convertvector(w_, f16x2)); } while (0)
+#define DSTA(st, j, pl) (st)[wbase + ((j) ^ sw) + (pl) * 2 * DT] = ((pl) == 0 ? u32x4{t0[0], t0[1], t0[2], t0[3]} : u32x4{t1[0], t1[1], t1[2], t1[3]})
+#define DLA(st, p, i) __builtin_bit_cast(f16x8, (st)[aread + ((p) * 2 + kh) * DT + (i) * 32])
+#define DLB(st, p, j) __builtin_bit_cast(f16x8, (st)[bread + ((p) * 2 + kh) * DT + (j) * 32])
+#define M1(ax, bx, i, j, work) do { acc[i][j] = MFH(ax[i], bx[j], acc[i][j]); work; SB(); } while (0)
+#define MM(ax, bx) _Pragma("unroll") for (int i = 0; i < 4; ++i) _Pragma("unroll") for (int j = 0; j < 4; ++j) acc[i][j] = MFH(ax[i], bx[j], acc[i][j])
+#include "dw2h_phase.inc"
+#define DSTAGE_ALL(st)                                                                                                 \
+  do {                                                                                                                 \
+    _Pragma("unroll") for (int j = 0; j < 4; ++j) {                                                                    \
+      _Pragma("unroll") for (int pr = 0; pr < 4; ++pr) { DU1(j, pr); DU2(j, pr); }                                     \
+      DSTA(st, j, 0); DSTA(st, j, 1);                                                                                  \
+    }                                                                                                                  \
+  } while (0)
+
+  const int nslab2 = (max(nslab, 1) + 1) & ~1;
+  f16x8 aH[4], aL[4], bP[4], bQ[4], bL[4];
+  DLOAD_ALL(0);
+  DLOADM_ALL(0);
+  DSTAGE_ALL(s0);
+  DLOAD_ALL(1);
+  DLOADM_ALL(1);
+  __syncthreads();
+#pragma unroll
+  for (int i = 0; i < 4; ++i) { aL[i] = DLA(s0, 1, i); aH[i] = DLA(s0, 0, i); }
+#pragma unroll
+  for (int j = 0; j < 4; ++j) { bP[j] = DLB(s0, 0, j); bL[j] = DLB(s0, 1, j); }
+  MM(aL, bP); MM(aH, bL);
+  DSTAGE_ALL(s1);
+  DLOAD_ALL(2);
+  DLOADM_ALL(2);
+  SYNC();
+  for (int s = 1; s + 1 < nslab2; s += 2) {
+    DHPHASE(s1, s0, s, bP, bQ);
+    SYNC();
+    DHPHASE(s0, s1, s + 1, bQ, bP);
+    SYNC();
+  }
+  DHPHASE(s1, s0, nslab2 - 1, bP, bQ);
+  SB();
+  MM(aH, bQ);
+  __syncthreads();
+#undef DU1
+#undef DU2
+#undef DSTA
+#undef DLA
+#undef DLB
+#undef M1
+#undef MM
+#undef DHPHASE
+#undef DSTAGE_ALL
+  const float unscale = h2_inv_scale(am_dy) * h2_inv_scale(am_x);
+  const float post = MASK ? g.ascale : 1.f;
+  u32x4* lds = lds_all;
+  DW2_STORE_COLSUM();
+  DW_EPILOGUE(DT, acc[i][j][r] * (MASK ? post * unscale : unscale));
diff --git a/hoisdf_amd/csrc/gemm_emu.h b/hoisdf_amd/csrc/gemm_emu.h
--- a/hoisdf_amd/csrc/gemm_emu.h
+++ b/hoisdf_amd/csrc/gemm_emu.h
@@ -62,6 +62,19 @@
   int M, N, K;
   int splitk, m_per_split, tiles_n, tiles_k;
   const uint32_t* dy_amax; const uint32_t* x_amax;
+};
+
+constexpr int DW_GROUP_MAX = 8;
+struct DwGroup {
+  DwArgs it[DW_GROUP_MAX];
+  int first[DW_GROUP_MAX + 1];
+  int n, unit0;
+};
+constexpr int DW_REDUCE_MAX = 2 * DW_GROUP_MAX;
+struct DwReduce {
+  struct Out { const float* part; long stride; float* out; long n; int splits; } o[DW_REDUCE_MAX];
+  int first_block[DW_REDUCE_MAX + 1];
+  int n;
 };
 
 __device__ __forceinline__ uint32_t h2_exp(uint32_t amax_bits) { return mag_exp(amax_bits); }
@@ -353,4 +366,8 @@
 int dw_tile(int K);
 void plan_dw(long M, int N, int K, int& splitk, int& mper);
 int emu_dw_launch(const DwArgs& g, bool h2, float* dW, float* db, float* workspace, hipStream_t st);
+struct DwShape { long M; int N, K; };
+int plan_dw_group(const DwShape* s, int n, int& rows_per_slice);
+long dw_group_workspace(const DwShape* s, int n);
+int emu_dw_group_launch(DwArgs* items, float* const* dW, float* const* db, int n, float* workspace, hipStream_t st);
 }
diff --git a/hoisdf_amd/csrc/gemm_emu.hip b/hoisdf_amd/csrc/gemm_emu.hip
--- a/hoisdf_amd/csrc/gemm_emu.hip
+++ b/hoisdf_amd/csrc/gemm_emu.hip
@@ -335,3 +335,95 @@
                                                 long workspace_floats, const uint32_t* dy_mag, const uint32_t* x_mag, void* stream) {
   return linear_bwd_weight_emu_mag(dy, lddy, relu_bits, drop_p, x, ldx, dW, lddw, db, M, N, K, workspace, workspace_floats, dy_mag, x_mag, stream);
 }
+
+namespace {
+bool group_item_ok(const hoisdf_dw_group_item& it) {
+  return it.M > 0 && it.M < (1L << 31) && it.N > 0 && it.K > 0 && it.N % 4 == 0 && it.K % 4 == 0;
+}
+bool in_group(const hoisdf_dw_group_item& it) { return form_h2() && dw_tile(it.K) == 256; }
+int group_shapes(const hoisdf_dw_group_item* items, int n, DwShape* shp, int* idx) {
+  int m = 0;
+  for (int i = 0; i < n; ++i)
+    if (in_group(items[i])) { shp[m] = DwShape{items[i].M, items[i].N, items[i].K}; idx[m++] = i; }
+  return m;
+}
+}
+
+extern "C" int hoisdf_linear_bwd_weight_emu_group_plan(const hoisdf_dw_group_item* items, int n, int* units, int* rows_per_slice, int* launches) {
+  HOISDF_REQUIRE(items && n > 0 && n <= DW_GROUP_MAX, HOISDF_ERR_INVALID, "linear_bwd_weight_emu_group_plan: 1 .. %d items", DW_GROUP_MAX);
+  DwShape shp[DW_GROUP_MAX];
+  for (int i = 0; i < n; ++i) {
+    HOISDF_REQUIRE(group_item_ok(items[i]), HOISDF_ERR_INVALID, "linear_bwd_weight_emu_group_plan: bad sizes (item %d)", i);
+    shp[i] = DwShape{items[i].M, items[i].N, items[i].K};
+  }
+  int rows;
+  const int u = plan_dw_group(shp, n, rows);
+  if (units) *units = u;
+  if (rows_per_slice) *rows_per_slice = rows;
+  if (launches) *launches = cdiv(u, 256);
+  return HOISDF_OK;
+}
+
+extern "C" long hoisdf_linear_bwd_weight_emu_group_workspace(const hoisdf_dw_group_item* items, int n) {
+  if (!items || n <= 0 || n > DW_GROUP_MAX) return 0;
+  DwShape shp[DW_GROUP_MAX]; int idx[DW_GROUP_MAX];
+  for (int i = 0; i < n; ++i) if (!group_item_ok(items[i])) return 0;
+  const int m = group_shapes(items, n, shp, idx);
+  long f = m > 0 ? dw_group_workspace(shp, m) : 0;
+  for (int i = 0; i < n; ++i)
+    if (!in_group(items[i])) f += (hoisdf_linear_bwd_weight_emu_workspace(items[i].M, items[i].N, items[i].K) + 3) & ~3L;
+  return f;
+}
+
+extern "C" int hoisdf_linear_bwd_weight_emu_group(const hoisdf_dw_group_item* items, int n, float* workspace, long workspace_floats, void* stream) {
+  HOISDF_REQUIRE(items && n > 0 && n <= DW_GROUP_MAX, HOISDF_ERR_INVALID, "linear_bwd_weight_emu_group: 1 .. %d items", DW_GROUP_MAX);
+  for (int i = 0; i < n; ++i) {
+    const hoisdf_dw_group_item& it = items[i];
+    HOISDF_REQUIRE(group_item_ok(it) && it.dy && it.x && it.dW && it.lddy >= it.N && it.ldx >= it.K && it.drop_p >= 0.f && it.drop_p < 1.f,
+                   HOISDF_ERR_INVALID, "linear_bwd_weight_emu_group: bad sizes or null pointer (item %d)", i);
+    HOISDF_REQUIRE(al16(it.dy) && al16(it.x) && al16(it.dW) && (it.lddy % 4 == 0) && (it.ldx % 4 == 0), HOISDF_ERR_INVALID,
+                   "linear_bwd_weight_emu_group: operands must be 16-byte aligned with leading dims multiples of 4 (item %d)", i);
+  }
+  const long need = hoisdf_linear_bwd_weight_emu_group_workspace(items, n);
+  HOISDF_REQUIRE(need == 0 || (workspace && workspace_floats >= need && al16(workspace)), HOISDF_ERR_WORKSPACE,
+                 "linear_bwd_weight_emu_group: workspace of %ld floats needed", need);
+  hipStream_t st = as_stream(stream);
+  DwShape shp[DW_GROUP_MAX]; int idx[DW_GROUP_MAX];
+  const int m = group_shapes(items, n, shp, idx);
+  float* w1 = workspace + (m > 0 ? dw_group_workspace(shp, m) : 0);
+  for (int i = 0; i < n; ++i) {
+    const hoisdf_dw_group_item& it = items[i];
+    if (in_group(it)) continue;
+    const long f = hoisdf_linear_bwd_weight_emu_workspace(it.M, it.N, it.K);
+    if (int rc = bwd_weight_emu(it.dy, it.lddy, it.relu_bits, it.relu_bits ? it.drop_p : 0.f, it.x, it.ldx, it.dW, it.K, it.db, it.M, it.N, it.K,
+                                w1, f, form_h2(), it.dy_mag, it.x_mag, stream)) return rc;
+    w1 += (f + 3) & ~3L;
+  }
+  if (m == 0) return HOISDF_OK;
+  long missing = 0;
+  for (int j = 0; j < m; ++j) missing += (items[idx[j]].dy_mag ? 0 : items[idx[j]].M) + (items[idx[j]].x_mag ? 0 : items[idx[j]].M);
+  uint32_t* words = nullptr;
+  if (missing > 0 && !(words = mag_scratch(st, missing))) { set_error("linear_bwd_weight_emu_group: cannot allocate the row magnitudes"); return HOISDF_ERR_LAUNCH; }
+  DwArgs args[DW_GROUP_MAX]; float* dW[DW_GROUP_MAX]; float* db[DW_GROUP_MAX];
+  for (int j = 0; j < m; ++j) {
+    const hoisdf_dw_group_item& it = items[idx[j]];
+    DwArgs g{};
+    g.dy = it.dy; g.lddy = it.lddy; g.x = it.x; g.ldx = it.ldx;
+    g.bits = it.relu_bits; g.ldbits = (it.N + 31) / 32; g.ascale = it.relu_bits ? 1.f / (1.f - it.drop_p) : 1.f;
+    g.M = (int)it.M; g.N = it.N; g.K = it.K;
+    g.tiles_n = cdiv(it.N, DT); g.tiles_k = cdiv(it.K, DT);
+    g.dy_amax = it.dy_mag; g.x_amax = it.x_mag;
+    if (!it.dy_mag) {
+      mag_trace("grad-weight dy", it.M, it.N);
+      if (int rc = emu_rowmag_launch(it.dy, it.lddy, it.M, it.N, words, st)) return rc;
+      g.dy_amax = words; words += it.M;
+    }
+    if (!it.x_mag) {
+      mag_trace("grad-weight x", it.M, it.K);
+      if (int rc = emu_rowmag_launch(it.x, it.ldx, it.M, it.K, words, st)) return rc;
+      g.x_amax = words; words += it.M;
+    }
+    args[j] = g; dW[j] = it.dW; db[j] = it.db;
+  }
+  return emu_dw_group_launch(args, dW, db, m, workspace, st);
+}
diff --git a/hoisdf_amd/csrc/gemm_emu_dw.hip b/hoisdf_amd/csrc/gemm_emu_dw.hip
--- a/hoisdf_amd/csrc/gemm_emu_dw.hip
+++ b/hoisdf_amd/csrc/gemm_emu_dw.hip
@@ -1,3 +1,5 @@
+#include <algorithm>
+
 #include "gemm_emu.h"
 
 namespace hoisdf {
@@ -26,7 +28,7 @@
 
 #define DW2_STORE_COLSUM()                                                                                             \
   do {                                                                                                                 \
-    if (HASDB && tk == 0) {                                                                                            \
+    if (HASDB && DW_COLSUM_RT && tk == 0) {                                                                            \
       float* red = reinterpret_cast<float*>(lds);                                                                      \
       if (isA) *reinterpret_cast<f32x4*>(&red[c * DT + 4 * cg]) = csum * post;                                         \
       __syncthreads();                                                                                                 \
@@ -205,6 +207,8 @@
   DW_EPILOGUE(DTK, acc[i][j][r]);
 }
 
+#define DW_MASKED_RT true
+#define DW_COLSUM_RT true
 #define DW2_STAGING_SETUP(A_U4_)                                                                                       \
    \
   const bool isA = wave < 2;                                                                                           \
@@ -217,9 +221,9 @@
    \
                                             \
   const int voff0 = col_ok ? (int)(((long)c * 8 * ld + col0) * 4) : 0x40000000;                                        \
-  const int boff0 = (MASK && isA && col_ok) ? (int)(((long)c * 8 * g.ldbits + (col0 >> 5)) * 4) : 0x40000000;          \
+  const int boff0 = (MASK && DW_MASKED_RT && isA && col_ok) ? (int)(((long)c * 8 * g.ldbits + (col0 >> 5)) * 4) : 0x40000000;          \
   const int ldb4 = (int)(ld * 4), ldm4 = g.ldbits * 4;                                                                 \
-  const uint32_t notA = isA ? 0u : 0xffffffffu;                                         \
+  const uint32_t notA = (isA && DW_MASKED_RT) ? 0u : 0xffffffffu;                       \
   const int bsh = col0 & 31;                                    \
   constexpr bool SWZ = true;                                                                                           \
   const int sw = SWZ ? (cg >> 1) & 3 : 0;                                                                              \
@@ -367,111 +371,57 @@
   u32x4* const s0 = lds_all;
   u32x4* const s1 = lds_all + STG;
   DW_TILE_SETUP(DT)
-  f16_saturate_on();
-  uint32_t am_dy = 0u, am_x = 0u;
-  for (int i = mbeg + (int)threadIdx.x; i < mend; i += NT) { am_dy = max(am_dy, g.dy_amax[i]); am_x = max(am_x, g.x_amax[i]); }
-  am_dy = block_max_u32(am_dy, red4);
-  __syncthreads();
-  am_x = block_max_u32(am_x, red4);
-
-  f32x16 acc[4][4];
-#pragma unroll
-  for (int i = 0; i < 4; ++i)
-#pragma unroll
-    for (int j = 0; j < 4; ++j)
-#pragma unroll
-      for (int r = 0; r < 16; ++r) acc[i][j][r] = 0.f;
-
-  DW2_STAGING_SETUP(A_U4)
-  uint32_t t0[4], t1[4];
-  const float sc = isA ? h2_scale(am_dy) : h2_scale(am_x);
-  f32x2 rp_, fu_;
-  f32x4 csum = {0.f, 0.f, 0.f, 0.f};
-#define DU1(j, pr)                                                                                                     \
-  do {                                                                                                                 \
-    f32x2 v_ = (j) < 2 ? f32x2{rvL[2 * (pr)][(j) & 1], rvL[2 * (pr) + 1][(j) & 1]} : f32x2{rvH[2 * (pr)][(j) & 1], rvH[2 * (pr) + 1][(j) & 1]}; \
-    if (MASK) {                                                                                                        \
-      if ((j) == 0) {                                                                                                  \
-        const uint32_t n0_ = ((rm[2 * (pr)] | notA) >> bsh) & 0xfu, n1_ = ((rm[2 * (pr) + 1] | notA) >> bsh) & 0xfu;   \
-        mpk = ((pr) == 0 ? 0u : mpk) | (n0_ << (8 * (pr))) | (n1_ << (8 * (pr) + 4));                                  \
-      }                                                                                                                \
-      float xa_, xb_;                                                              \
-      asm("v_and_b32 %0, %1, %2" : "=v"(xa_) : "v"(__builtin_amdgcn_sbfe((int)mpk, 8 * (pr) + (j), 1)), "v"(v_.x));    \
-      asm("v_and_b32 %0, %1, %2" : "=v"(xb_) : "v"(__builtin_amdgcn_sbfe((int)mpk, 8 * (pr) + 4 + (j), 1)), "v"(v_.y)); \
-      v_ = f32x2{xa_, xb_};                                                                                            \
-    }                                                                                                                  \
-    if (HASDB) csum[j] += v_.x + v_.y;                                                                                 \
-    v_ *= sc;                                                                                                          \
-    const f16x2 h_ = __builtin_convertvector(v_, f16x2);                       \
-    t0[pr] = __builtin_bit_cast(uint32_t, h_); rp_ = v_;                                                               \
-    fu_ = __builtin_convertvector(h_, f32x2);                                                                          \
-  } while (0)
-#define DU2(j, pr) do { f32x2 w_; PK_SUB(w_, rp_, fu_); t1[pr] = __builtin_bit_cast(uint32_t, __builtin_convertvector(w_, f16x2)); } while (0)
-#define DSTA(st, j, pl) (st)[wbase + ((j) ^ sw) + (pl) * 2 * DT] = ((pl) == 0 ? u32x4{t0[0], t0[1], t0[2], t0[3]} : u32x4{t1[0], t1[1], t1[2], t1[3]})
-#define DLA(st, p, i) __builtin_bit_cast(f16x8, (st)[aread + ((p) * 2 + kh) * DT + (i) * 32])
-#define DLB(st, p, j) __builtin_bit_cast(f16x8, (st)[bread + ((p) * 2 + kh) * DT + (j) * 32])
-#define M1(ax, bx, i, j, work) do { acc[i][j] = MFH(ax[i], bx[j], acc[i][j]); work; SB(); } while (0)
-#define MM(ax, bx) _Pragma("unroll") for (int i = 0; i < 4; ++i) _Pragma("unroll") for (int j = 0; j < 4; ++j) acc[i][j] = MFH(ax[i], bx[j], acc[i][j])
-#include "dw2h_phase.inc"
-#define DSTAGE_ALL(st)                                                                                                 \
-  do {                                                                                                                 \
-    _Pragma("unroll") for (int j = 0; j < 4; ++j) {                                                                    \
-      _Pragma("unroll") for (int pr = 0; pr < 4; ++pr) { DU1(j, pr); DU2(j, pr); }                                     \
-      DSTA(st, j, 0); DSTA(st, j, 1);                                                                                  \
-    }                                                                                                                  \
-  } while (0)
-
-  const int nslab2 = (max(nslab, 1) + 1) & ~1;
-  f16x8 aH[4], aL[4], bP[4], bQ[4], bL[4];
-  DLOAD_ALL(0);
-  DLOADM_ALL(0);
-  DSTAGE_ALL(s0);
-  DLOAD_ALL(1);
-  DLOADM_ALL(1);
-  __syncthreads();
-#pragma unroll
-  for (int i = 0; i < 4; ++i) { aL[i] = DLA(s0, 1, i); aH[i] = DLA(s0, 0, i); }
-#pragma unroll
-  for (int j = 0; j < 4; ++j) { bP[j] = DLB(s0, 0, j); bL[j] = DLB(s0, 1, j); }
-  MM(aL, bP); MM(aH, bL);
-  DSTAGE_ALL(s1);
-  DLOAD_ALL(2);
-  DLOADM_ALL(2);
-  SYNC();
-  for (int s = 1; s + 1 < nslab2; s += 2) {
-    DHPHASE(s1, s0, s, bP, bQ);
-    SYNC();
-    DHPHASE(s0, s1, s + 1, bQ, bP);
-    SYNC();
-  }
-  DHPHASE(s1, s0, nslab2 - 1, bP, bQ);
-  SB();
-  MM(aH, bQ);
-  __syncthreads();
-#undef DU1
-#undef DU2
-#undef DSTA
-#undef DLA
-#undef DLB
-#undef M1
-#undef MM
-#undef DHPHASE
-#undef DSTAGE_ALL
-  const float unscale = h2_inv_scale(am_dy) * h2_inv_scale(am_x);
-  const float post = MASK ? g.ascale : 1.f;
-  u32x4* lds = lds_all;
-  DW2_STORE_COLSUM();
-  DW_EPILOGUE(DT, acc[i][j][r] * (MASK ? post * unscale : unscale));
-}
-
-__global__ __launch_bounds__(1024) void emu_reduce_partials_kernel(const float* __restrict__ part, long stride, int splits,
-                                                                   float* __restrict__ out, long n, int blocks0,
-                                                                   const float* __restrict__ part1, long stride1,
-                                                                   float* __restrict__ out1, long n1) {
+#include "dw2h_body.inc"
+}
+
+#undef DW_MASKED_RT
+#undef DW_COLSUM_RT
+#define DW_MASKED_RT (g.bits != nullptr)
+#define DW_COLSUM_RT (g.colsum != nullptr)
+#define DW_GROUP_SETUP(u_)                                                                                             \
+  const int tid = threadIdx.x, lane = tid & 63, wave = tid >> 6;                                                       \
+  const int wm = wave >> 1, wn = wave & 1;                                                                             \
+  const int l31 = lane & 31, kh = lane >> 5;                                                                           \
+  const int ntile = g.tiles_n * g.tiles_k;                                                                             \
+  const int u = (u_), sfull = g.splitk & ~7, srest = g.splitk & 7;                                                      \
+  const bool in8 = u < sfull * ntile;                         \
+  const int split = in8 ? (u & 7) + 8 * (u / (8 * ntile)) : sfull + (u - sfull * ntile) % max(srest, 1);               \
+  const int t = in8 ? (u >> 3) % ntile : (u - sfull * ntile) / max(srest, 1);                                          \
+  if (split >= g.splitk || t >= ntile) return;                                                                         \
+  const int tn = t / g.tiles_k, tk = t - tn * g.tiles_k;                                                               \
+  const int n0 = tn * DT, k0 = tk * DT;                                                                                \
+  const int mbeg = split * g.m_per_split;                                                                              \
+  const int mend = min(g.M, mbeg + g.m_per_split);                                                                     \
+  const int nslab = (mend - mbeg + KS - 1) / KS;
+__global__ __launch_bounds__(NT, 1) void emu_dw2h_group_kernel(DwGroup grp) {
+  constexpr bool MASK = true, HASDB = true;
+  constexpr int A_U4 = 2 * 2 * DT;
+  constexpr int STG = 2 * A_U4;
+  constexpr int EPI = (4 * 32 * (DT / 2 + 4) * 4 + 15) / 16;
+  __shared__ __attribute__((aligned(16))) u32x4 lds_all[2 * STG > EPI ? 2 * STG : EPI];
+  __shared__ uint32_t red4[4];
+  u32x4* const s0 = lds_all;
+  u32x4* const s1 = lds_all + STG;
+  const int unit = grp.unit0 + (int)blockIdx.x;
+  int item = 0;
+  for (int i = 1; i < grp.n; ++i) item = unit >= grp.first[i] ? i : item;
+  const DwArgs g = grp.it[item];
+  DW_GROUP_SETUP(unit - grp.first[item])
+#include "dw2h_body.inc"
+}
+#undef DW_MASKED_RT
+#undef DW_COLSUM_RT
+
+__global__ __launch_bounds__(1024) void emu_reduce_partials_kernel(DwReduce r) {
+  int e = 0;
+  for (int i = 1; i < r.n; ++i) e = (int)blockIdx.x >= r.first_block[i] ? i : e;
+  const float* __restrict__ part = r.o[e].part;
+  float* __restrict__ out = r.o[e].out;
+  const long stride = r.o[e].stride, n = r.o[e].n;
+  const int splits = r.o[e].splits;
+  const int blk = (int)blockIdx.x - r.first_block[e];
   __shared__ float4 red[16][64];
   const int lane = threadIdx.x & 63, w = threadIdx.x >> 6;
-  int blk = blockIdx.x;
-  if (blk >= blocks0) { blk -= blocks0; part = part1; stride = stride1; out = out1; n = n1; }
   const long i = ((long)blk * 64 + lane) * 4;
   float4 s = make_float4(0.f, 0.f, 0.f, 0.f);
   if (i < n) {
@@ -514,6 +464,18 @@
   splitk = cdiv(M, mper);
 }
 
+namespace {
+void reduce_add(DwReduce& r, const float* part, long n, int splits, float* out) {
+  r.o[r.n] = DwReduce::Out{part, n, out, n, splits};
+  r.first_block[r.n + 1] = r.first_block[r.n] + (int)((n + 255) / 256);
+  ++r.n;
+}
+int reduce_launch(const DwReduce& r, hipStream_t st) {
+  hipLaunchKernelGGL(emu_reduce_partials_kernel, dim3((unsigned)r.first_block[r.n]), dim3(1024), 0, st, r);
+  return check_launch("linear_bwd_weight_emu reduce");
+}
+}
+
 int emu_dw_launch(const DwArgs& g, bool h2, float* dW, float* db, float* workspace, hipStream_t st) {
   const int dtk = dw_tile(g.K);
   const unsigned lb = 2u * (3 * 2 * DT + 3 * 2 * 128) * 16u;
@@ -537,13 +499,81 @@
   else hipLaunchKernelGGL((mask ? emu_dw_kernel<true, 128> : emu_dw_kernel<false, 128>), grid, block, lb, st, g);
   if (int rc = check_launch("linear_bwd_weight_emu")) return rc;
   if (g.splitk > 1) {
-    const long n = (long)g.N * g.K;
-    const int b0 = (int)((n + 255) / 256), b1 = db ? (g.N + 255) / 256 : 0;
-    hipLaunchKernelGGL(emu_reduce_partials_kernel, dim3((unsigned)(b0 + b1)), dim3(1024), 0, st, workspace, n, g.splitk, dW, n, b0,
-                       workspace + (size_t)g.splitk * g.N * g.K, (long)g.N, db, (long)g.N);
-    return check_launch("linear_bwd_weight_emu reduce");
+    DwReduce r{};
+    reduce_add(r, workspace, (long)g.N * g.K, g.splitk, dW);
+    if (db) reduce_add(r, workspace + (size_t)g.splitk * g.N * g.K, (long)g.N, g.splitk, db);
+    return reduce_launch(r, st);
   }
   return HOISDF_OK;
 }
 
-}
+constexpr int DW_SLOTS = 256;
+int plan_dw_group(const DwShape* s, int n, int& rows_per_slice) {
+  long tiles = 0, maxslabs = 1;
+  for (int i = 0; i < n; ++i) {
+    tiles += (long)cdiv(s[i].N, DT) * cdiv(s[i].K, DT);
+    maxslabs = std::max(maxslabs, (long)cdiv(s[i].M, KS));
+  }
+  long L = maxslabs, units = tiles;
+  if (tiles <= DW_SLOTS) {
+    for (L = 8; L < maxslabs; ++L) {
+      units = 0;
+      bool ok = true;
+      for (int i = 0; i < n && ok; ++i) {
+        const long slabs = cdiv(s[i].M, KS), sl = cdiv(slabs, L);
+        ok = sl <= std::max(1L, slabs / 8);
+        units += sl * cdiv(s[i].N, DT) * cdiv(s[i].K, DT);
+      }
+      if (ok && units <= DW_SLOTS) break;
+    }
+    if (L >= maxslabs) { L = std::max(maxslabs, 8L); units = tiles; }
+  }
+  rows_per_slice = (int)(L * KS);
+  return (int)units;
+}
+long dw_group_workspace(const DwShape* s, int n) {
+  int rows;
+  plan_dw_group(s, n, rows);
+  long f = 0;
+  for (int i = 0; i < n; ++i) {
+    const long sl = cdiv(s[i].M, rows);
+    if (sl > 1) f += sl * ((long)s[i].N * s[i].K + s[i].N);
+  }
+  return f;
+}
+
+int emu_dw_group_launch(DwArgs* items, float* const* dW, float* const* db, int n, float* workspace, hipStream_t st) {
+  if (n <= 0) return HOISDF_OK;
+  DwShape shp[DW_GROUP_MAX];
+  for (int i = 0; i < n; ++i) shp[i] = DwShape{items[i].M, items[i].N, items[i].K};
+  int rows;
+  const int units = plan_dw_group(shp, n, rows);
+  DwGroup grp{};
+  DwReduce r{};
+  float* w = workspace;
+  grp.n = n;
+  for (int i = 0; i < n; ++i) {
+    DwArgs& g = items[i];
+    g.m_per_split = rows; g.splitk = cdiv(g.M, rows);
+    if (g.splitk > 1) {
+      g.C = w; g.c_split_stride = (long)g.N * g.K;
+      w += (size_t)g.splitk * g.N * g.K;
+      g.colsum = db[i] ? w : nullptr; g.colsum_split_stride = g.N;
+      w += (size_t)g.splitk * g.N;
+      reduce_add(r, g.C, (long)g.N * g.K, g.splitk, dW[i]);
+      if (db[i]) reduce_add(r, g.colsum, (long)g.N, g.splitk, db[i]);
+    } else {
+      g.C = dW[i]; g.c_split_stride = 0; g.colsum = db[i]; g.colsum_split_stride = 0;
+    }
+    grp.it[i] = g;
+    grp.first[i + 1] = grp.first[i] + g.tiles_n * g.tiles_k * g.splitk;
+  }
+  if (grp.first[n] != units) { set_error("linear_bwd_weight_emu_group: plan and table disagree"); return HOISDF_ERR_INVALID; }
+  for (grp.unit0 = 0; grp.unit0 < units; grp.unit0 += DW_SLOTS) {
+    hipLaunchKernelGGL(emu_dw2h_group_kernel, dim3((unsigned)std::min(DW_SLOTS, units - grp.unit0)), dim3(NT), 0, st, grp);
+    if (int rc = check_launch("linear_bwd_weight_emu_group")) return rc;
+  }
+  return r.n > 0 ? reduce_launch(r, st) : HOISDF_OK;
+}
+
+}
diff --git a/hoisdf_amd/csrc/heads.hip b/hoisdf_amd/csrc/heads.hip
--- a/hoisdf_amd/csrc/heads.hip
+++ b/hoisdf_amd/csrc/heads.hip
@@ -57,6 +57,8 @@
   uint32_t* mg = chain_mags(c, M, m->n_layers + 1);
   const bool fwd_mags = mg && s.mag && saved_mags().get(s.mag) != 0;
   const uint32_t* g_mag = nullptr;
+  const bool dmags = c.dry && chain_mags_on(c, M);
+  if (dmags && emu_rows(c, M, dy, lddy, m->dims[last + 1])) g_mag = dry_words();
   if (mg && emu_rows(c, M, dy, lddy, m->dims[last + 1])) {
     if ((c.rc = emu_mag_measure(dy, lddy, M, m->dims[last + 1], mg + (long)(last + 1) * M, c.st)) != HOISDF_OK) return;
     g_mag = mg + (long)(last + 1) * M;
@@ -74,6 +76,7 @@
     uint32_t* gin_mag = mg && i > 0 && emu_rows(c, M, g, ldg, m->dims[i + 1]) ? mg + (long)i * M : nullptr;
     lin_bwd_input(c, g, ldg, s.bits[i], 0.f, m->w[i], m->dims[i], m->img_t[i], gin, ldgin, M, m->dims[i + 1], m->dims[i], i == 0 ? accumulate_dx : 0,
                   g_mag, gin_mag);
+    if (dmags && i > 0 && emu_rows(c, M, g, ldg, m->dims[i + 1])) gin_mag = dry_words();
     g = gin; ldg = ldgin; g_mag = gin_mag;
   }
 }
@@ -119,6 +122,7 @@
     c.rc = hoisdf_token_build_bwd_ordered(dtok, s.fea, F, sdf, beta, dfea, F, dbeta, part, B, P, S, row0, D, stream);
   }
   mlp_backward(c, mlp, G, feat, mlp->dims[0], M, s.mlp, dfea, F, dfeat, mlp->dims[0], accumulate_dfeat);
+  dw_flush(c);
   if (c.ok() && !dry && ws.overflow) { set_error("tokens_bwd: workspace too small"); return HOISDF_ERR_WORKSPACE; }
   return c.rc;
 }
@@ -214,6 +218,7 @@
   const int E = mv->dims[0];
   mlp_backward(c, mv, Gv, enc, E, M, s.vote, doff, 3 * J, denc, E, 0);
   mlp_backward(c, mc, Gc, enc, E, M, s.cl, dcls, J, denc, E, 1, enc_mag(c, mv, enc, E, M, s.vote));
+  dw_flush(c);
   if (c.ok() && !dry && ws.overflow) { set_error("heads_vote_bwd: workspace too small"); return HOISDF_ERR_WORKSPACE; }
   return c.rc;
 }
diff --git a/hoisdf_amd/csrc/layers.hip b/hoisdf_amd/csrc/layers.hip
--- a/hoisdf_amd/csrc/layers.hip
+++ b/hoisdf_amd/csrc/layers.hip
@@ -207,8 +207,8 @@
   const long bmag_bytes = ((long)MAG_BROWS * M + Ms + (long)g.H * g.B) * 4;
   uint32_t* bmag = static_cast<uint32_t*>(ws.take(bmag_bytes));
   const bool mags = layer_mags(c, g) && (dry || bmag);
-  auto mg = [&](int i) -> uint32_t* { return mags && bmag ? bmag + (long)i * M : nullptr; };
-  uint32_t* const mag_dqkv = mags && bmag ? bmag + (long)MAG_BROWS * M : nullptr;
+  auto mg = [&](int i) -> uint32_t* { return !mags ? nullptr : bmag ? bmag + (long)i * M : dry ? dry_words() : nullptr; };
+  uint32_t* const mag_dqkv = !mags ? nullptr : bmag ? bmag + (long)MAG_BROWS * M : dry ? dry_words() : nullptr;
   uint32_t* const head_do = mags && bmag ? bmag + (long)MAG_BROWS * M + Ms : nullptr;
   auto fm = [&](int i) -> const uint32_t* { return mags && fwd_mags && s.mag ? s.mag + (long)i * M : nullptr; };
   uint32_t* const smag = mags && fwd_mags ? s.mag : nullptr;
@@ -256,6 +256,7 @@
     lin_bwd_weight(c, dkv, 2 * E, nullptr, 0.f, x, E, G->dw_in + (size_t)E * E, G->db_in ? G->db_in + E : nullptr, Ms, 2 * E, E);
     if (!dry && c.ok()) c.rc = rows_copy_add(dx, (long)g.S * E, dxq, (long)g.nq * E, g.B, g.nq, E, 1, c.st);
   }
+  dw_flush(c);
   if (c.ok() && !dry && ws.overflow) { set_error("encoder_layer_bwd: workspace too small"); return HOISDF_ERR_WORKSPACE; }
   return c.rc;
 }
diff --git a/hoisdf_amd/csrc/sdf_query.hip b/hoisdf_amd/csrc/sdf_query.hip
--- a/hoisdf_amd/csrc/sdf_query.hip
+++ b/hoisdf_amd/csrc/sdf_query.hip
@@ -261,8 +261,9 @@
   uint32_t* bmag = static_cast<uint32_t*>(ws.take((long)BM_N * n * 4));
   const bool mags = train_mags(c, n) && !dry && bmag && s.mag;
   const bool fmags = mags && saved_mags().get(s.mag) != 0;
-  auto mg = [&](int i) -> uint32_t* { return mags ? bmag + (long)i * n : nullptr; };
-  auto fm = [&](int i) -> const uint32_t* { return fmags ? s.mag + (long)i * n : nullptr; };
+  const bool dmags = dry && train_mags(c, n);
+  auto mg = [&](int i) -> uint32_t* { return mags ? bmag + (long)i * n : dmags ? dry_words() : nullptr; };
+  auto fm = [&](int i) -> const uint32_t* { return fmags ? s.mag + (long)i * n : dmags ? dry_words() : nullptr; };
   if (mags) c.rc = hipMemsetAsync(bmag, 0, (size_t)BM_N * n * 4, c.st) == hipSuccess ? HOISDF_OK : HOISDF_ERR_LAUNCH;
   if (!dry && c.ok()) c.rc = sdf_head_bwd_mag(d_sdf, s.raw, s.h3, HID0, w->dec_w4, dh3, HID0, G->d_dec_w4, G->d_dec_b4, n, HID0, clamp, mg(BM_DH3), stream);
   lin_bwd_input(c, dh3, HID0, s.b3, drop_p, w->dec_w3, HID0, w->emu_img_t[5], dh2, HID0, n, HID0, HID0, 0, mg(BM_DH3), mg(BM_DH2));
@@ -279,6 +280,7 @@
   lin_bwd_weight(c, dx0, CAT_LD, s.bf, 0.f, s.ha, HID0, G->d_sdfin_w1, G->d_sdfin_b1, n, LAT, HID0, 0, nullptr, fm(TM_HA));
   lin_bwd_input(c, dha, HID0, s.ba, 0.f, w->sdfin_w0, C, w->emu_img_t[0], dfeat, C, n, HID0, C, 0, mg(BM_DHA), nullptr);
   lin_bwd_weight(c, dha, HID0, s.ba, 0.f, s.feat, C, G->d_sdfin_w0, G->d_sdfin_b0, n, HID0, C, 0, mg(BM_DHA), fm(TM_FEAT));
+  dw_flush(c);
   if (!dry && c.ok() && dpyr)
     c.rc = hoisdf_project_gather_bwd(dpyr, points, sample_idx, n, rps, center, cam_intr, scale, img_h, img_w, dfeat, C, stream);
   if (c.ok() && !dry && ws.overflow) { set_error("sdf_query_bwd: workspace too small"); return HOISDF_ERR_WORKSPACE; }
diff --git a/include/hoisdf.h b/include/hoisdf.h
--- a/include/hoisdf.h
+++ b/include/hoisdf.h
@@ -95,6 +95,17 @@
 int hoisdf_linear_bwd_weight_emu_mag(const float* dy, int lddy, const uint32_t* relu_bits, float drop_p, const float* x, int ldx,
                                      float* dW, int lddw, float* db, long M, int N, int K, float* workspace, long workspace_floats,
                                      const uint32_t* dy_mag, const uint32_t* x_mag, void* stream);
+typedef struct hoisdf_dw_group_item {
+  const float* dy; int lddy;
+  const uint32_t* relu_bits; float drop_p;
+  const float* x; int ldx;
+  float* dW; float* db;
+  long M; int N, K;
+  const uint32_t* dy_mag; const uint32_t* x_mag;
+} hoisdf_dw_group_item;
+int hoisdf_linear_bwd_weight_emu_group(const hoisdf_dw_group_item* items, int n, float* workspace, long workspace_floats, void* stream);
+long hoisdf_linear_bwd_weight_emu_group_workspace(const hoisdf_dw_group_item* items, int n);
+int hoisdf_linear_bwd_weight_emu_group_plan(const hoisdf_dw_group_item* items, int n, int* units, int* rows_per_slice, int* launches);
 int hoisdf_linear_fwd_emu(const float* x, int ldx, const void* w_image, const float* bias, float* y, int ldy, long M, int N,
                           int K, int act, float drop_p, uint64_t seed, uint32_t* relu_bits, void* stream);
 int hoisdf_linear_bwd_input_emu(const float* dy, int lddy, const uint32_t* relu_bits, float drop_p, const void* wt_image,
```

Result: faster. 451.3 (median of 5 runs) (+1.4%).
